# nreHieW/Eagle

Measured on AMD Instinct MI355X. Metric: frames/sec end-to-end (detect+keypoint+homography) @1280x720, higher is better.
Workload: dtype f32 (split: hi/lo binary16 pairs, 3 x fp16 MFMA per product, fp32 accumulate); detector (1.4 % of the FLOP): f32, exact v_mfma_f32_16x16x4_f32 chains

## Files before the change

eagle_amd/csrc/common.h:

```cpp
#pragma once
#include <hip/hip_runtime.h>
#include <hip/hip_fp16.h>
#include <cstdint>
#include <cstdio>
#include <string>
#include <vector>

#include "../../include/eagle.h"

namespace eagle {

enum Act : int { ACT_NONE = 0, ACT_RELU = 1, ACT_SILU = 2 };

struct Err {
    int code;
    std::string msg;
};
[[noreturn]] void fail(int code, const char* fmt, ...);

#define HIP_CHECK(expr)                                                                                \
    do {                                                                                               \
        hipError_t _e = (expr);                                                                        \
        if (_e != hipSuccess) ::eagle::fail(EAGLE_E_HIP, "%s failed: %s (%s:%d)", #expr, hipGetErrorString(_e), \
                                            __FILE__, __LINE__);                                       \
    } while (0)

void ensure_max_dynamic_lds(const void* fn, int bytes);

struct TView {
    void* p = nullptr;
    int n = 0, h = 0, w = 0;
    int c = 0;
    int cs = 0;
    int off = 0;
    int f32 = 0;
    size_t esize() const { return f32 ? 4 : 2; }
    TView slice(int o, int cc) const { TView v = *this; v.off = off + o; v.c = cc; return v; }
};

struct ConvConfig {
    int ks = 3, stride = 1;
    int kc = 0;
    int nt = 0;
    int wx = 2;
    int cin = 0, cout_pad = 0;
    int variant = 0;
};
struct ArgmaxPart { float score; int idx; };
struct ConvLaunch {
    ConvConfig cfg;
    TView x, y, r1, r2;
    const void* w = nullptr;
    const float* bias = nullptr;
    int pre_act = 0, post_act = 0;
    int out_f32 = 0;
    double flop = 0;
    float descale = 1.0f;
    ArgmaxPart* const* am_slot = nullptr;
    unsigned* const* sat_slot = nullptr;
};
int conv_tiles_per_frame(int precision, const ConvConfig& cfg, int ho, int wo);
bool conv_supported(int precision, const ConvConfig& cfg);
void conv_launch(int precision, const ConvLaunch& L, hipStream_t s);
size_t conv_weight_elems(int precision, const ConvConfig& cfg);
size_t conv_lds_bytes(int precision, const ConvConfig& cfg);
void conv_tile_weights(int precision, const ConvConfig& cfg, const float* w_hwio, int cin_real, int cout_real, void* dst, float* descale = nullptr);
inline int prec_tensor_fmt(int precision) { return precision == EAGLE_PREC_F32 ? 1 : precision == EAGLE_PREC_F32S ? 2 : 0; }
inline bool prec_is_f16_kernels(int precision) { return precision == EAGLE_PREC_F16 || precision == EAGLE_PREC_F32S; }
ConvConfig conv_choose(int precision, int ks, int stride, int cin_pad, int cout_pad, int wo, bool plain_epilogue = false, bool second_residual = false);

struct BneckLaunch {
    TView x, res, y;
    const void *w1 = nullptr, *w2 = nullptr, *w3 = nullptr;
    const float *b1 = nullptr, *b2 = nullptr, *b3 = nullptr;
    float ds1 = 1.f, ds2 = 1.f, ds3 = 1.f;
    unsigned* const* sat_slot = nullptr;
    unsigned long long* dbg = nullptr;
    bool ds_fused = false;
};
bool bneck_supported(const TView& x, int cmid, int cout);
void bneck_tile_weights(const float* w, int taps, int cin, int cout, std::vector<_Float16>& out, float* descale);
void bneck_scale_bias(std::vector<float>& b, float descale);
void bneck_launch(const BneckLaunch& L, hipStream_t s);

struct LetterBox { int new_h, new_w, top, left, out_h, out_w; };
LetterBox letterbox_geometry(int h, int w, int imgsz, int square = 0);
void preprocess_launch(int precision, const uint8_t* d_bgr, int n, int h, int w, const TView& kp, const TView& det,
                       const LetterBox& lb, hipStream_t s, int which = 3, int det_precision = -1);
struct FuseUp { TView z; };
void fuse_sum_launch(const TView& base, const FuseUp* ups, int n_up, int relu, const TView& y, hipStream_t s, unsigned* sat = nullptr);
void maxpool5_launch(const TView& x, const TView& y, hipStream_t s);
void upsample2_launch(const TView& x, const TView& y, hipStream_t s);
void split_to_f32_launch(const TView& x, const TView& y, hipStream_t s);

void heat_argmax_launch(const TView& logits, ArgmaxPart* parts, int chunks, hipStream_t s);

struct DetLevel { TView box, cls; int gh, gw; float stride; int a0; };
struct DetScratch {
    int A = 0;
    float* boxes = nullptr;
    float* conf = nullptr;
    int* cls = nullptr;
    unsigned long long* keys = nullptr;
    int* count = nullptr;
};
void yolo_decode_launch(const DetLevel* lv, int n_lv, int n, int nc, float conf_floor, const DetScratch& sc, hipStream_t s);

struct PostParams {
    int frame_h, frame_w, in_h, in_w;
    int hm_h, hm_w, hm_chunks;
    double keypoint_conf, detector_conf, ransac_thresh;
    float nms_iou;
    int ransac_max_iters, lm_iters;
};
void nms_launch(const DetScratch& sc, int n, const PostParams& pp, EagleFrameResult* d_out, hipStream_t s);
void post_launch(const ArgmaxPart* parts, int n, const PostParams& pp, EagleFrameResult* d_out, hipStream_t s);
void reproject_launch(EagleFrameResult* d_recs, const double* d_Hs, const unsigned char* d_flags, int n, int frame_h, int frame_w, hipStream_t s);
void homography_only_launch(const float* d_img, const float* d_world, int npts, double thresh, int max_iters, int lm_iters,
                            double* d_H, uint8_t* d_mask, int* d_ok, hipStream_t s);


struct ClipView {
    const uint8_t* bgr = nullptr;
    const uint8_t* g[3] = {nullptr, nullptr, nullptr};
    int lh[3] = {0, 0, 0}, lw[3] = {0, 0, 0};
    int levels = 0;
    int n = 0, h = 0, w = 0;
};
struct MemList { int n; EagleFlowKp kp[EAGLE_N_LANDMARKS]; };
struct ChainState {
    int n_prev; EagleFlowKp prev[EAGLE_N_LANDMARKS];
    int has_H, compute_h; double H[9];
    int stalled;
    int error;
    int lk_valid, lk_n;
    float lk_prev[2 * EAGLE_N_LANDMARKS], lk_next[2 * EAGLE_N_LANDMARKS];
    unsigned char lk_status[EAGLE_N_LANDMARKS];
    int flow_n; EagleFlowKp flow[EAGLE_N_LANDMARKS];
};
void gray_pyramid_launch(const uint8_t* d_bgr, int n, int h, int w, uint8_t* g0, uint8_t* g1, uint8_t* g2, hipStream_t s);
void lk_launch(const ClipView& cv, int src_frame, int dst_frame, ChainState* st, const MemList* mem, int kint, hipStream_t s);
struct EccResult { int ok, iters; double rho; float M[6]; };
void ecc_small_launch(const uint8_t* gray, uint8_t* small, int n, int h, int w, int dh, int dw, double inv_scale , hipStream_t s);
void ecc_launch(const uint8_t* small, const uint8_t* carry, const int2* pairs, int n_pairs, EccResult* out, int h, int w, int max_iter, double eps, hipStream_t s);
struct YuvArgs {
    const uint8_t* src;
    uint8_t* dst;
    int h, w;
    int64_t frame_stride, y_pitch, c_offset, c_pitch, v_offset;
    int c_step;
    int vec;
};
void yuv_to_bgr_launch(const YuvArgs& a, int n, hipStream_t s);
void team_colors_launch(const uint8_t* d_bgr, int n_frames, int fh, int fw, const EagleCrop* d_crops, int n_crops, int* d_counts, hipStream_t s);

void reid_crop_launch(const uint8_t* d_bgr, int n_frames, int fh, int fw, const EagleCrop* d_crops, int n, const TView& out, hipStream_t s);
void reid_conv7_launch(const TView& x, const float* w, const float* b, const TView& y, int n, hipStream_t s);
void reid_maxpool3s2_launch(const TView& x, const TView& y, int n, hipStream_t s);
void reid_avgpool2_launch(const TView& x, const TView& y, int n, hipStream_t s);
void reid_dw3_launch(const TView& x, const float* w, const float* b, const TView& y, int n, hipStream_t s);
void reid_gate_launch(const TView* streams, const float* w1, const float* b1, const float* w2, const float* b2, int c_real, int r, float* g, const TView& y, int n, hipStream_t s);
void reid_head_launch(const TView& x, const float* w, const float* b, float* feats, int dim, int n, hipStream_t s);

struct Tracker;
Tracker* tracker_create(const EagleTrackParams* p);
void tracker_destroy(Tracker* t);
bool tracker_apply(Tracker* t, EagleFrameResult* rec, int frame_h, int frame_w, double detector_conf, const double* warp = nullptr,
                   const float* feats = nullptr, const int* feat_det = nullptr, int n_feat = 0);
void similarity_ransac(const double* p0, const double* p1, int n, double* W6);
int lk_debug(const char* key, long long value, void* out, long long out_bytes);
void decode_mem_launch(const ArgmaxPart* parts, int n, const PostParams& pp, MemList* mem, int first, int stride, hipStream_t s);
void chain_launch(const ClipView& cv, ChainState* st, const MemList* mem, EagleFrameResult* recs, const PostParams& pp, int frame,
                  int kint, int hint, int calib, hipStream_t s);
void flow_filter_launch(const ClipView& cv, ChainState* st, int hue_frame, hipStream_t s);

}
```

eagle_amd/csrc/conv.hip:

```cpp
#include <algorithm>
#include <cmath>
#include <cstdlib>
#include <mutex>

#include "common.h"
#include "dmath.h"
#include "conv_internal.h"

namespace eagle {

static int f16_ps(int kc) { const int g = kc / 8; return kc * 2 + ((g % 2 == 0) ? 16 : 0); }
static int f16_ni(int ks, int kc) { return (ks * ks * (kc / 8) + 3) / 4; }

enum FormKind { GENERIC, WSTAT, ADIRECT };
enum StrideForm { S1, S2D, S2T };
enum WeightImage { W_F32, W_F16, W_F16_S2D, W_SPLIT, W_SPLIT_AD, W_SPLIT_S2D, W_SPLIT_M32 };
struct Form {
    int prec, variant, kind;
    int pw;
    int sform, rows, cols;
    int kc, nt, halo_bufs;
    int wimage;
    int grid_cap;
    ConvKernelGetter get;
};
static constexpr Form gen(int prec, int variant, int pw, int wimage, int kind = GENERIC) { return {prec, variant, kind, pw, S1, 0, 0, 0, 0, 0, wimage, 0, nullptr}; }
static constexpr Form ad(int prec, int variant, int sform, int rows, int cols, int nt, int halo_bufs, int wimage, ConvKernelGetter get, int grid_cap = 0)
{
    return {prec, variant, ADIRECT, 0, sform, rows, cols, prec == EAGLE_PREC_F16 ? 32 : 16, nt, halo_bufs, wimage, grid_cap, get};
}
static constexpr int F16 = EAGLE_PREC_F16, F32 = EAGLE_PREC_F32, F32S = EAGLE_PREC_F32S;
static constexpr Form g_forms[] = {
    gen(F32, 0, 4, W_F32), gen(F32, 3, 2, W_F32), gen(F32, 4, 1, W_F32),
    gen(F16, 0, 4, W_F16), gen(F16, 2, 4, W_F16), gen(F16, 3, 2, W_F16), gen(F16, 4, 1, W_F16), gen(F16, 6, 4, W_F16, WSTAT), gen(F16, 7, 2, W_F16, WSTAT),
    ad(F16, 8, S1, 4, 32, 12, 2, W_F16, conv_ad_kernel_s1_bn192), ad(F16, 9, S1, 8, 32, 6, 2, W_F16, conv_ad_kernel_s1_bn96),
    ad(F16, 10, S2D, 4, 32, 12, 2, W_F16_S2D, conv_ad_kernel_s2_bn192), ad(F16, 11, S2D, 8, 32, 6, 2, W_F16_S2D, conv_ad_kernel_s2_bn96),
    gen(F32S, 0, 4, W_SPLIT), gen(F32S, 3, 2, W_SPLIT), gen(F32S, 18, 6, W_SPLIT),
    ad(F32S, 8, S1, 4, 32, 12, 2, W_SPLIT_AD, conv_ad_split_kernel_bn192), ad(F32S, 9, S1, 8, 32, 6, 2, W_SPLIT_AD, conv_ad_split_kernel_bn96),
    ad(F32S, 10, S2D, 4, 32, 12, 2, W_SPLIT_S2D, conv_ad_split_kernel_s2_bn192), ad(F32S, 11, S2D, 8, 32, 6, 2, W_SPLIT_S2D, conv_ad_split_kernel_s2_bn96),
    ad(F32S, 12, S1, 8, 32, 3, 2, W_SPLIT_AD, conv_ad_split_kernel48), ad(F32S, 13, S1, 16, 32, 3, 1, W_SPLIT_AD, conv_ad_split_kernel48sb),
    ad(F32S, 19, S1, 16, 32, 3, 2, W_SPLIT_AD, conv_ad_split_kernel48ring, 256),
    ad(F32S, 14, S2T, 4, 32, 12, 1, W_SPLIT_AD, conv_ad_split_kernel_s2t_bn192), ad(F32S, 15, S2T, 4, 32, 6, 1, W_SPLIT_AD, conv_ad_split_kernel_s2t_bn96),
    ad(F32S, 21, S1, 4, 32, 12, 2, W_SPLIT_M32, conv_ad_split32_kernel_bn192), ad(F32S, 22, S1, 8, 32, 6, 2, W_SPLIT_M32, conv_ad_split32_kernel_bn96),
    ad(F32S, 23, S1, 2, 64, 12, 2, W_SPLIT_M32, conv_ad_split32_kernel_w64_bn192), ad(F32S, 24, S1, 4, 64, 6, 2, W_SPLIT_M32, conv_ad_split32_kernel_w64_bn96)};

static const Form* find_form(int precision, int variant)
{
    for (const Form& f : g_forms)
        if (f.prec == precision && f.variant == variant) return &f;
    return nullptr;
}
static const Form& form_of(int precision, const ConvConfig& c)
{
    const Form* f = find_form(precision, c.variant);
    if (!f) fail(EAGLE_E_NOKERNEL, "no conv kernel form: prec=%d variant=%d", precision, c.variant);
    return *f;
}
static int kind_of(int precision, const ConvConfig& c) { const Form* f = find_form(precision, c.variant); return f ? f->kind : -1; }

static size_t lds_bytes(int precision, const ConvConfig& c)
{
    const Form& f = form_of(precision, c);
    if (f.kind == ADIRECT) {
        int hpix, rec, strips;
        if (precision == EAGLE_PREC_F16) { hpix = f.sform == S2D ? (f.rows + 1) * 33 : (f.rows + 2) * 34; rec = 96; strips = 4 * 32 * 112; }
        else if (f.wimage == W_SPLIT_M32) { hpix = (f.rows + 2) * (f.cols + 2); rec = 80; strips = 4 * 32 * 128; }
        else { hpix = f.sform == S2T ? (2 * f.rows + 1) * 66 : (f.rows + 2) * 34; rec = 96; strips = 4 * 16 * 208; }
        const int slabs = ((hpix * rec + 1023) / 1024 + 3) / 4 * 4;
        return (size_t)f.halo_bufs * slabs * 1024 + strips;
    }
    const int th = 4 * f.pw / c.wx, tw = 16 * c.wx;
    const int hw = (tw - 1) * c.stride + c.ks, hh = (th - 1) * c.stride + c.ks;
    const int bn = c.nt * 16;
    if (precision == EAGLE_PREC_F16) {
        const size_t operands = (size_t)f16_ni(c.ks, c.kc) * 4 * bn * 16 + (size_t)hh * hw * f16_ps(c.kc);
        const size_t strips = (size_t)4 * f.pw * 16 * (bn * 2 + 16);
        return f.kind == WSTAT ? operands + strips + 16 : std::max(operands + 16, strips);
    }
    if (precision == EAGLE_PREC_F32S) {
        const size_t operands = (size_t)f16_ni(c.ks, c.kc) * 2 * 4 * bn * 16 + (size_t)hh * hw * f16_ps(2 * c.kc);
        const size_t strips = (size_t)4 * f.pw * 16 * (bn * 4 + 16);
        return std::max(operands + 16, strips);
    }
    return (size_t)c.ks * c.ks * (c.kc / 4) * 4 * bn * 4 + (size_t)hh * hw * (c.kc + 1) * 4;
}

size_t conv_lds_bytes(int precision, const ConvConfig& c) { return lds_bytes(precision, c); }
int conv_tiles_per_frame(int precision, const ConvConfig& c, int ho, int wo)
{
    const Form& f = form_of(precision, c);
    const int th = f.kind == ADIRECT ? f.rows : 4 * f.pw / c.wx, tw = f.kind == ADIRECT ? f.cols : 16 * c.wx;
    return ((wo + tw - 1) / tw) * ((ho + th - 1) / th);
}

static const Inst* generic_inst(int precision, const ConvConfig& c)
{
    for (auto part : {conv_inst_part0, conv_inst_part1, conv_inst_part2, conv_inst_part3, conv_inst_split0, conv_inst_split1, conv_inst_split2}) {
        int n = 0;
        const Inst* t = part(&n);
        for (int k = 0; k < n; ++k)
            if (t[k].prec == precision && t[k].ks == c.ks && t[k].s == c.stride && t[k].kc == c.kc && t[k].nt == c.nt && t[k].variant == c.variant) return &t[k];
    }
    return nullptr;
}
bool conv_supported(int precision, const ConvConfig& c)
{
    const Form* f = find_form(precision, c.variant);
    if (f && f->kind == ADIRECT) return c.ks == 3 && c.stride == (f->sform == S1 ? 1 : 2) && c.kc == f->kc && c.nt == f->nt;
    return f && generic_inst(precision, c);
}

struct Tuned { int ks, s, cin, cout, wo, kc, nt, wx, variant; };
static const Tuned g_tuned[] = {
#include "conv_tuned.inc"
    {0, 0, 0, 0, 0, 0, 0, 0, 0}};
static const Tuned g_tuned_f32[] = {
#include "conv_tuned_f32.inc"
    {0, 0, 0, 0, 0, 0, 0, 0, 0}};
static const Tuned g_tuned_split[] = {
#include "conv_tuned_split.inc"
    {0, 0, 0, 0, 0, 0, 0, 0, 0}};
static bool tuned_match(const Tuned& t, const ConvConfig& c, int wo, ConvConfig* q)
{
    if (t.ks != c.ks || t.s != c.stride || t.cin != c.cin || t.cout != c.cout_pad || t.wo != wo) return false;
    *q = c; q->kc = t.kc; q->nt = t.nt; q->wx = t.wx; q->variant = t.variant;
    return true;
}

static bool env_force(const char* name, int* a, int* b, int* c) { const char* f = getenv(name); return f && sscanf(f, "%d,%d,%d", a, b, c) == 3; }
static bool env_off(const char* name) { const char* e = getenv(name); return e && atoi(e) == 0; }

static const int g_nts[] = {6, 4, 3, 2, 1};
static ConvConfig with_ad(ConvConfig c, int kc, int v192, int v96)
{
    c.kc = kc;
    if (c.cout_pad % 192 == 0) { c.nt = 12; c.variant = v192; } else { c.nt = 6; c.variant = v96; }
    return c;
}

static ConvConfig choose_f32(ConvConfig c, int wo)
{
    ConvConfig q = c; q.kc = (c.cin < 16) ? 4 : 16;
    if (env_force("EAGLE_F32_FORCE", &q.nt, &q.wx, &q.variant) && (q.wx == 1 || q.wx == 2) && q.nt >= 1 && c.cout_pad % (16 * q.nt) == 0 &&
        conv_supported(EAGLE_PREC_F32, q) && lds_bytes(EAGLE_PREC_F32, q) <= 160 * 1024)
        return q;
    for (const Tuned& t : g_tuned_f32)
        if (tuned_match(t, c, wo, &q) && conv_supported(EAGLE_PREC_F32, q)) return q;
    c.nt = 1;
    for (int nt : g_nts)
        if (c.cout_pad % (16 * nt) == 0) { c.nt = nt; break; }
    c.kc = (c.cin < 16) ? 4 : 16;
    if (c.stride == 2 && c.ks == 3) {
        q = c; q.variant = 3;
        if (conv_supported(EAGLE_PREC_F32, q)) return q;
    }
    return c;
}

static ConvConfig choose_split(ConvConfig c, int wo, bool plain_epilogue)
{
    const int prec = EAGLE_PREC_F32S, cin = c.cin, cout = c.cout_pad;
    ConvConfig q = c;
    if (env_force("EAGLE_CONV_FORCE", &q.kc, &q.nt, &q.variant) && cin % q.kc == 0 && cout % (16 * q.nt) == 0 && conv_supported(prec, q)) {
        if (form_of(prec, q).pw == 6) q.wx = 3;
        if (lds_bytes(prec, q) <= 160 * 1024) return q;
    }
    if (plain_epilogue && c.ks == 3 && c.stride == 2 && cin % 48 == 0 && cout % 96 == 0) return with_ad(c, 16, 14, 15);
    if (!env_off("EAGLE_CONV_M32") && plain_epilogue && c.ks == 3 && c.stride == 1 && cin % 16 == 0 && cout % 96 == 0) return with_ad(c, 16, 21, wo > 32 ? 24 : 22);
    for (const Tuned& t : g_tuned_split)
        if (tuned_match(t, c, wo, &q)) {
            const Form* f = find_form(prec, q.variant);
            if (kind_of(prec, q) == ADIRECT && !(plain_epilogue && cin % (f->sform == S2D ? 16 : 48) == 0)) continue;
            if (conv_supported(prec, q) && lds_bytes(prec, q) <= 160 * 1024) return q;
        }
    if (plain_epilogue && c.ks == 3 && c.stride == 1 && cin % 48 == 0 && cout % 96 == 0) return with_ad(c, 16, 8, 9);
    static const int skcs[] = {32, 16, 8};
    long best = -1;
    c.nt = 1; c.kc = 8; c.variant = 0;
    for (int variant : {0, 3})
        for (int nt : g_nts) {
            if (cout % (16 * nt)) continue;
            for (int kc : skcs) {
                if (cin % kc) continue;
                ConvConfig t = c; t.nt = nt; t.kc = kc; t.variant = variant;
                if (!conv_supported(prec, t)) continue;
                if (lds_bytes(prec, t) > 80 * 1024) continue;
                const int pw = form_of(prec, t).pw;
                if (nt * pw > 12) continue;
                const long score = (long)nt * pw * 1000 + kc * 10 + (variant == 0 ? 1 : 0);
                if (score > best) { best = score; c.nt = nt; c.kc = kc; c.variant = variant; }
            }
        }
    return c;
}

static ConvConfig choose_f16(ConvConfig c, int wo, bool plain_epilogue, bool plain_one)
{
    const int prec = EAGLE_PREC_F16, cin = c.cin, cout = c.cout_pad;
    ConvConfig q = c;
    if (env_force("EAGLE_CONV_FORCE", &q.kc, &q.nt, &q.variant) && cin % q.kc == 0 && cout % (16 * q.nt) == 0 && conv_supported(prec, q) &&
        lds_bytes(prec, q) <= 160 * 1024 && (kind_of(prec, q) == WSTAT ? plain_one : kind_of(prec, q) == ADIRECT ? plain_epilogue : true))
        return q;
    if (plain_epilogue && c.ks == 3 && c.stride == 1 && cin % 32 == 0 && cout % 96 == 0) return with_ad(c, 32, 8, 9);
    if (plain_epilogue && c.ks == 3 && c.stride == 2 && cin % 8 == 0 && cin >= 32 && cout % 96 == 0) return with_ad(c, 32, 10, 11);
    for (const Tuned& t : g_tuned)
        if (tuned_match(t, c, wo, &q)) {
            if (kind_of(prec, q) == WSTAT && !plain_one) continue;
            if (conv_supported(prec, q) && lds_bytes(prec, q) <= 160 * 1024) return q;
        }
    static const int kcs[] = {64, 48, 32, 16, 8};
    long best = -1;
    c.nt = 1; c.kc = 8;
    for (int nt : g_nts) {
        if (cout % (16 * nt)) continue;
        for (int kc : kcs) {
            if (cin % kc) continue;
            ConvConfig t = c; t.nt = nt; t.kc = kc;
            if (!conv_supported(prec, t)) continue;
            if (lds_bytes(prec, t) > 80 * 1024) continue;
            const long score = (long)kc * nt * 1000 + kc;
            if (score > best) { best = score; c.nt = nt; c.kc = kc; }
        }
    }
    return c;
}

ConvConfig conv_choose(int precision, int ks, int stride, int cin_pad, int cout_pad, int wo, bool plain_epilogue, bool second_residual)
{
    ConvConfig c;
    c.ks = ks; c.stride = stride; c.cin = cin_pad; c.cout_pad = cout_pad;
    c.wx = (wo > 16) ? 2 : 1;
    if (precision == EAGLE_PREC_F32) return choose_f32(c, wo);
    if (precision == EAGLE_PREC_F32S) return choose_split(c, wo, plain_epilogue);
    return choose_f16(c, wo, plain_epilogue, plain_epilogue && !second_residual);
}

size_t conv_weight_elems(int precision, const ConvConfig& c)
{
    const int bn = c.nt * 16, nblk = c.cout_pad / bn, nch = c.cin / c.kc;
    switch (form_of(precision, c).wimage) {
    case W_F16_S2D: return (size_t)nblk * (4 * c.cin / 32) * 16 * bn * 8;
    case W_F16: return (size_t)nblk * nch * f16_ni(c.ks, c.kc) * 4 * bn * 8;
    case W_SPLIT_S2D: return (size_t)nblk * (4 * c.cin / 16) * 6 * 4 * bn * 8;
    case W_SPLIT_M32: return (size_t)nblk * (c.cin / 16) * 18 * (bn / 32) * 512;
    case W_SPLIT_AD: return (size_t)nblk * (c.cin / 16) * 14 * 4 * bn * 8;
    case W_SPLIT: return (size_t)nblk * nch * f16_ni(c.ks, c.kc) * 2 * 4 * bn * 8;
    default: return (size_t)nblk * nch * c.ks * c.ks * (c.kc / 4) * 4 * bn;
    }
}

void conv_tile_weights(int precision, const ConvConfig& c, const float* w, int cin_real, int cout_real, void* dst, float* descale)
{
    const int bn = c.nt * 16, nblk = c.cout_pad / bn, nch = c.cin / c.kc, taps = c.ks * c.ks, wimage = form_of(precision, c).wimage;
    auto W = [&](int tap, int ci, int co) -> float {
        return (ci < cin_real && co < cout_real) ? w[((size_t)tap * cin_real + ci) * cout_real + co] : 0.0f;
    };
    if (descale) *descale = 1.0f;
    if (precision == EAGLE_PREC_F32S) {
        float amax = 0.f;
        for (size_t k = 0; k < (size_t)taps * cin_real * cout_real; ++k) amax = std::max(amax, std::fabs(w[k]));
        int e = 0;
        if (amax > 0.f) (void)std::frexp(amax, &e);
        const int sw = 15 - e;
        const float scale = std::ldexp(1.0f, sw);
        if (descale) *descale = std::ldexp(1.0f, -(sw + 4));
        _Float16* d = (_Float16*)dst;
        if (wimage == W_SPLIT_S2D) {
            const int per_phase = c.cin / 16;
            for (int b = 0; b < nblk; ++b)
                for (int ch = 0; ch < 4 * per_phase; ++ch)
                    for (int k = 0; k < 6; ++k)
                        for (int qq = 0; qq < 4; ++qq)
                            for (int nn = 0; nn < bn; ++nn)
                                for (int j = 0; j < 8; ++j) {
                                    const int ph = ch / per_phase, c0 = (ch - ph * per_phase) * 16, ry = ph >> 1, rx = ph & 1;
                                    const int tp = k < 4 ? k : 2 * (k - 4) + (qq >> 1), tyy = tp >> 1, txx = tp & 1;
                                    const int ky = tyy == 0 ? (ry == 1 ? 0 : -1) : (ry == 0 ? 1 : 2), kx = txx == 0 ? (rx == 1 ? 0 : -1) : (rx == 0 ? 1 : 2);
                                    float v = 0.f;
                                    if (ky >= 0 && kx >= 0) v = W(ky * 3 + kx, c0 + (qq & 1) * 8 + j, b * bn + nn) * scale;
                                    const _Float16 hi = (_Float16)v;
                                    *d++ = k < 4 ? hi : (_Float16)(v - (float)hi);
                                }
            return;
        }
        if (wimage == W_SPLIT_M32) {
            for (int b = 0; b < nblk; ++b)
                for (int ch = 0; ch < c.cin / 16; ++ch)
                    for (int tap = 0; tap < 9; ++tap)
                        for (int part = 0; part < 2; ++part)
                            for (int mb = 0; mb < bn / 32; ++mb)
                                for (int l = 0; l < 64; ++l)
                                    for (int j = 0; j < 8; ++j) {
                                        const float v = W(tap, ch * 16 + (l >> 5) * 8 + j, b * bn + mb * 32 + (l & 31)) * scale;
                                        const _Float16 hi = (_Float16)v;
                                        *d++ = part == 0 ? hi : (_Float16)(v - (float)hi);
                                    }
            return;
        }
        if (wimage == W_SPLIT_AD) {
            for (int b = 0; b < nblk; ++b)
                for (int ch = 0; ch < c.cin / 16; ++ch)
                    for (int k = 0; k < 14; ++k)
                        for (int qq = 0; qq < 4; ++qq)
                            for (int nn = 0; nn < bn; ++nn)
                                for (int j = 0; j < 8; ++j) {
                                    const int tap = k < 9 ? k : 2 * (k - 9) + (qq >> 1);
                                    float v = 0.f;
                                    if (tap < 9) v = W(tap, ch * 16 + (qq & 1) * 8 + j, b * bn + nn) * scale;
                                    const _Float16 hi = (_Float16)v;
                                    *d++ = k < 9 ? hi : (_Float16)(v - (float)hi);
                                }
            return;
        }
        const int G = c.kc / 8, NGR = taps * G, NI = f16_ni(c.ks, c.kc);
        for (int b = 0; b < nblk; ++b)
            for (int ch = 0; ch < nch; ++ch)
                for (int i = 0; i < NI; ++i)
                    for (int part = 0; part < 2; ++part)
                        for (int qq = 0; qq < 4; ++qq)
                            for (int nn = 0; nn < bn; ++nn)
                                for (int j = 0; j < 8; ++j) {
                                    const int g = 4 * i + qq;
                                    float v = 0.f;
                                    if (g < NGR) { const int tap = g / G, cg = g % G; v = W(tap, ch * c.kc + cg * 8 + j, b * bn + nn) * scale; }
                                    const _Float16 hi = (_Float16)v;
                                    *d++ = part == 0 ? hi : (_Float16)(v - (float)hi);
                                }
        return;
    }
    if (wimage == W_F16_S2D) {
        _Float16* d = (_Float16*)dst;
        const int nch2 = 4 * c.cin / 32;
        for (int b = 0; b < nblk; ++b)
            for (int ch = 0; ch < nch2; ++ch)
                for (int g = 0; g < 16; ++g)
                    for (int nn = 0; nn < bn; ++nn)
                        for (int j = 0; j < 8; ++j) {
                            const int tp = g / 4, cg = g % 4, tyy = tp >> 1, txx = tp & 1;
                            const int sc = ch * 32 + cg * 8 + j, ph = sc / c.cin, ci = sc - ph * c.cin, ry = ph >> 1, rx = ph & 1;
                            const int ky = tyy == 0 ? (ry == 1 ? 0 : -1) : (ry == 0 ? 1 : 2), kx = txx == 0 ? (rx == 1 ? 0 : -1) : (rx == 0 ? 1 : 2);
                            *d++ = (_Float16)((ky < 0 || kx < 0) ? 0.f : W(ky * 3 + kx, ci, b * bn + nn));
                        }
        return;
    }
    if (precision == EAGLE_PREC_F16) {
        const int G = c.kc / 8, NGR = taps * G, NI = f16_ni(c.ks, c.kc);
        _Float16* d = (_Float16*)dst;
        for (int b = 0; b < nblk; ++b)
            for (int ch = 0; ch < nch; ++ch)
                for (int g = 0; g < NI * 4; ++g)
                    for (int nn = 0; nn < bn; ++nn)
                        for (int j = 0; j < 8; ++j) {
                            float v = 0.f;
                            if (g < NGR) {
                                const int tap = g / G, cg = g % G;
                                v = W(tap, ch * c.kc + cg * 8 + j, b * bn + nn);
                            }
                            *d++ = (_Float16)v;
                        }
    } else {
        const int CSTEPS = c.kc / 4;
        float* d = (float*)dst;
        for (int b = 0; b < nblk; ++b)
            for (int ch = 0; ch < nch; ++ch)
                for (int tap = 0; tap < taps; ++tap)
                    for (int cs = 0; cs < CSTEPS; ++cs)
                        for (int qq = 0; qq < 4; ++qq)
                            for (int nn = 0; nn < bn; ++nn) *d++ = W(tap, ch * c.kc + cs * 4 + qq, b * bn + nn);
    }
}

static std::mutex g_page_mutex;
static const void* conv_zero_page()
{
    static void* z[64] = {};
    int dev = 0;
    HIP_CHECK(hipGetDevice(&dev));
    std::lock_guard<std::mutex> g(g_page_mutex);
    if (!z[dev]) { HIP_CHECK(hipMalloc(&z[dev], 256)); HIP_CHECK(hipMemset(z[dev], 0, 256)); }
    return z[dev];
}
static void* conv_trash_page()
{
    static void* z[64] = {};
    int dev = 0;
    HIP_CHECK(hipGetDevice(&dev));
    std::lock_guard<std::mutex> g(g_page_mutex);
    if (!z[dev]) HIP_CHECK(hipMalloc(&z[dev], 8192));
    return z[dev];
}

void conv_launch(int precision, const ConvLaunch& L, hipStream_t s)
{
    const ConvConfig& c = L.cfg;
    if (!conv_supported(precision, c)) fail(EAGLE_E_NOKERNEL, "no conv kernel instance: prec=%d ks=%d s=%d kc=%d nt=%d", precision, c.ks, c.stride, c.kc, c.nt);
    const Form& f = form_of(precision, c);
    ConvArgs a;
    a.x = L.x.p; a.xcs = L.x.cs; a.xoff = L.x.off; a.N = L.x.n; a.H = L.x.h; a.W = L.x.w;
    a.w = L.w; a.bias = L.bias;
    a.y = L.y.p; a.ycs = L.y.cs; a.yoff = L.y.off; a.Ho = L.y.h; a.Wo = L.y.w;
    a.r1 = L.r1.p; a.r1cs = L.r1.cs; a.r1off = L.r1.off;
    a.r2 = L.r2.p; a.r2cs = L.r2.cs; a.r2off = L.r2.off;
    a.descale = L.descale;
    if (precision == EAGLE_PREC_F32S) {
        if (L.x.f32 != 2 || (L.r1.p && L.r1.f32 != 2) || (L.r2.p && L.r2.f32 != 2) || L.y.f32 != (L.out_f32 ? 1 : 2))
            fail(EAGLE_E_INVALID, "split conv: operand tensor formats do not match the family");
        a.xcs *= 2; a.xoff *= 2; a.r1cs *= 2; a.r1off *= 2; a.r2cs *= 2; a.r2off *= 2;
        if (!L.out_f32) { a.ycs *= 2; a.yoff *= 2; }
    }
    if (!a.r1 && a.r2) { a.r1 = a.r2; a.r1cs = a.r2cs; a.r1off = a.r2off; a.r2 = nullptr; }
    a.pre_act = L.pre_act; a.post_act = L.post_act; a.out_f32 = L.out_f32 || precision == EAGLE_PREC_F32;
    a.wx = c.wx;
    a.nchunks = c.cin / c.kc;
    a.zeros = conv_zero_page(); a.trash = conv_trash_page(); a.xcd = 0; a.gy = 1; a.stack = 0;
    a.am = L.am_slot ? *L.am_slot : nullptr; a.am_cs = c.cout_pad;
    a.sat = (L.sat_slot && precision == EAGLE_PREC_F32S) ? *L.sat_slot : nullptr;
    if (f.kind == ADIRECT) {
        if (a.out_f32 || a.pre_act != 0 || a.post_act > 1 || L.am_slot || (precision == EAGLE_PREC_F32S && c.cin % (f.wimage == W_SPLIT_AD ? 48 : 16)))
            fail(EAGLE_E_NOKERNEL, "A-direct conv needs 2-byte / split output, pre_act none, post_act in {none, ReLU} and, in the split family, Cin = 16 k (48 k for variants 8, 9 and 12 - 15)");
        if (f.sform == S2D) a.nchunks = 4 * c.cin / c.kc;
        a.tiles_x = (a.Wo + f.cols - 1) / f.cols; a.tiles_y = (a.Ho + f.rows - 1) / f.rows;
        a.gy = c.cout_pad / (c.nt * 16);
        const size_t lim = (size_t)1 << 31;
        if ((size_t)a.N * a.H * a.W * a.xcs * 2 >= lim || (size_t)a.N * a.Ho * a.Wo * std::max(std::max(a.ycs, a.r1 ? a.r1cs : 0), a.r2 ? a.r2cs : 0) * 2 >= lim)
            fail(EAGLE_E_INVALID, "fp16 conv: a tensor of %d frames reaches 2 GiB; use a smaller device batch", a.N);
        const int nres = (a.r1 ? 1 : 0) + (a.r2 ? 1 : 0);
        const int items = a.tiles_x * a.tiles_y * a.N * a.gy;
        const bool deep = items <= 256;
        for (bool d : {false, true}) ensure_max_dynamic_lds((const void*)f.get(nres, d), 160 * 1024);
        hipLaunchKernelGGL(f.get(nres, deep), dim3(f.grid_cap ? std::min(items, f.grid_cap) : items), dim3(256), lds_bytes(precision, c), s, a);
        HIP_CHECK(hipGetLastError());
        return;
    }
    const int th = 4 * f.pw / c.wx, tw = 16 * c.wx;
    a.tiles_x = (a.Wo + tw - 1) / tw; a.tiles_y = (a.Ho + th - 1) / th;
    if (precision == EAGLE_PREC_F32) {
        if (!env_off("EAGLE_F32_STACK") && c.stride == 1 && a.N > 1 && a.Ho == a.H) { a.stack = 1; a.tiles_y = (a.N * (a.Ho + 1) + th - 1) / th; }
        if ((size_t)a.N * a.H * a.W * a.xcs * 4 >= ((size_t)1 << 31)) fail(EAGLE_E_INVALID, "fp32 conv: the input tensor of %d frames reaches 2 GiB; use a smaller device batch", a.N);
    }
    const bool ws = f.kind == WSTAT;
    if (a.am && (!prec_is_f16_kernels(precision) || ws))
        fail(EAGLE_E_NOKERNEL, "fused heat-map maxima need the generic fp16 kernel");
    if (prec_is_f16_kernels(precision)) {
        const size_t lim = (size_t)1 << 31;
        const size_t cs_out = std::max(std::max(a.out_f32 ? 2 * a.ycs : a.ycs, a.r1 ? a.r1cs : 0), a.r2 ? a.r2cs : 0);
        if ((size_t)a.N * a.H * a.W * a.xcs * 2 >= lim || (size_t)a.N * a.Ho * a.Wo * cs_out * 2 >= lim)
            fail(EAGLE_E_INVALID, "fp16 conv: a tensor of %d frames reaches 2 GiB; use a smaller device batch", a.N);
    }
    const ConvKernel fn = generic_inst(precision, c)->fn;
    const size_t lds = lds_bytes(precision, c);
    ensure_max_dynamic_lds((const void*)fn, 160 * 1024);
    const int gy = c.cout_pad / (c.nt * 16);
    int gx = a.stack ? a.tiles_x * a.tiles_y : a.tiles_x * a.tiles_y * a.N;
    if (ws) {
        if (c.kc != c.cin || a.out_f32 || a.r2 || a.pre_act != 0 || a.post_act > 1 || (size_t)a.N * a.H * a.W * a.xcs * 2 >= (1ull << 31) || (size_t)a.N * a.Ho * a.Wo * std::max(a.ycs, a.r1 ? a.r1cs : 0) * 2 >= (1ull << 31))
            fail(EAGLE_E_NOKERNEL, "weight-stationary conv needs kc == cin, fp16 output, at most one residual, pre_act none, post_act in {none, ReLU} and tensors below 2 GiB (kc=%d cin=%d)", c.kc, c.cin);
        const int per_cu = (int)std::max<size_t>(1, std::min<size_t>(2, (160 * 1024) / lds));
        const int unit = 8 * gy;
        gx = std::max(unit, std::min((gx * gy + unit - 1) / unit * unit, 256 * per_cu / unit * unit));
    }
    a.gy = gy;
    a.xcd = (prec_is_f16_kernels(precision) && !ws && (c.ks == 3 || (c.ks == 1 && gy > 1))) ? 1 : 0;
    dim3 grid(gx, gy);
    if (a.xcd) grid = dim3(gx * gy, 1);
    if (ws) grid = dim3(gx, 1);
    hipLaunchKernelGGL(fn, grid, dim3(256), lds, s, a);
    HIP_CHECK(hipGetLastError());
}

}
```

eagle_amd/csrc/conv_internal.h:

```cpp
#pragma once
#include "common.h"

namespace eagle {

using half8 = __attribute__((ext_vector_type(8))) _Float16;
using half4 = __attribute__((ext_vector_type(4))) _Float16;
using f32x4 = __attribute__((ext_vector_type(4))) float;
using u32x4 = __attribute__((ext_vector_type(4))) unsigned int;
using u32x2 = __attribute__((ext_vector_type(2))) unsigned int;

struct ConvArgs {
    const void* x; int xcs, xoff; int N, H, W;
    const void* w; const float* bias;
    void* y; int ycs, yoff; int Ho, Wo;
    const void* r1; int r1cs, r1off;
    const void* r2; int r2cs, r2off;
    int pre_act, post_act, out_f32;
    int wx, tiles_x, tiles_y, nchunks;
    int gy;
    int stack;
    int xcd;
    ArgmaxPart* am;
    int am_cs;
    float descale;
    const void* zeros;
    void* trash;
    unsigned* sat;
};

struct BneckArgs {
    const void* x; int xcs, xoff; int N, H, W, nch1;
    const void *w1, *w2, *w3; const float *b1, *b2, *b3; float ds1, ds2, ds3;
    const void* r; int rcs, roff;
    void* y; int ycs, yoff;
    int tiles_x, tiles_y;
    unsigned* sat;
    unsigned long long* dbg;
};

typedef void (*ConvKernel)(ConvArgs);
struct Inst { int prec, ks, s, kc, nt, variant; ConvKernel fn; };
const Inst* conv_inst_part0(int* n); const Inst* conv_inst_part1(int* n); const Inst* conv_inst_part2(int* n); const Inst* conv_inst_part3(int* n);
const Inst* conv_inst_split0(int* n); const Inst* conv_inst_split1(int* n); const Inst* conv_inst_split2(int* n);
inline int res_slot(int n_res) { return n_res < 0 ? 0 : n_res > 2 ? 2 : n_res; }
typedef ConvKernel (*ConvKernelGetter)(int n_res, bool deep);
ConvKernel conv_ad_kernel_s1_bn192(int n_res, bool deep);
ConvKernel conv_ad_kernel_s1_bn96(int n_res, bool deep);
ConvKernel conv_ad_kernel_s2_bn192(int n_res, bool deep);
ConvKernel conv_ad_kernel_s2_bn96(int n_res, bool deep);
ConvKernel conv_ad_split_kernel_bn192(int n_res, bool deep);
ConvKernel conv_ad_split_kernel_bn96(int n_res, bool deep);
ConvKernel conv_ad_split_kernel_s2_bn192(int n_res, bool deep);
ConvKernel conv_ad_split_kernel_s2_bn96(int n_res, bool deep);
ConvKernel conv_ad_split_kernel_s2t_bn192(int n_res, bool deep);
ConvKernel conv_ad_split_kernel_s2t_bn96(int n_res, bool deep);
ConvKernel conv_ad_split_kernel48(int n_res, bool deep);
ConvKernel conv_ad_split_kernel48sb(int n_res, bool deep);
ConvKernel conv_ad_split_kernel48ring(int n_res, bool deep);
ConvKernel conv_ad_split32_kernel_bn192(int n_res, bool deep);
ConvKernel conv_ad_split32_kernel_bn96(int n_res, bool deep);
ConvKernel conv_ad_split32_kernel_w64_bn192(int n_res, bool deep);
ConvKernel conv_ad_split32_kernel_w64_bn96(int n_res, bool deep);

}
```

eagle_amd/csrc/conv_kernels.inc:

```
#ifndef EAGLE_CONV_KERNELS_INC
#define EAGLE_CONV_KERNELS_INC
#ifndef EAGLE_ABL
#define EAGLE_ABL 0
#endif
template <int KC> struct F16Geom {
    static constexpr int G = KC / 8;
    static constexpr int PS = KC * 2 + ((G % 2 == 0) ? 16 : 0);
};

using i32x4 = __attribute__((ext_vector_type(4))) int;
__device__ __forceinline__ i32x4 make_rsrc(const void* p, int bytes)
{
    const unsigned long long b = (unsigned long long)p;
    i32x4 r = {(int)(unsigned)b, (int)((unsigned)(b >> 32) & 0xFFFF), bytes, 0x00020000};
    return r;
}
__device__ __forceinline__ float relu_if(float v, bool relu) { return (relu && !(v > 0.0f)) ? 0.0f : v; }

using rsrc_t = __amdgpu_buffer_rsrc_t;
__device__ __forceinline__ rsrc_t tensor_rsrc(const void* p) { return __builtin_amdgcn_make_buffer_rsrc((void*)p, 0, p ? 0x7FFFFFFF : 0, 0x00020000); }
constexpr unsigned OOB_OFF = 0x80000000u;
#ifndef EAGLE_STORE_NT
#define EAGLE_STORE_NT 1
#endif
// ... 114 lines not shown
                float best = -1.0f; int idx = 0x7fffffff;
#pragma unroll
                for (int p = 0; p < PW; ++p) {
                    if (pix[p] == OOB_OFF) continue;
                    const float sg = d_sigmoidf(acc[tt][p][r]);
                    const int li = (int)pix[p] - n * a.Ho * a.Wo;
                    if (sg > best || (sg == best && li < idx)) { best = sg; idx = li; }
                }
                bs[tt * 4 + r] = best; bi[tt * 4 + r] = idx;
            }
#pragma unroll
        for (int m = 1; m < 16; m <<= 1)
#pragma unroll
            for (int k = 0; k < NT * 4; ++k) {
                const float ob = __shfl_xor(bs[k], m, 64); const int oi = __shfl_xor(bi[k], m, 64);
                if (ob > bs[k] || (ob == bs[k] && oi < bi[k])) { bs[k] = ob; bi[k] = oi; }
            }
        ArgmaxPart* red = (ArgmaxPart*)smem_base;
        if (lx == 0) {
#pragma unroll
            for (int tt = 0; tt < NT; ++tt)
#pragma unroll
                for (int r = 0; r < 4; ++r) { ArgmaxPart v; v.score = bs[tt * 4 + r]; v.idx = bi[tt * 4 + r]; red[wave * BN + tt * 16 + q * 4 + r] = v; }
        }
        __syncthreads();
        const int tid = wave * 64 + lane;
        if (tid < BN) {
            ArgmaxPart b = red[tid];
#pragma unroll
            for (int w = 1; w < 4; ++w) { const ArgmaxPart o = red[w * BN + tid]; if (o.score > b.score || (o.score == b.score && o.idx < b.idx)) b = o; }
            const int TH = 4 * PW / WX, TW = 16 * WX;
            const int tile = (oy0 / TH) * a.tiles_x + ox0 / TW;
            a.am[((size_t)n * a.tiles_x * a.tiles_y + tile) * a.am_cs + nb * BN + tid] = b;
        }
        return;
    }
    if (a.out_f32) {
#pragma unroll
        for (int p = 0; p < PW; ++p) {
            if (pix[p] == OOB_OFF) continue;
#pragma unroll
            for (int tt = 0; tt < NT; ++tt)
                *(float4*)((float*)a.y + (size_t)pix[p] * a.ycs + a.yoff + co0 + tt * 16) = make_float4(acc[tt][p][0], acc[tt][p][1], acc[tt][p][2], acc[tt][p][3]);
        }
        return;
    }
    if constexpr (SPLIT) {
        float m = 0.0f;
#pragma unroll
        for (int p = 0; p < PW; ++p)
#pragma unroll
            for (int tt = 0; tt < NT; ++tt) { const float mm = split_absmax4(m, acc[tt][p][0], acc[tt][p][1], acc[tt][p][2], acc[tt][p][3]); m = pix[p] == OOB_OFF ? m : mm; }
        split_report(a.sat, n, m);
    }
#pragma unroll
    for (int p = 0; p < PW; ++p)
#pragma unroll
        for (int tt = 0; tt < NT; ++tt) {
            if constexpr (SPLIT) {
                split_store4(strip + (p * 16 + lx) * RS + split_elem(tt * 16 + q * 4) * 2, acc[tt][p][0], acc[tt][p][1], acc[tt][p][2], acc[tt][p][3]);
            } else {
                half4 o = {(_Float16)acc[tt][p][0], (_Float16)acc[tt][p][1], (_Float16)acc[tt][p][2], (_Float16)acc[tt][p][3]};
                *(half4*)(strip + (p * 16 + lx) * RS + (tt * 16 + q * 4) * 2) = o;
            }
        }
    const rsrc_t ys = tensor_rsrc(a.y);
#pragma unroll
    for (int e0 = 0; e0 < PW * 16 * GO; e0 += 64) {
        const int e = e0 + lane;
        const int px = e / GO, grp = e - px * GO, p = px >> 4, lxp = px & 15;
        const int s = wave * PW + p, row = s / WX, xb = s - row * WX;
        const int oy = oy0 + row, ox = ox0 + xb * 16 + lxp;
        const bool ok = e < PW * 16 * GO && oy < a.Ho && ox < a.Wo;
        const u32x4 v = *(const u32x4*)(strip + (ok ? px * RS + grp * 16 : 0));
        const unsigned vo = (ok && !((EAGLE_ABL == 3 || EAGLE_ABL >= 4) && SPLIT)) ? ((unsigned)((n * a.Ho + oy) * a.Wo + ox) * (unsigned)a.ycs + (unsigned)(a.yoff + nb * EB + grp * 8)) * 2u : OOB_OFF;
        __builtin_amdgcn_raw_buffer_store_b128(v, ys, vo, 0, SPLIT ? EAGLE_STORE_NT * 2 : EAGLE_F16_STORE_NT * 2);
    }
}

template <int R_, int M_, int r> __device__ __forceinline__ void sg_step()
{
    if constexpr (r < R_) {
        __builtin_amdgcn_sched_group_barrier(0x100, 1, 0);
        __builtin_amdgcn_sched_group_barrier(0x008, (M_ * (r + 1)) / R_ - (M_ * r) / R_, 0);
        sg_step<R_, M_, r + 1>();
    }
}
template <int NI_, int R_, int M_, int i> __device__ __forceinline__ void sg_all()
{
    if constexpr (i + 1 < NI_) { sg_step<R_, M_, 0>(); sg_all<NI_, R_, M_, i + 1>(); }
}
template <int NI_, int R_, int M_> __device__ __forceinline__ void mfma_phase_schedule_rm()
{
    __builtin_amdgcn_sched_group_barrier(0x100, R_, 0);
    sg_all<NI_, R_, M_, 0>();
    __builtin_amdgcn_sched_group_barrier(0x008, M_, 0);
}
template <int NI_, int NT_, int PW_> __device__ __forceinline__ void mfma_phase_schedule()
{
    __builtin_amdgcn_sched_group_barrier(0x100, NT_ + PW_, 0);
    sg_all<NI_, NT_ + PW_, NT_ * PW_, 0>();
    __builtin_amdgcn_sched_group_barrier(0x008, NT_ * PW_, 0);
}

#if EAGLE_ABL == 1 || EAGLE_ABL == 4 || EAGLE_ABL == 5 || EAGLE_ABL == 6 || EAGLE_ABL == 8 || EAGLE_ABL == 9
__device__ __forceinline__ f32x4 abl_xor(const half8& a, const half8& b, f32x4 c)
{
    const u32x4 ua = __builtin_bit_cast(u32x4, a), ub = __builtin_bit_cast(u32x4, b);
    u32x4 uc = __builtin_bit_cast(u32x4, c);
    uc[0] = uc[0] ^ ua[0] ^ ub[3];
    return __builtin_bit_cast(f32x4, uc);
}
#define EAGLE_MFMA_SPLIT(A_, B_, C_) abl_xor(A_, B_, C_)
#else
#define EAGLE_MFMA_SPLIT(A_, B_, C_) __builtin_amdgcn_mfma_f32_16x16x32_f16(A_, B_, C_, 0, 0, 0)
#endif
template <int KS, int S, int KC, int NT, bool PIPE, int PW, bool SPLIT = false>
__global__ __launch_bounds__(256, 2) void conv_f16_kernel(ConvArgs a)
{
    constexpr int KCS = SPLIT ? 2 * KC : KC;
    constexpr int GL = KC / 8;
    constexpr int G = F16Geom<KCS>::G;
#ifndef EAGLE_SPLIT_PLANAR
#define EAGLE_SPLIT_PLANAR 0
#endif
    constexpr bool PLANAR = SPLIT && KC == 16 && EAGLE_SPLIT_PLANAR;
    constexpr int PS = PLANAR ? 96 : F16Geom<KCS>::PS;
    constexpr int LO_OFF = PLANAR ? 32 : 16;
#ifndef EAGLE_S2_COLPLANES
#define EAGLE_S2_COLPLANES 0
#endif
    constexpr bool COLPLANES = S == 2 && KS == 3 && EAGLE_S2_COLPLANES;
    constexpr int TAPS = KS * KS;
    constexpr int NGR = TAPS * GL;
    constexpr int NI = (NGR + 3) / 4;
    constexpr int BN = NT * 16;
    constexpr int HALFW = 4 * BN * 16;
    constexpr int STEPB = SPLIT ? 2 * HALFW : HALFW;
    constexpr int WBYTES = NI * STEPB;
    extern __shared__ __attribute__((aligned(16))) char smem[];
    char* lds_w = smem;
    char* lds_a = smem + WBYTES + 16;

    const int WX = a.wx, TH = 4 * PW / WX, TW = 16 * WX;
    const int halo_w = (TW - 1) * S + KS, halo_h = (TH - 1) * S + KS;
    const int tid = threadIdx.x, lane = tid & 63, wave = tid >> 6, q = lane >> 4, lx = lane & 15;
    int t = blockIdx.x, nb = blockIdx.y;
    if (a.xcd) {
        const int gy = a.gy, total = a.tiles_x * a.tiles_y * a.N * gy;
        const int b = blockIdx.x, xcd = b & 7, k = b >> 3, qn = total >> 3, rn = total & 7;
        const int item = (xcd < rn ? xcd * (qn + 1) : rn * (qn + 1) + (xcd - rn) * qn) + k;
        t = item / gy; nb = item - t * gy;
    }
    const int tx = t % a.tiles_x; t /= a.tiles_x;
    const int ty = t % a.tiles_y;
    const int n = t / a.tiles_y;
    const int oy0 = ty * TH, ox0 = tx * TW;
    const int iy0 = oy0 * S - KS / 2, ix0 = ox0 * S - KS / 2;

    f32x4 acc[NT][PW];
#pragma unroll
    for (int i = 0; i < NT; ++i)
#pragma unroll
        for (int p = 0; p < PW; ++p) acc[i][p] = f32x4{0.f, 0.f, 0.f, 0.f};

    int abase[PW];
#pragma unroll
    for (int p = 0; p < PW; ++p) {
        const int s = wave * PW + p, row = s / WX, xb = s - row * WX;
        abase[p] = ((row * S) * halo_w + (xb * 16 + lx) * (COLPLANES ? 1 : S)) * PS;
    }
    int koff[NI];
#pragma unroll
    for (int i = 0; i < NI; ++i) {
        const int g = 4 * i + q;
        if (g < NGR) {
            const int tap = g / GL, cg = g - tap * GL, ky = tap / KS, kx = tap - ky * KS;
            koff[i] = (ky * halo_w + (COLPLANES ? (kx & 1) * ((halo_w + 1) >> 1) + (kx >> 1) : kx)) * PS + cg * ((SPLIT && !PLANAR) ? 32 : 16);
        } else {
            koff[i] = 0;
        }
    }
    const int wlane = (q * BN + lx) * 16;
    const int ngroups = halo_h * halo_w * G;

    constexpr int MAXPIX = (KS == 1) ? 64 * PW : ((S == 1) ? (PW == 6 ? 500 : (PW == 4 ? 340 : (PW == 2 ? 204 : 136))) : (PW == 4 ? 1105 : (PW == 2 ? 585 : 325)));
    constexpr int NPA = (MAXPIX * G + 255) / 256;
    constexpr int NPW = (WBYTES / 16 + 255) / 256;
    constexpr int RND = PIPE ? NPA : 8;
    static_assert(!PIPE || NPA <= 8, "pipelined staging is meant for small chunks");
    const rsrc_t xrs = tensor_rsrc(a.x), wrs = tensor_rsrc(a.w);
    unsigned aoff[NPA];
    int ldso[NPA];
#pragma unroll
    for (int j = 0; j < NPA; ++j) {
        const int idx = tid + 256 * j;
        const int pix = idx / G, g = idx - pix * G;
        const int hy = pix / halo_w, hx = pix - hy * halo_w;
        const int iy = iy0 + hy, ix = ix0 + hx;
        const bool ok = idx < ngroups && iy >= 0 && iy < a.H && ix >= 0 && ix < a.W;
        aoff[j] = ok ? (unsigned)(((n * a.H + iy) * a.W + ix) * a.xcs + g * 8) * 2u : OOB_OFF;
        const int slot = PLANAR ? (g & 1) * 2 + (g >> 1) : g;
        const int lpix = COLPLANES ? hy * halo_w + (hx & 1) * ((halo_w + 1) >> 1) + (hx >> 1) : pix;
        ldso[j] = idx < ngroups ? lpix * PS + slot * 16 : -16;
    }
    u32x4 pw[NPW], pa[RND];
#define STAGE_LOAD(CH_, R0_)                                                                                            \
    {                                                                                                                   \
        if ((R0_) == 0) {                                                                                               \
            const unsigned wso_ = (unsigned)(nb * a.nchunks + (CH_)) * (unsigned)WBYTES;                                \
            if (!((EAGLE_ABL == 5 || EAGLE_ABL == 6 || EAGLE_ABL >= 8) && SPLIT && (CH_) > 0))                                               \
            _Pragma("unroll") for (int i = 0; i < NPW; ++i) { const int o = (tid + 256 * i) * 16; pw[i] = __builtin_amdgcn_raw_buffer_load_b128(wrs, o < WBYTES ? o : 0, wso_, 0); } \
        }                                                                                                               \
        const unsigned xso_ = (unsigned)(a.xoff + (CH_) * KCS) * 2u;                                                    \
        _Pragma("unroll") for (int j = 0; j < RND; ++j)                                                                 \
            if ((R0_) + j < NPA && !((EAGLE_ABL == 2 || EAGLE_ABL >= 4) && SPLIT && (CH_) > 0)) pa[j] = __builtin_amdgcn_raw_buffer_load_b128(xrs, aoff[(R0_) + j < NPA ? (R0_) + j : 0], xso_, 0); \
    }
#define STAGE_STORE(R0_)                                                                                                \
    if (!((EAGLE_ABL == 6 || EAGLE_ABL >= 8) && SPLIT && ch > 0))                                                                         \
    {                                                                                                                   \
        if ((R0_) == 0) {                                                                                               \
            _Pragma("unroll") for (int i = 0; i < NPW; ++i) { const int o = (tid + 256 * i) * 16; if (o < WBYTES) *(u32x4*)(lds_w + o) = pw[i]; } \
        }                                                                                                               \
        _Pragma("unroll") for (int j = 0; j < RND; ++j)                                                                 \
            if ((R0_) + j < NPA) *(u32x4*)(lds_a + ldso[(R0_) + j < NPA ? (R0_) + j : 0]) = pa[j];                      \
    }
#ifndef EAGLE_SPLIT_RPRE
#define EAGLE_SPLIT_RPRE 1
#endif
    constexpr bool RPRE = KS == 3 && NT * PW <= 12 && (!SPLIT || EAGLE_SPLIT_RPRE);
    u32x2 r1pre[NT][PW], r1prel[NT][PW];
#pragma unroll
    for (int tt = 0; tt < NT; ++tt)
#pragma unroll
        for (int p = 0; p < PW; ++p) { r1pre[tt][p] = u32x2{0u, 0u}; if constexpr (SPLIT) r1prel[tt][p] = u32x2{0u, 0u}; }
    if (PIPE) STAGE_LOAD(0, 0)
    for (int ch = 0; ch < a.nchunks; ++ch) {
        if (PIPE) {
            if (ch > 0) __syncthreads();
            STAGE_STORE(0)
            __syncthreads();
            if (ch + 1 < a.nchunks) STAGE_LOAD(ch + 1, 0)
        } else {
#pragma unroll
            for (int r0 = 0; r0 < NPA; r0 += RND) {
                STAGE_LOAD(ch, r0)
                STAGE_STORE(r0)
            }
            __syncthreads();
        }
        if (RPRE && ch == a.nchunks - 1 && a.r1) {
            const rsrc_t rs_ = tensor_rsrc(a.r1);
#pragma unroll
            for (int p = 0; p < PW; ++p) {
                const int s = wave * PW + p, row = s / WX, xb_ = s - row * WX;
                const int oy = oy0 + row, ox = ox0 + xb_ * 16 + lx;
                const int ce_ = SPLIT ? nb * 2 * BN + (q >> 1) * 16 + (q & 1) * 4 : nb * BN + q * 4;
                const unsigned vo_ = (oy < a.Ho && ox < a.Wo) ? ((unsigned)((n * a.Ho + oy) * a.Wo + ox) * (unsigned)a.r1cs + (unsigned)(a.r1off + ce_)) * 2u : OOB_OFF;
#pragma unroll
                for (int tt = 0; tt < NT; ++tt) {
                    r1pre[tt][p] = __builtin_amdgcn_raw_buffer_load_b64(rs_, vo_ + tt * (SPLIT ? 64 : 32), 0, SPLIT ? EAGLE_RES_NT * 2 : 0);
                    if constexpr (SPLIT) r1prel[tt][p] = __builtin_amdgcn_raw_buffer_load_b64(rs_, vo_ + tt * 64 + 16, 0, EAGLE_RES_NT * 2);
                }
            }
        }
#ifndef EAGLE_NO_SETPRIO
        if constexpr (NT >= 4) __builtin_amdgcn_s_setprio(3);
#endif
        if constexpr (SPLIT) {
#pragma unroll
            for (int i_ = 0; i_ < NI; ++i_) {
                const int i = (EAGLE_ABL >= 8) ? 0 : i_;
                half8 wa[NT], wl[NT], xb[PW], xl[PW];
#pragma unroll
                for (int tt = 0; tt < NT; ++tt) wa[tt] = *(const half8*)(lds_w + wlane + i * STEPB + tt * 256);
#pragma unroll
                for (int p = 0; p < PW; ++p) xb[p] = *(const half8*)(lds_a + abase[p] + koff[i]);
#pragma unroll
                for (int tt = 0; tt < NT; ++tt)
#pragma unroll
                    for (int p = 0; p < PW; ++p)
                        acc[tt][p] = EAGLE_MFMA_SPLIT(wa[tt], xb[p], acc[tt][p]);
#pragma unroll
                for (int p = 0; p < PW; ++p) xl[p] = *(const half8*)(lds_a + abase[p] + koff[i] + LO_OFF);
#pragma unroll
                for (int tt = 0; tt < NT; ++tt)
#pragma unroll
                    for (int p = 0; p < PW; ++p)
                        acc[tt][p] = EAGLE_MFMA_SPLIT(wa[tt], xl[p], acc[tt][p]);
#pragma unroll
                for (int tt = 0; tt < NT; ++tt) wl[tt] = *(const half8*)(lds_w + wlane + i * STEPB + HALFW + tt * 256);
#pragma unroll
                for (int tt = 0; tt < NT; ++tt)
#pragma unroll
                    for (int p = 0; p < PW; ++p)
                        acc[tt][p] = EAGLE_MFMA_SPLIT(wl[tt], xb[p], acc[tt][p]);
            }
#if defined(EAGLE_SPLIT_SCHED) && EAGLE_SPLIT_SCHED == 2
            __builtin_amdgcn_sched_group_barrier(0x100, NT + PW, 0);
#pragma unroll
            for (int i = 0; i < NI; ++i) {
                __builtin_amdgcn_sched_group_barrier(0x100, PW, 0); __builtin_amdgcn_sched_group_barrier(0x008, NT * PW, 0);
                __builtin_amdgcn_sched_group_barrier(0x100, NT, 0); __builtin_amdgcn_sched_group_barrier(0x008, NT * PW, 0);
                if (i + 1 < NI) __builtin_amdgcn_sched_group_barrier(0x100, NT + PW, 0);
                __builtin_amdgcn_sched_group_barrier(0x008, NT * PW, 0);
            }
#elif defined(EAGLE_SPLIT_SCHED)
            mfma_phase_schedule_rm<NI, 2 * (NT + PW), 3 * NT * PW>();
#endif
        } else {
#pragma unroll
        for (int i = 0; i < NI; ++i) {
            half8 wa[NT], xb[PW];
#pragma unroll
            for (int tt = 0; tt < NT; ++tt) wa[tt] = *(const half8*)(lds_w + wlane + i * (4 * BN * 16) + tt * 256);
#pragma unroll
            for (int p = 0; p < PW; ++p) xb[p] = *(const half8*)(lds_a + abase[p] + koff[i]);
#pragma unroll
            for (int tt = 0; tt < NT; ++tt)
#pragma unroll
                for (int p = 0; p < PW; ++p)
                    acc[tt][p] = __builtin_amdgcn_mfma_f32_16x16x32_f16(wa[tt], xb[p], acc[tt][p], 0, 0, 0);
        }
        mfma_phase_schedule<NI, NT, PW>();
        }
#ifndef EAGLE_NO_SETPRIO
        if constexpr (NT >= 4) __builtin_amdgcn_s_setprio(0);
#endif
        if (!PIPE) __syncthreads();
    }
#undef STAGE_LOAD
#undef STAGE_STORE

    if (PIPE) __syncthreads();
    constexpr int RS_ = (SPLIT ? BN * 4 : BN * 2) + 16;
    if (EAGLE_ABL == 9 && SPLIT) {
        float sacc = 0.f;
#pragma unroll
        for (int tt = 0; tt < NT; ++tt)
#pragma unroll
            for (int p = 0; p < PW; ++p) sacc += acc[tt][p][0] + acc[tt][p][1] + acc[tt][p][2] + acc[tt][p][3];
        if (sacc == 1.2345e38f) *(float*)a.trash = sacc;
        return;
    }
    f16_epilogue<NT, PW, SPLIT>(a, acc, smem + wave * (PW * 16 * RS_), n, oy0, ox0, nb, wave, q, lx, lane, RPRE ? r1pre : nullptr, smem, (RPRE && SPLIT) ? r1prel : nullptr);
}

template <int CIN, int NT, int PW, int WGS>
__global__ __launch_bounds__(256, WGS) void conv_f16_ws_kernel(ConvArgs a)
{
    constexpr int KS = 3;
    constexpr int G = CIN / 8;
    constexpr int PS = F16Geom<CIN>::PS;
    constexpr int NGR = 9 * G;
    constexpr int NI = (NGR + 3) / 4;
    constexpr int BN = NT * 16, GO = BN / 8, RS = BN * 2 + 16;
    constexpr int WBYTES = NI * 4 * BN * 16;
    extern __shared__ __attribute__((aligned(16))) char smem[];
    char* lds_w = smem;
    char* lds_a = smem + WBYTES + 16;

    const int WX = a.wx, TH = 4 * PW / WX, TW = 16 * WX;
    const int halo_w = TW + 2, halo_h = TH + 2;
    const int tid = threadIdx.x, lane = tid & 63, wave = tid >> 6, q = lane >> 4, lx = lane & 15;
    char* strip = lds_a + halo_h * halo_w * PS + wave * (PW * 16 * RS);

    const int gy = a.gy, nwg = gridDim.x;
// ... 70 lines not shown

    const bool post_relu = a.post_act == 1;
    constexpr int NRV = NT * PW;
    static_assert(NPA <= 16 && NRV <= 16 && NSO <= 16, "prefetch registers");
    u32x4 pa0, pa1, pa2, pa3, pa4, pa5, pa6, pa7, pa8, pa9, pa10, pa11, pa12, pa13, pa14, pa15;
    u32x2 rv0, rv1, rv2, rv3, rv4, rv5, rv6, rv7, rv8, rv9, rv10, rv11, rv12, rv13, rv14, rv15;
#define WS_LIST16(M) M(0) M(1) M(2) M(3) M(4) M(5) M(6) M(7) M(8) M(9) M(10) M(11) M(12) M(13) M(14) M(15)
#define WS_LD1(j)                                                                                                       \
    if constexpr (j < NPA) {                                                                                            \
        const int iy = iy0_ + (hyx[j < NPA ? j : 0] >> 16), ix = ix0_ + (hyx[j < NPA ? j : 0] & 0xFFFF);                \
        const bool ok_ = (unsigned)iy < (unsigned)a.H && (unsigned)ix < (unsigned)a.W;                                   \
        const int vo_ = ok_ ? xb_ + goff[j < NPA ? j : 0] : OOB;                                                        \
        asm volatile("buffer_load_dwordx4 %0, %1, %2, 0 offen" : "=v"(pa##j) : "v"(vo_), "s"(xrs));                     \
    }
#define WS_LOAD_HALO(N_, OY0_, OX0_)                                                                                     \
    {                                                                                                                   \
        const int iy0_ = (OY0_) - 1, ix0_ = (OX0_) - 1;                                                                 \
        const int xb_ = ((((N_) * a.H + iy0_) * a.W + ix0_) * a.xcs + a.xoff) * 2;                                      \
        WS_LIST16(WS_LD1)                                                                                               \
    }
#define WS_RS1(e)                                                                                                       \
    if constexpr (e < NRV) {                                                                                            \
        constexpr int p = (e < NRV ? e : 0) / NT, tt = (e < NRV ? e : 0) % NT;                                          \
        asm volatile("buffer_load_dwordx2 %0, %1, %2, 0 offen offset:%3" : "=v"(rv##e) : "v"(rvo_[p]), "s"(rrs), "n"(tt * 32)); \
    }
#define WS_LOAD_RES(N_, OY0_, OX0_)                                                                                      \
    {                                                                                                                   \
        const int rb_ = (((N_) * a.Ho + (OY0_)) * a.Wo + (OX0_)) * a.r1cs * 2;                                          \
        int rvo_[PW];                                                                                                   \
        _Pragma("unroll") for (int p = 0; p < PW; ++p)                                                                  \
            rvo_[p] = ((OY0_) + (r_yx[p] >> 16) < a.Ho && (OX0_) + (r_yx[p] & 0xFFFF) < a.Wo) ? rb_ + r_off[p] : OOB;   \
        WS_LIST16(WS_RS1)                                                                                               \
    }
#define WS_PIN_PA(j) if constexpr (j < NPA) asm volatile("" : "+v"(pa##j));
#define WS_PIN_RV(e) if constexpr (e < NRV) asm volatile("" : "+v"(rv##e));
#define WS_ST1(j) if constexpr (j < NPA) *(u32x4*)(lds_a + loff[j < NPA ? j : 0]) = pa##j;
#define WS_EP1(e)                                                                                                       \
    if constexpr (e < NRV) {                                                                                            \
        constexpr int p = (e < NRV ? e : 0) / NT, tt = (e < NRV ? e : 0) % NT;                                          \
        const float4 bv = bvr[tt];                                                                                      \
        float v[4] = {acc[tt][p][0] + bv.x, acc[tt][p][1] + bv.y, acc[tt][p][2] + bv.z, acc[tt][p][3] + bv.w};          \
        if constexpr (hasr_) {                                                                                          \
            const half4 rh = __builtin_bit_cast(half4, rv##e);                                                          \
            _Pragma("unroll") for (int r = 0; r < 4; ++r) v[r] = (float)rh[r] + v[r];                                   \
        }                                                                                                               \
        if constexpr (relu_) {                                                                                          \
            _Pragma("unroll") for (int r = 0; r < 4; ++r) v[r] = __builtin_fmaxf(v[r], 0.0f);                           \
        }                                                                                                               \
        half4 o = {(_Float16)v[0], (_Float16)v[1], (_Float16)v[2], (_Float16)v[3]};                                     \
        *(half4*)(strip + (p * 16 + lx) * RS + (tt * 16 + q * 4) * 2) = o;                                              \
    }
#define WS_EPILOGUE(RELU_, HASR_) { constexpr bool relu_ = RELU_, hasr_ = HASR_; WS_LIST16(WS_EP1) }
    const bool has_r1 = a.r1 != nullptr;

    __builtin_amdgcn_s_waitcnt(0x0F70);
    int cx, cy, cn;
    {
        const int tx0 = t_begin % a.tiles_x, r0 = t_begin / a.tiles_x;
        cn = r0 / a.tiles_y; cy = r0 - cn * a.tiles_y; cx = tx0;
        WS_LOAD_HALO(cn, cy * TH, cx * TW)
        WS_LOAD_RES(cn, cy * TH, cx * TW)
    }
    asm volatile("s_waitcnt vmcnt(%0)" ::"n"(NRV));
    for (int t = t_begin; t < t_end; ++t) {
        __builtin_amdgcn_s_barrier();
        asm volatile("s_waitcnt vmcnt(%0)" ::"n"(NSO + NRV));
        WS_LIST16(WS_PIN_PA)
        WS_LIST16(WS_ST1)
        __builtin_amdgcn_fence(__ATOMIC_RELEASE, "workgroup", "local");
        __builtin_amdgcn_s_barrier();
        __builtin_amdgcn_fence(__ATOMIC_ACQUIRE, "workgroup", "local");

        const int n = cn, oy0 = cy * TH, ox0 = cx * TW;
        if (t + 1 < t_end) {
            if (++cx == a.tiles_x) { cx = 0; if (++cy == a.tiles_y) { cy = 0; ++cn; } }
        }
        const int n1 = cn, oy1 = cy * TH, ox1 = cx * TW;
        WS_LOAD_HALO(n1, oy1, ox1)

        f32x4 acc[NT][PW];
#pragma unroll
        for (int i = 0; i < NT; ++i)
#pragma unroll
            for (int p = 0; p < PW; ++p) acc[i][p] = f32x4{0.f, 0.f, 0.f, 0.f};
#pragma unroll
        for (int i = 0; i < NI; ++i) {
            half8 wa[NT], xb[PW];
#pragma unroll
            for (int tt = 0; tt < NT; ++tt) wa[tt] = *(const half8*)(lds_w + wlane + i * (4 * BN * 16) + tt * 256);
#pragma unroll
            for (int p = 0; p < PW; ++p) xb[p] = *(const half8*)(lds_a + abase[p] + koff[i]);
#pragma unroll
            for (int tt = 0; tt < NT; ++tt)
#pragma unroll
                for (int p = 0; p < PW; ++p)
                    acc[tt][p] = __builtin_amdgcn_mfma_f32_16x16x32_f16(wa[tt], xb[p], acc[tt][p], 0, 0, 0);
        }
        mfma_phase_schedule<NI, NT, PW>();

        asm volatile("s_waitcnt vmcnt(%0)" ::"n"(NPA));
        WS_LIST16(WS_PIN_RV)
        if (post_relu) {
            if (has_r1) WS_EPILOGUE(true, true) else WS_EPILOGUE(true, false)
        } else {
            if (has_r1) WS_EPILOGUE(false, true) else WS_EPILOGUE(false, false)
        }
        const int yb = ((n * a.Ho + oy0) * a.Wo + ox0) * a.ycs * 2;
#pragma unroll
        for (int k = 0; k < NSO; ++k) {
            const u32x4 v = *(const u32x4*)(strip + so_l[k]);
            const int vo = (oy0 + (so_yx[k] >> 16) < a.Ho && ox0 + (so_yx[k] & 0xFFFF) < a.Wo) ? yb + so_g[k] : OOB;
            asm volatile("buffer_store_dwordx4 %0, %1, %2, 0 offen\n\ts_nop 1" ::"v"(v), "v"(vo), "s"(yrs) : "memory");
        }
        WS_LOAD_RES(n1, oy1, ox1)
    }
    asm volatile("s_waitcnt vmcnt(0)");
#undef WS_LOAD_HALO
#undef WS_LOAD_RES
#undef WS_LD1
#undef WS_RS1
#undef WS_ST1
#undef WS_EP1
#undef WS_EPILOGUE
#undef WS_PIN_PA
#undef WS_PIN_RV
#undef WS_LIST16
}



template <int KS, int S, int KC, int NT, int PW = 4>
__global__ __launch_bounds__(256) void conv_f32_kernel(ConvArgs a)
{
    constexpr int PSF = KC + 1;
    constexpr int TAPS = KS * KS;
    constexpr int CSTEPS = KC / 4;
    constexpr int NI = TAPS * CSTEPS;
    constexpr int BN = NT * 16;
    constexpr int WFLOATS = NI * 4 * BN;
    extern __shared__ __attribute__((aligned(16))) char smem[];
    float* lds_w = (float*)smem;
    float* lds_a = lds_w + WFLOATS;

    const int WX = a.wx, TH = 4 * PW / WX, TW = 16 * WX;
    const int halo_w = (TW - 1) * S + KS, halo_h = (TH - 1) * S + KS;
    const int tid = threadIdx.x, lane = tid & 63, wave = tid >> 6, q = lane >> 4, lx = lane & 15;
    const bool stack = a.stack != 0;
    const int Hs = a.Ho + 1;
    int t = blockIdx.x;
    const int tx = t % a.tiles_x; t /= a.tiles_x;
    const int ty = stack ? t : t % a.tiles_y;
    const int n0 = stack ? 0 : t / a.tiles_y;
    const int nb = blockIdx.y;
    const int oy0 = ty * TH, ox0 = tx * TW;
    const int iy0 = oy0 * S - KS / 2, ix0 = ox0 * S - KS / 2;

    f32x4 acc[NT][PW];
#pragma unroll
    for (int i = 0; i < NT; ++i)
#pragma unroll
        for (int p = 0; p < PW; ++p) acc[i][p] = f32x4{0.f, 0.f, 0.f, 0.f};
    int abase[PW];
#pragma unroll
    for (int p = 0; p < PW; ++p) {
        const int s = wave * PW + p, row = s / WX, xb = s - row * WX;
        abase[p] = ((row * S) * halo_w + (xb * 16 + lx) * S) * PSF + q;
    }
    const int wlane = q * BN + lx;
    const int nelem = halo_h * halo_w * CSTEPS;
    constexpr int MAXPIX = (KS == 1) ? ((64 * PW - 1) * S + 1) : (S == 1 ? (PW == 4 ? 340 : PW == 2 ? 204 : 136) : (PW == 4 ? 1105 : PW == 2 ? 585 : 325));
    constexpr int NPA = (MAXPIX * CSTEPS + 255) / 256;
    const rsrc_t xrs = tensor_rsrc(a.x);
    unsigned aoff[NPA];
    int ldso[NPA];
#pragma unroll
    for (int j = 0; j < NPA; ++j) {
        const int idx = tid + 256 * j;
        const int pix = idx / CSTEPS, g = idx - pix * CSTEPS;
        const int hy = pix / halo_w, hx = pix - hy * halo_w;
        const int ix = ix0 + hx;
        int n = n0, iy = iy0 + hy;
        bool ok = idx < nelem && ix >= 0 && ix < a.W;
        if (stack) { n = iy >= 0 ? iy / Hs : 0; iy -= n * Hs; ok = ok && n < a.N; }
        ok = ok && iy >= 0 && iy < a.H;
        aoff[j] = ok ? (unsigned)(((n * a.H + iy) * a.W + ix) * a.xcs + a.xoff + g * 4) * 4u : OOB_OFF;
        ldso[j] = idx < nelem ? pix * PSF + g * 4 : -1;
    }

    for (int ch = 0; ch < a.nchunks; ++ch) {
        {
            const float* wsrc = (const float*)a.w + (size_t)(nb * a.nchunks + ch) * WFLOATS;
            for (int o = tid * 4; o < WFLOATS; o += 256 * 4) *(float4*)(lds_w + o) = *(const float4*)(wsrc + o);
        }
        const unsigned cso = (unsigned)(ch * KC) * 4u;
#pragma unroll
        for (int r0 = 0; r0 < NPA; r0 += 8) {
            u32x4 v[8];
#pragma unroll
            for (int j = 0; j < 8; ++j)
                if (r0 + j < NPA) v[j] = __builtin_amdgcn_raw_buffer_load_b128(xrs, aoff[r0 + j < NPA ? r0 + j : 0], cso, 0);
#pragma unroll
            for (int j = 0; j < 8; ++j)
                if (r0 + j < NPA) {
                    const int o = ldso[r0 + j < NPA ? r0 + j : 0];
                    if (o >= 0) {
                        float* d = lds_a + o;
                        const f32x4 f = __builtin_bit_cast(f32x4, v[j]);
                        d[0] = f[0]; d[1] = f[1]; d[2] = f[2]; d[3] = f[3];
                    }
                }
        }
        __syncthreads();
#pragma unroll
        for (int tap = 0; tap < TAPS; ++tap) {
            const int ky = tap / KS, kx = tap - ky * KS;
            const int toff = (ky * halo_w + kx) * PSF;
#pragma unroll
            for (int cs = 0; cs < CSTEPS; ++cs) {
                const int i = tap * CSTEPS + cs;
                float wa[NT], xb[PW];
#pragma unroll
                for (int tt = 0; tt < NT; ++tt) wa[tt] = lds_w[wlane + i * (4 * BN) + tt * 16];
#pragma unroll
                for (int p = 0; p < PW; ++p) xb[p] = lds_a[abase[p] + toff + cs * 4];
#pragma unroll
                for (int tt = 0; tt < NT; ++tt)
#pragma unroll
                    for (int p = 0; p < PW; ++p)
                        acc[tt][p] = __builtin_amdgcn_mfma_f32_16x16x4f32(wa[tt], xb[p], acc[tt][p], 0, 0, 0);
            }
        }
        __syncthreads();
    }

#pragma unroll
    for (int p = 0; p < PW; ++p) {
        const int s = wave * PW + p, row = s / WX, xb = s - row * WX;
        int n = n0, oy = oy0 + row;
        const int ox = ox0 + xb * 16 + lx;
        if (stack) { n = oy / Hs; oy -= n * Hs; }
        if (n >= a.N || oy >= a.Ho || ox >= a.Wo) continue;
        const size_t pidx = (size_t)(n * a.Ho + oy) * a.Wo + ox;
#pragma unroll
        for (int tt = 0; tt < NT; ++tt) {
            const int co = nb * BN + tt * 16 + q * 4;
            const float4 bv = *(const float4*)(a.bias + co);
            float v[4] = {acc[tt][p][0] + bv.x, acc[tt][p][1] + bv.y, acc[tt][p][2] + bv.z, acc[tt][p][3] + bv.w};
#pragma unroll
            for (int r = 0; r < 4; ++r) v[r] = d_act(v[r], a.pre_act);
            if (a.r1) {
                const float4 rv = *(const float4*)((const float*)a.r1 + pidx * a.r1cs + a.r1off + co);
                v[0] = rv.x + v[0]; v[1] = rv.y + v[1]; v[2] = rv.z + v[2]; v[3] = rv.w + v[3];
            }
            if (a.r2) {
                const float4 rv = *(const float4*)((const float*)a.r2 + pidx * a.r2cs + a.r2off + co);
                v[0] = v[0] + rv.x; v[1] = v[1] + rv.y; v[2] = v[2] + rv.z; v[3] = v[3] + rv.w;
            }
#pragma unroll
            for (int r = 0; r < 4; ++r) v[r] = d_act(v[r], a.post_act);
            if constexpr (EAGLE_F32_STORE_NT != 0) __builtin_nontemporal_store(f32x4{v[0], v[1], v[2], v[3]}, (f32x4*)((float*)a.y + pidx * a.ycs + a.yoff + co));
            else *(float4*)((float*)a.y + pidx * a.ycs + a.yoff + co) = make_float4(v[0], v[1], v[2], v[3]);
        }
    }
}

#endif
```

eagle_amd/csrc/elementwise.hip:

```cpp
#include <type_traits>
#include "common.h"
#include "dmath.h"

namespace eagle {

using half8 = __attribute__((ext_vector_type(8))) _Float16;

struct ResizeAxis { int s0, s1; int a0, a1; };

__device__ __forceinline__ ResizeAxis lin_coef(int d, int dsize, int ssize)
{
    const double scale = (double)ssize / (double)dsize;
    float f = (float)(((double)d + 0.5) * scale - 0.5);
    int s = (int)floorf(f);
    f -= (float)s;
    if (s < 0) { s = 0; f = 0.f; }
    if (s >= ssize - 1) { s = ssize - 1; f = 0.f; }
    ResizeAxis r;
    r.s0 = s; r.s1 = (s + 1 < ssize) ? s + 1 : s;
    r.a0 = (int)(short)lrintf((1.f - f) * 2048.f);
    r.a1 = (int)(short)lrintf(f * 2048.f);
    return r;
}

// ... 154 lines not shown
struct FuseArgs { TView base, y; TView z[3]; float sh[3], sw[3]; int n_up; int relu; unsigned* sat; };

constexpr int FUSE_ROWS = 8;
template <typename T, int NUP>
__global__ __launch_bounds__(256) void fuse_sum_kernel(FuseArgs a)
{
    constexpr int VN = Vec<T>::N;
    const int H = a.y.h, W = a.y.w, groups = a.y.c / VN;
    const unsigned col = blockIdx.y * 256u + threadIdx.x;
    if (col >= (unsigned)(W * groups)) return;
    const int hb = (H + FUSE_ROWS - 1) / FUSE_ROWS;
    const int band = gridDim.x >> 3, rb = (int)(blockIdx.x & 7) * band + (int)(blockIdx.x >> 3);
    if (rb >= a.y.n * hb) return;
    const int n = rb / hb, oy0 = (rb - n * hb) * FUSE_ROWS;
    const int ox = (int)(col / (unsigned)groups), g = (int)(col - (unsigned)ox * (unsigned)groups);
    constexpr int NU = NUP > 0 ? NUP : 1;
    Vec<T> p00[NU], p01[NU], p10[NU], p11[NU];
    float lx1[NU];
    int cy0[NU], cy1[NU];
    unsigned zc0[NU], zc1[NU];
#pragma unroll
    for (int j = 0; j < NUP; ++j) {
        const TView& z = a.z[j];
        const float fx = a.sw[j] * (float)ox;
        const int x0 = (int)fx, x1 = x0 + (x0 < z.w - 1 ? 1 : 0);
        lx1[j] = fx - (float)x0;
        const unsigned co = (unsigned)(z.off + g * VN);
        zc0[j] = (unsigned)x0 * (unsigned)z.cs + co; zc1[j] = (unsigned)x1 * (unsigned)z.cs + co;
        cy0[j] = -1; cy1[j] = -1;
    }
    for (int r = 0; r < FUSE_ROWS; ++r) {
        const int oy = oy0 + r;
        if (oy >= H) break;
        const unsigned pix = ((unsigned)n * H + (unsigned)oy) * (unsigned)W + (unsigned)ox;
        Vec<T> acc; acc.load(a.base.p, (size_t)pix * a.base.cs + a.base.off + g * VN);
        float ly1[NU];
#pragma unroll
        for (int j = 0; j < NUP; ++j) {
            const TView& z = a.z[j];
            const float fy = a.sh[j] * (float)oy;
            const int y0 = __builtin_amdgcn_readfirstlane((int)fy);
            const int y1 = y0 + (y0 < z.h - 1 ? 1 : 0);
            ly1[j] = fy - (float)y0;
            const unsigned b = (unsigned)n * z.h;
            if (y0 != cy0[j]) {
                if (y0 == cy1[j]) { p00[j] = p10[j]; p01[j] = p11[j]; }
                else {
                    const unsigned ro = (b + (unsigned)y0) * (unsigned)z.w * (unsigned)z.cs;
                    p00[j].load(z.p, (size_t)(ro + zc0[j])); p01[j].load(z.p, (size_t)(ro + zc1[j]));
                }
                cy0[j] = y0;
            }
            if (y1 != cy1[j]) {
                if (y1 == y0) { p10[j] = p00[j]; p11[j] = p01[j]; }
                else {
                    const unsigned ro = (b + (unsigned)y1) * (unsigned)z.w * (unsigned)z.cs;
                    p10[j].load(z.p, (size_t)(ro + zc0[j])); p11[j].load(z.p, (size_t)(ro + zc1[j]));
                }
                cy1[j] = y1;
            }
        }
#pragma unroll
        for (int j = 0; j < NUP; ++j) {
            const float ly0 = 1.0f - ly1[j], lx0 = 1.0f - lx1[j];
#pragma unroll
            for (int k = 0; k < VN; ++k) {
                const float top = fmaf(lx1[j], p01[j].v[k], lx0 * p00[j].v[k]);
                const float bot = fmaf(lx1[j], p11[j].v[k], lx0 * p10[j].v[k]);
                acc.v[k] = acc.v[k] + fmaf(ly1[j], bot, ly0 * top);
            }
        }
        if (a.relu)
#pragma unroll
            for (int k = 0; k < VN; ++k) acc.v[k] = acc.v[k] > 0.f ? acc.v[k] : 0.f;
        if constexpr (EAGLE_FUSE_NT && std::is_same<T, SplitT>::value) acc.store_nt(a.y.p, (size_t)pix * a.y.cs + a.y.off + g * VN);
        else acc.store(a.y.p, (size_t)pix * a.y.cs + a.y.off + g * VN);
        if constexpr (__is_same(T, SplitT)) {
            float m = 0.0f;
#pragma unroll
            for (int k = 0; k < VN; ++k) m = __builtin_fmaxf(m, __builtin_fabsf(acc.v[k]));
            if (a.sat != nullptr && m > 65504.0f) atomicAdd(a.sat + n, 1u);
        }
    }
}

static int ew_blocks(size_t total) { return (int)std::min<size_t>((total + 255) / 256, 256 * 16); }

void fuse_sum_launch(const TView& base, const FuseUp* ups, int n_up, int relu, const TView& y, hipStream_t s, unsigned* sat)
{
    FuseArgs a; a.base = base; a.y = y; a.n_up = n_up; a.relu = relu; a.sat = sat;
    for (int i = 0; i < n_up; ++i) {
        a.z[i] = ups[i].z;
        a.sh[i] = (y.h > 1) ? (float)(ups[i].z.h - 1) / (float)(y.h - 1) : 0.f;
        a.sw[i] = (y.w > 1) ? (float)(ups[i].z.w - 1) / (float)(y.w - 1) : 0.f;
    }
    const int vn = y.f32 == 1 ? 4 : 8;
    const size_t total = (size_t)y.n * y.h * y.w * (y.c / vn);
    size_t biggest = (size_t)y.n * y.h * y.w * std::max(y.cs, base.cs);
    for (int i = 0; i < n_up; ++i) biggest = std::max(biggest, (size_t)ups[i].z.n * ups[i].z.h * ups[i].z.w * ups[i].z.cs);
    if (biggest >= ((size_t)1 << 31)) fail(EAGLE_E_INVALID, "fuse: a tensor of %d frames reaches 2^31 elements; use a smaller device batch", y.n);
    (void)total;
    const dim3 grid((unsigned)((y.n * ((y.h + FUSE_ROWS - 1) / FUSE_ROWS) + 7) / 8 * 8), (unsigned)((y.w * (y.c / vn) + 255) / 256));
#define FUSE_LAUNCH(T_) \
    switch (n_up) { \
    case 0: hipLaunchKernelGGL((fuse_sum_kernel<T_, 0>), grid, dim3(256), 0, s, a); break; \
    case 1: hipLaunchKernelGGL((fuse_sum_kernel<T_, 1>), grid, dim3(256), 0, s, a); break; \
    case 2: hipLaunchKernelGGL((fuse_sum_kernel<T_, 2>), grid, dim3(256), 0, s, a); break; \
    default: hipLaunchKernelGGL((fuse_sum_kernel<T_, 3>), grid, dim3(256), 0, s, a); break; \
    }
    if (n_up > 3) fail(EAGLE_E_INVALID, "fuse: at most three low-resolution operands");
    if (y.f32 != base.f32) fail(EAGLE_E_INVALID, "fuse: operand formats differ");
    for (int i = 0; i < n_up; ++i) if (ups[i].z.f32 != y.f32) fail(EAGLE_E_INVALID, "fuse: operand formats differ");
    if (y.f32 == 1) { FUSE_LAUNCH(float) } else if (y.f32 == 2) { FUSE_LAUNCH(SplitT) } else { FUSE_LAUNCH(_Float16) }
#undef FUSE_LAUNCH
    HIP_CHECK(hipGetLastError());
}

template <typename T>
__global__ __launch_bounds__(256) void maxpool5_kernel(TView x, TView y)
{
    constexpr int VN = Vec<T>::N;
    const int H = x.h, W = x.w, groups = x.c / VN;
    const size_t total = (size_t)x.n * H * W * groups;
    for (size_t i = (size_t)blockIdx.x * blockDim.x + threadIdx.x; i < total; i += (size_t)gridDim.x * blockDim.x) {
        const int g = (int)(i % groups);
        const size_t pix = i / groups;
        const int ox = (int)(pix % W), oy = (int)((pix / W) % H), n = (int)(pix / ((size_t)W * H));
        Vec<T> m;
        for (int k = 0; k < VN; ++k) m.v[k] = -INFINITY;
        for (int dy = -2; dy <= 2; ++dy) {
            const int iy = oy + dy;
            if (iy < 0 || iy >= H) continue;
            for (int dx = -2; dx <= 2; ++dx) {
                const int ix = ox + dx;
                if (ix < 0 || ix >= W) continue;
                Vec<T> v; v.load(x.p, ((size_t)(n * H + iy) * W + ix) * x.cs + x.off + g * VN);
                for (int k = 0; k < VN; ++k) m.v[k] = v.v[k] > m.v[k] ? v.v[k] : m.v[k];
            }
        }
        m.store(y.p, pix * y.cs + y.off + g * VN);
    }
}
void maxpool5_launch(const TView& x, const TView& y, hipStream_t s)
{
    const int vn = x.f32 == 1 ? 4 : 8;
    const size_t total = (size_t)x.n * x.h * x.w * (x.c / vn);
    if (x.f32 == 1) hipLaunchKernelGGL(maxpool5_kernel<float>, dim3(ew_blocks(total)), dim3(256), 0, s, x, y);
    else if (x.f32 == 2) hipLaunchKernelGGL(maxpool5_kernel<SplitT>, dim3(ew_blocks(total)), dim3(256), 0, s, x, y);
    else hipLaunchKernelGGL(maxpool5_kernel<_Float16>, dim3(ew_blocks(total)), dim3(256), 0, s, x, y);
    HIP_CHECK(hipGetLastError());
}

template <typename T>
__global__ __launch_bounds__(256) void upsample2_kernel(TView x, TView y)
{
    constexpr int VN = Vec<T>::N;
    const int H = y.h, W = y.w, groups = x.c / VN;
    const size_t total = (size_t)y.n * H * W * groups;
    for (size_t i = (size_t)blockIdx.x * blockDim.x + threadIdx.x; i < total; i += (size_t)gridDim.x * blockDim.x) {
        const int g = (int)(i % groups);
        const size_t pix = i / groups;
        const int ox = (int)(pix % W), oy = (int)((pix / W) % H), n = (int)(pix / ((size_t)W * H));
        Vec<T> v; v.load(x.p, ((size_t)(n * x.h + oy / 2) * x.w + ox / 2) * x.cs + x.off + g * VN);
        v.store(y.p, pix * y.cs + y.off + g * VN);
    }
}
void upsample2_launch(const TView& x, const TView& y, hipStream_t s)
{
    const int vn = x.f32 == 1 ? 4 : 8;
    const size_t total = (size_t)y.n * y.h * y.w * (x.c / vn);
    if (x.f32 == 1) hipLaunchKernelGGL(upsample2_kernel<float>, dim3(ew_blocks(total)), dim3(256), 0, s, x, y);
    else if (x.f32 == 2) hipLaunchKernelGGL(upsample2_kernel<SplitT>, dim3(ew_blocks(total)), dim3(256), 0, s, x, y);
    else hipLaunchKernelGGL(upsample2_kernel<_Float16>, dim3(ew_blocks(total)), dim3(256), 0, s, x, y);
    HIP_CHECK(hipGetLastError());
}

__global__ __launch_bounds__(256) void split_to_f32_kernel(TView x, TView y)
{
    const int groups = x.c / 8;
    const size_t total = (size_t)x.n * x.h * x.w * groups;
    for (size_t i = (size_t)blockIdx.x * blockDim.x + threadIdx.x; i < total; i += (size_t)gridDim.x * blockDim.x) {
        const int g = (int)(i % groups);
        const size_t pix = i / groups;
        Vec<SplitT> v; v.load(x.p, pix * x.cs + x.off + g * 8);
        float* o = (float*)y.p + pix * y.cs + y.off + g * 8;
        *(float4*)o = make_float4(v.v[0] * 0.0625f, v.v[1] * 0.0625f, v.v[2] * 0.0625f, v.v[3] * 0.0625f);
        *(float4*)(o + 4) = make_float4(v.v[4] * 0.0625f, v.v[5] * 0.0625f, v.v[6] * 0.0625f, v.v[7] * 0.0625f);
    }
}
void split_to_f32_launch(const TView& x, const TView& y, hipStream_t s)
{
    const size_t total = (size_t)x.n * x.h * x.w * (x.c / 8);
    hipLaunchKernelGGL(split_to_f32_kernel, dim3(ew_blocks(total)), dim3(256), 0, s, x, y);
    HIP_CHECK(hipGetLastError());
}

__global__ __launch_bounds__(256) void heat_argmax_kernel(TView lg, ArgmaxPart* parts, int chunks)
{
    const int c = threadIdx.x & 63, pl = threadIdx.x >> 6;
    const int n = blockIdx.y, chunk = blockIdx.x;
    const int HW = lg.h * lg.w;
    const int per = (HW + chunks - 1) / chunks;
    const int p0 = chunk * per, p1 = min(HW, p0 + per);
    const float* base = (const float*)lg.p + (size_t)n * HW * lg.cs + lg.off + c;
    float best = -1.0f; int bi = 0x7fffffff;
    for (int p = p0 + pl; p < p1; p += 4) {
        const float sg = d_sigmoidf(base[(size_t)p * lg.cs]);
        if (sg > best) { best = sg; bi = p; }
    }
    __shared__ float sb[256];
    __shared__ int si[256];
    sb[threadIdx.x] = best; si[threadIdx.x] = bi;
    __syncthreads();
    if (pl == 0) {
        for (int k = 1; k < 4; ++k) {
            const float ob = sb[k * 64 + c]; const int oi = si[k * 64 + c];
            if (ob > best || (ob == best && oi < bi)) { best = ob; bi = oi; }
        }
        ArgmaxPart r; r.score = best; r.idx = bi;
        parts[((size_t)n * chunks + chunk) * 64 + c] = r;
    }
}
void heat_argmax_launch(const TView& logits, ArgmaxPart* parts, int chunks, hipStream_t s)
{
    hipLaunchKernelGGL(heat_argmax_kernel, dim3(chunks, logits.n), dim3(256), 0, s, logits, parts, chunks);
    HIP_CHECK(hipGetLastError());
}

}
```

eagle_amd/csrc/nets.hip:

```cpp
#include "runtime.h"

namespace eagle {

struct Builder {
    EagleHandle* H;
    Net* net;
    int prec;
    double bn_eps;
    int N;
    const char* label_suffix = "";
    int cur_stream = 0;
    void set_stream(int k) { cur_stream = k; net->pool = k; }
    void fork_join(Op::Kind kind, int nbranch) { Op op; op.kind = kind; op.nbranch = nbranch; op.tag = kind == Op::FORK ? "fork" : "join"; net->ops.push_back(op); }

    int gran() const { return prec == EAGLE_PREC_F32 ? 4 : 8; }

    TView act(int h, int w, int c, bool f32 = false)
    {
        TView v; v.n = N; v.h = h; v.w = w; v.c = c; v.cs = c; v.off = 0;
        v.f32 = (f32 || prec == EAGLE_PREC_F32) ? 1 : prec_tensor_fmt(prec);
        v.p = net->get((size_t)N * h * w * c * v.esize());
        return v;
    }
    void release(const TView& v) { net->put(v.p); }

    const HostTensor& W(const std::string& name)
    {
        auto it = H->weights.find(name);
        if (it == H->weights.end()) fail(EAGLE_E_MISSING, "weight tensor '%s' was not loaded", name.c_str());
        return it->second;
    }

    TView conv(const TView& x, const std::string& cname, const std::string& bn, int stride, int pre, const TView* r1,
               const TView* r2, int post, const TView* out = nullptr, bool out_f32 = false, ArgmaxPart* const* am_slot = nullptr)
    {
        std::vector<float> hwio, bias; int cin, cout, ks;
        fold(cname, bn, hwio, bias, cin, cout, ks);
        if (cin > x.c) fail(EAGLE_E_INVALID, "%s: input has %d channels, weight expects %d", cname.c_str(), x.c, cin);
        const int cout_pad = (cout + 15) / 16 * 16;
        bias.resize(cout_pad, 0.f);
        const int ho = (x.h + 2 * (ks / 2) - ks) / stride + 1, wo = (x.w + 2 * (ks / 2) - ks) / stride + 1;
        if (const char* dump = getenv("EAGLE_DUMP_LAYERS")) {
            if (FILE* f = fopen(dump, "a")) { fprintf(f, "%d,%d,%d,%d,%d,%d,%d\n", ks, stride, x.c, cout_pad, x.h, x.w, N); fclose(f); }
        }
        ConvLaunch L;
        L.cfg = conv_choose(prec, ks, stride, x.c, cout_pad, wo, pre == ACT_NONE && post <= ACT_RELU && !out_f32, r1 && r2);
        if (!conv_supported(prec, L.cfg))
            fail(EAGLE_E_NOKERNEL, "%s: no kernel instance (ks=%d s=%d kc=%d nt=%d)", cname.c_str(), ks, stride, L.cfg.kc, L.cfg.nt);
        const size_t ne = conv_weight_elems(prec, L.cfg);
        std::vector<char> tiled(ne * (prec == EAGLE_PREC_F32 ? 4 : 2));
        conv_tile_weights(prec, L.cfg, hwio.data(), cin, cout, tiled.data(), &L.descale);
        L.w = net->upload(tiled.data(), tiled.size());
        L.bias = (const float*)net->upload(bias.data(), bias.size() * 4);
        L.x = x;
        if (out) {
            L.y = *out;
            if (out->c != cout_pad || out->h != ho || out->w != wo) fail(EAGLE_E_INVALID, "%s: output slice mismatch", cname.c_str());
        } else {
            L.y = act(ho, wo, cout_pad, out_f32);
        }
        if (r1) L.r1 = *r1;
        if (r2) L.r2 = *r2;
        L.pre_act = pre; L.post_act = post; L.out_f32 = out_f32 ? 1 : 0;
        refuse_2gib(cname, "layer", {&L.x, &L.y, r1 ? &L.r1 : nullptr, r2 ? &L.r2 : nullptr});
        L.am_slot = am_slot;
        if (prec == EAGLE_PREC_F32S && !out_f32 && !am_slot) L.sat_slot = &H->cur_sat;
        if (am_slot) { H->hm_chunks = conv_tiles_per_frame(prec, L.cfg, ho, wo); H->fused_argmax = true; }
        L.flop = 2.0 * N * ho * wo * (double)cout * cin * ks * ks;
        const int pr = prec;
        char label[64];
        snprintf(label, sizeof(label), "conv %dx%d/%d %d->%d @%dx%d v%d%s", ks, ks, stride, cin, cout, ho, wo, L.cfg.variant, label_suffix);
        const double es = prec == EAGLE_PREC_F16 ? 2 : 4;
        emit_conv(label, L.flop, (double)N * x.h * x.w * cin * es + (double)N * ho * wo * cout * ((out_f32 || prec != EAGLE_PREC_F16) ? 4 : 2) * (am_slot ? 0 : 1) +
                                 (r1 ? (double)N * ho * wo * cout * es : 0) + (r2 ? (double)N * ho * wo * cout * es : 0) + (double)ks * ks * cin * cout * es,
                  [L, pr](hipStream_t s) { conv_launch(pr, L, s); });
        return L.y;
    }
    void fold(const std::string& cname, const std::string& bn, std::vector<float>& hwio, std::vector<float>& bias, int& cin, int& cout, int& ks)
    {
        const HostTensor& w = W(cname + ".weight");
        if (w.shape.size() != 4) fail(EAGLE_E_INVALID, "%s.weight: expected 4-d", cname.c_str());
        cout = (int)w.shape[0]; cin = (int)w.shape[1]; ks = (int)w.shape[2];
        hwio.assign((size_t)ks * ks * cin * cout, 0.f); bias.assign(cout, 0.f);
        std::vector<double> scale(cout, 1.0);
        if (!bn.empty()) {
            const HostTensor &g = W(bn + ".weight"), &b = W(bn + ".bias"), &m = W(bn + ".running_mean"), &v = W(bn + ".running_var");
            for (int o = 0; o < cout; ++o) {
                scale[o] = (double)g.data[o] / std::sqrt((double)v.data[o] + bn_eps);
                bias[o] = (float)((double)b.data[o] - (double)m.data[o] * scale[o]);
            }
        } else if (H->weights.count(cname + ".bias")) {
            const HostTensor& b = W(cname + ".bias");
            for (int o = 0; o < cout; ++o) bias[o] = b.data[o];
        }
        for (int o = 0; o < cout; ++o)
            for (int i = 0; i < cin; ++i)
                for (int t = 0; t < ks * ks; ++t) {
                    const float wv = w.data[((size_t)o * cin + i) * ks * ks + t];
                    hwio[((size_t)t * cin + i) * cout + o] = bn.empty() ? wv : (float)((double)wv * scale[o]);
                }
    }
    void refuse_2gib(const std::string& name, const char* what, std::initializer_list<const TView*> ts)
    {
        for (const TView* t : ts)
            if (t && (size_t)t->n * t->h * t->w * t->cs * t->esize() >= ((size_t)1 << 31))
                fail(EAGLE_E_INVALID, "%s: a %d x %d x %d x %d-channel tensor of this %s reaches 2 GiB at a device batch of %d frames (32-bit tensor offsets); use a smaller EagleConfig.batch",
                     name.c_str(), t->n, t->h, t->w, t->cs, what, N);
    }
    void emit_conv(const char* label, double flop, double bytes, std::function<void(hipStream_t)> run)
    {
        net->names.emplace_back(new std::string(label));
        Op op; op.kind = Op::CONV; op.flop = flop; op.bytes = bytes; op.tag = net->names.back()->c_str(); op.stream = cur_stream; op.run = std::move(run);
        net->ops.push_back(op);
    }
    TView bottleneck(const TView& x, const std::string& q, const TView& res, const std::string& ds_conv = "", const std::string& ds_bn = "")
    {
        BneckLaunch L;
        const bool dsf = !ds_conv.empty();
        std::vector<float> hw, bs; int ci, co, ks;
        std::vector<_Float16> img;
        double flop = 0;
        const char* cn[3] = {"conv1", "conv2", "conv3"}; const char* bnn[3] = {"bn1", "bn2", "bn3"};
        const int want_ks[3] = {1, 3, 1}, want_ci[3] = {x.c, 64, 64}, want_co[3] = {64, 64, 256};
        for (int k = 0; k < 3; ++k) {
            fold(q + cn[k], q + bnn[k], hw, bs, ci, co, ks);
            if (ks != want_ks[k] || ci != want_ci[k] || co != want_co[k]) fail(EAGLE_E_INVALID, "%s%s: not the Bottleneck shape of the fused kernel", q.c_str(), cn[k]);
            if (k == 2 && dsf) {
                std::vector<float> hwd, bd; int cid, cod, ksd;
                fold(ds_conv, ds_bn, hwd, bd, cid, cod, ksd);
                if (ksd != 1 || cid != 64 || cod != 256 || x.c != 64) fail(EAGLE_E_INVALID, "%s: not the 1x1 64->256 downsample of the fused kernel", ds_conv.c_str());
                hw.insert(hw.end(), hwd.begin(), hwd.end());
                for (int o = 0; o < 256; ++o) bs[o] = bs[o] + bd[o];
                ci = 128;
                flop += 2.0 * N * x.h * x.w * 256.0 * 64;
            }
            float ds = 1.f;
            bneck_tile_weights(hw.data(), ks * ks, ci, co, img, &ds);
            bneck_scale_bias(bs, ds);
            const void* dw = net->upload(img.data(), img.size() * 2);
            const float* db = (const float*)net->upload(bs.data(), bs.size() * 4);
            if (k == 0) { L.w1 = dw; L.b1 = db; L.ds1 = ds; } else if (k == 1) { L.w2 = dw; L.b2 = db; L.ds2 = ds; } else { L.w3 = dw; L.b3 = db; L.ds3 = ds; }
            flop += 2.0 * N * x.h * x.w * (double)co * (k == 2 ? 64 : ci) * ks * ks;
        }
        L.x = x; L.y = act(x.h, x.w, 256); L.res = dsf ? L.y : res; L.ds_fused = dsf;
        L.sat_slot = &H->cur_sat;
        refuse_2gib(q, "block", {&L.x, &L.y, &L.res});
        char label[64];
        snprintf(label, sizeof(label), "bneck %d->64->256%s @%dx%d%s", x.c, dsf ? "+ds" : "", x.h, x.w, label_suffix);
        emit_conv(label, flop, (double)N * x.h * x.w * 4.0 * (x.c + 256 + ((dsf || res.p == x.p) ? 0 : 256)) + 4.0 * (x.c * 64 + 9 * 64 * 64 + 64 * 256 + (dsf ? 64 * 256 : 0)),
                  [L](hipStream_t s) { bneck_launch(L, s); });
        return L.y;
    }
    static double vbytes(const TView& v) { return (double)v.n * v.h * v.w * v.c * (v.f32 ? 4 : 2); }
    void other(std::function<void(hipStream_t)> fn, const char* tag, double bytes = 0)
    {
        Op op; op.kind = Op::OTHER; op.run = std::move(fn); op.tag = tag; op.stream = cur_stream; op.bytes = bytes;
        net->ops.push_back(op);
    }
};

static const char* HRP = "unnormalized_model.0.";

static std::vector<TView> hr_stage(Builder& B, std::vector<TView> xs, int stage_idx, int n_modules, int nb, bool last_single)
{
    const int R = ACT_RELU;
    for (int m = 0; m < n_modules; ++m) {
        const std::string q = std::string(HRP) + "stage" + std::to_string(stage_idx) + "." + std::to_string(m) + ".";
        B.fork_join(Op::FORK, nb - 1);
        const bool interleave = !(getenv("EAGLE_HR_INTERLEAVE") && atoi(getenv("EAGLE_HR_INTERLEAVE")) == 0);
        for (int step = 0; step < 4 * nb; ++step) {
            const int k = interleave ? step / nb : step % 4, b = interleave ? nb - 1 - step % nb : step / 4;
            B.set_stream(b);
            TView x = xs[b];
            const std::string r = q + "branches." + std::to_string(b) + "." + std::to_string(k) + ".";
            TView o = B.conv(x, r + "conv1", r + "bn1", 1, 0, nullptr, nullptr, R);
            TView y = B.conv(o, r + "conv2", r + "bn2", 1, 0, &x, nullptr, R);
            B.release(o);
            B.release(x);
            xs[b] = y;
        }
        B.set_stream(0);
        B.fork_join(Op::JOIN, nb - 1);
        const int n_out = (last_single && m == n_modules - 1) ? 1 : nb;
        std::vector<TView> out;
        if (n_out > 1) B.fork_join(Op::FORK, n_out - 1);
        for (int i = 0; i < n_out; ++i) {
            B.set_stream(n_out > 1 ? i : 0);
            TView y; bool have_y = false;
            for (int j = 0; j < i; ++j) {
                TView t = xs[j];
                for (int k = 0; k < i - j; ++k) {
                    const std::string r = q + "fuse_layers." + std::to_string(i) + "." + std::to_string(j) + "." + std::to_string(k) + ".";
                    const bool last = k == i - j - 1;
                    TView nt;
                    if (!last) {
                        nt = B.conv(t, r + "0", r + "1", 2, 0, nullptr, nullptr, R);
                    } else {
                        const TView* ident = (j == i - 1) ? &xs[i] : nullptr;
                        const bool relu_now = ident && i == nb - 1;
                        nt = B.conv(t, r + "0", r + "1", 2, 0, have_y ? &y : nullptr, ident, relu_now ? R : 0);
                    }
                    if (k > 0) B.release(t);
                    t = nt;
                }
                if (have_y) B.release(y);
                y = t; have_y = true;
            }
            if (i == 0) y = xs[0];
            FuseUp ups[3]; int nu = 0;
            for (int j = i + 1; j < nb; ++j) {
                const std::string r = q + "fuse_layers." + std::to_string(i) + "." + std::to_string(j) + ".";
                ups[nu++].z = B.conv(xs[j], r + "0", r + "1", 1, 0, nullptr, nullptr, 0);
            }
            if (nu) {
                TView o = B.act(y.h, y.w, y.c);
                const TView base = y; FuseUp u0 = ups[0], u1 = ups[1], u2 = ups[2]; const int n_up = nu;
                EagleHandle* const Hh = B.H;
                B.other([base, u0, u1, u2, n_up, o, Hh](hipStream_t s) { FuseUp u[3] = {u0, u1, u2}; fuse_sum_launch(base, u, n_up, 1, o, s, Hh->cur_sat); }, "fuse_sum",
                        Builder::vbytes(base) + Builder::vbytes(o) + (nu > 0 ? Builder::vbytes(ups[0].z) : 0) + (nu > 1 ? Builder::vbytes(ups[1].z) : 0) + (nu > 2 ? Builder::vbytes(ups[2].z) : 0));
                for (int k = 0; k < nu; ++k) B.release(ups[k].z);
                if (i != 0) B.release(y);
                y = o;
            }
            out.push_back(y);
        }
        B.set_stream(0);
        if (n_out > 1) B.fork_join(Op::JOIN, n_out - 1);
        for (int b = 0; b < nb; ++b) B.release(xs[b]);
        xs = out;
    }
    return xs;
}

static TView build_hrnet(Builder& B, const TView& x_in)
{
    const int R = ACT_RELU;
    const std::string P = HRP;
    TView x = B.conv(x_in, P + "conv1", P + "bn1", 2, 0, nullptr, nullptr, R);
    TView x2 = B.conv(x, P + "conv2", P + "bn2", 2, 0, nullptr, nullptr, R);
    B.release(x); x = x2;
    for (int b = 0; b < 4; ++b) {
        const std::string q = P + "layer1." + std::to_string(b) + ".";
        const char* fe = getenv("EAGLE_BNECK_FUSED");
        const char* de = getenv("EAGLE_BNECK_DS");
        const bool fused = B.prec == EAGLE_PREC_F32S && !(fe && atoi(fe) == 0) && bneck_supported(x, 64, 256);
        const bool dsf = fused && b == 0 && x.c == 64 && !(de && atoi(de) == 0);
        TView res = x;
        if (b == 0 && !dsf) res = B.conv(x, q + "downsample.0", q + "downsample.1", 1, 0, nullptr, nullptr, 0);
        if (fused) {
            TView y = dsf ? B.bottleneck(x, q, x, q + "downsample.0", q + "downsample.1") : B.bottleneck(x, q, res);
            if (b == 0 && !dsf) B.release(res);
            B.release(x);
            x = y;
            continue;
        }
        TView o1 = B.conv(x, q + "conv1", q + "bn1", 1, 0, nullptr, nullptr, R);
        TView o2 = B.conv(o1, q + "conv2", q + "bn2", 1, 0, nullptr, nullptr, R);
        TView y = B.conv(o2, q + "conv3", q + "bn3", 1, 0, &res, nullptr, R);
        B.release(o1); B.release(o2);
        if (b == 0) B.release(res);
        B.release(x);
        x = y;
    }
    std::vector<TView> ys(2);
    B.fork_join(Op::FORK, 1);
    B.set_stream(1);
    ys[1] = B.conv(x, P + "transition1.1.0.0", P + "transition1.1.0.1", 2, 0, nullptr, nullptr, R);
    B.set_stream(0);
    ys[0] = B.conv(x, P + "transition1.0.0", P + "transition1.0.1", 1, 0, nullptr, nullptr, R);
    B.fork_join(Op::JOIN, 1);
    B.release(x);
    ys = hr_stage(B, ys, 2, 1, 2, false);
    ys.push_back(B.conv(ys.back(), P + "transition2.2.0.0", P + "transition2.2.0.1", 2, 0, nullptr, nullptr, R));
    ys = hr_stage(B, ys, 3, 4, 3, false);
    ys.push_back(B.conv(ys.back(), P + "transition3.3.0.0", P + "transition3.3.0.1", 2, 0, nullptr, nullptr, R));
    ys = hr_stage(B, ys, 4, 3, 4, true);
    ArgmaxPart* const* am = (prec_is_f16_kernels(B.prec) && !getenv("EAGLE_NO_FUSED_ARGMAX")) ? &B.H->cur_parts : nullptr;
    TView logits = B.conv(ys[0], "unnormalized_model.1", "", 1, 0, nullptr, nullptr, 0, nullptr, true, am);
    B.release(ys[0]);
    return logits;
}

struct YoloDims { int c[5]; int n[4]; };
static YoloDims yolo_dims(int variant)
{
    static const double D[5] = {0.33, 0.33, 0.67, 1.0, 1.0}, Wd[5] = {0.25, 0.5, 0.75, 1.0, 1.25};
    static const int MC[5] = {1024, 1024, 768, 512, 512};
    YoloDims y;
    const int base[5] = {64, 128, 256, 512, 1024};
    for (int i = 0; i < 5; ++i) y.c[i] = (int)std::ceil(std::min(base[i], MC[variant]) * Wd[variant] / 8.0) * 8;
    const int rep[4] = {3, 6, 6, 3};
    for (int i = 0; i < 4; ++i) y.n[i] = std::max((int)std::nearbyint(rep[i] * D[variant]), 1);
    return y;
}

struct YoloBuilder {
    Builder& B;
    int S = ACT_SILU;
    TView cv(const TView& x, const std::string& name, int stride = 1, const TView* r1 = nullptr, const TView* out = nullptr)
    {
        return B.conv(x, name + ".conv", name + ".bn", stride, S, r1, nullptr, 0, out);
    }
    TView c2f(const TView& x, int idx, int cout, int n, bool shortcut, const TView* out = nullptr)
    {
        const std::string p = "model." + std::to_string(idx);
        const int c = cout / 2;
        TView cat = B.act(x.h, x.w, (2 + n) * c);
        TView first = cat.slice(0, 2 * c);
        cv(x, p + ".cv1", 1, nullptr, &first);
        for (int k = 0; k < n; ++k) {
            TView in = cat.slice((1 + k) * c, c);
            TView t = cv(in, p + ".m." + std::to_string(k) + ".cv1");
            TView o = cat.slice((2 + k) * c, c);
            cv(t, p + ".m." + std::to_string(k) + ".cv2", 1, shortcut ? &in : nullptr, &o);
            B.release(t);
        }
        TView y = cv(cat, p + ".cv2", 1, nullptr, out);
        B.release(cat);
        return y;
    }
};

static void build_yolo(Builder& B, const TView& x_in, int variant, DetLevel lv[3], int nc, bool mixed = false)
{
    YoloBuilder Y{B};
    const YoloDims d = yolo_dims(variant);
    const int c1 = d.c[0], c2 = d.c[1], c3 = d.c[2], c4 = d.c[3], c5 = d.c[4];
    TView x0 = Y.cv(x_in, "model.0", 2);
    TView x1 = Y.cv(x0, "model.1", 2); B.release(x0);
    TView x2 = Y.c2f(x1, 2, c2, d.n[0], true); B.release(x1);
    TView x3 = Y.cv(x2, "model.3", 2); B.release(x2);
    const int h3 = x3.h, w3 = x3.w;
    const int h4 = (h3 - 1) / 2 + 1, w4 = (w3 - 1) / 2 + 1, h5 = (h4 - 1) / 2 + 1, w5 = (w4 - 1) / 2 + 1;
    TView cat15 = B.act(h3, w3, c4 + c3);
    TView cat12 = B.act(h4, w4, c5 + c4);
    TView cat18 = B.act(h4, w4, c3 + c4);
    TView cat21 = B.act(h5, w5, c4 + c5);
    TView p3 = cat15.slice(c4, c3), p4 = cat12.slice(c5, c4), p5 = cat21.slice(c4, c5), h12 = cat18.slice(c3, c4);
    Y.c2f(x3, 4, c3, d.n[1], true, &p3); B.release(x3);
    TView x5 = Y.cv(p3, "model.5", 2);
    Y.c2f(x5, 6, c4, d.n[2], true, &p4); B.release(x5);
    TView x7 = Y.cv(p4, "model.7", 2);
    TView x8 = Y.c2f(x7, 8, c5, d.n[3], true); B.release(x7);
    {
        const int ch = c5 / 2;
        TView cat = B.act(h5, w5, 4 * ch);
        TView s0 = cat.slice(0, ch), s1 = cat.slice(ch, ch), s2 = cat.slice(2 * ch, ch), s3 = cat.slice(3 * ch, ch);
        Y.cv(x8, "model.9.cv1", 1, nullptr, &s0); B.release(x8);
        B.other([s0, s1](hipStream_t s) { maxpool5_launch(s0, s1, s); }, "maxpool5", 2 * Builder::vbytes(s0));
        B.other([s1, s2](hipStream_t s) { maxpool5_launch(s1, s2, s); }, "maxpool5", 2 * Builder::vbytes(s0));
        B.other([s2, s3](hipStream_t s) { maxpool5_launch(s2, s3, s); }, "maxpool5", 2 * Builder::vbytes(s0));
        Y.cv(cat, "model.9.cv2", 1, nullptr, &p5);
        B.release(cat);
    }
    {
        TView u = cat12.slice(0, c5);
        B.other([p5, u](hipStream_t s) { upsample2_launch(p5, u, s); }, "upsample2", Builder::vbytes(p5) + Builder::vbytes(u));
        Y.c2f(cat12, 12, c4, d.n[0], false, &h12);
    }
    TView h15, h18, h21;
    {
        TView u = cat15.slice(0, c4);
        B.other([h12, u](hipStream_t s) { upsample2_launch(h12, u, s); }, "upsample2", Builder::vbytes(h12) + Builder::vbytes(u));
    }
    if (!mixed) {
        h15 = Y.c2f(cat15, 15, c3, d.n[0], false);
        {
            TView o = cat18.slice(0, c3);
            Y.cv(h15, "model.16", 2, nullptr, &o);
        }
        h18 = Y.c2f(cat18, 18, c4, d.n[0], false);
        {
            TView o = cat21.slice(0, c4);
            Y.cv(h18, "model.19", 2, nullptr, &o);
        }
        h21 = Y.c2f(cat21, 21, c5, d.n[0], false);
    } else {
        B.prec = EAGLE_PREC_F32;
        auto to_f32 = [&B](const TView& x, const TView& y) {
            B.other([x, y](hipStream_t s) { split_to_f32_launch(x, y, s); }, "split_to_f32", Builder::vbytes(x) + Builder::vbytes(y));
        };
        TView cat15f = B.act(h3, w3, c4 + c3), cat18f = B.act(h4, w4, c3 + c4), cat21f = B.act(h5, w5, c4 + c5);
        to_f32(cat15, cat15f);
        h15 = Y.c2f(cat15f, 15, c3, d.n[0], false);
        {
            TView o = cat18f.slice(0, c3);
            Y.cv(h15, "model.16", 2, nullptr, &o);
            to_f32(h12, cat18f.slice(c3, c4));
        }
        h18 = Y.c2f(cat18f, 18, c4, d.n[0], false);
        {
            TView o = cat21f.slice(0, c4);
            Y.cv(h18, "model.19", 2, nullptr, &o);
            to_f32(p5, cat21f.slice(c4, c5));
        }
        h21 = Y.c2f(cat21f, 21, c5, d.n[0], false);
    }
    const TView feats[3] = {h15, h18, h21};
    const float strides[3] = {8.f, 16.f, 32.f};
    int a0 = 0;
    for (int l = 0; l < 3; ++l) {
        const std::string pb = "model.22.cv2." + std::to_string(l), pc = "model.22.cv3." + std::to_string(l);
        TView b0 = Y.cv(feats[l], pb + ".0");
        TView b1 = Y.cv(b0, pb + ".1"); B.release(b0);
        TView box = B.conv(b1, pb + ".2", "", 1, 0, nullptr, nullptr, 0, nullptr, true); B.release(b1);
        TView k0 = Y.cv(feats[l], pc + ".0");
        TView k1 = Y.cv(k0, pc + ".1"); B.release(k0);
        TView cls = B.conv(k1, pc + ".2", "", 1, 0, nullptr, nullptr, 0, nullptr, true); B.release(k1);
        lv[l].box = box; lv[l].cls = cls; lv[l].gh = box.h; lv[l].gw = box.w; lv[l].stride = strides[l]; lv[l].a0 = a0;
        a0 += box.h * box.w;
    }
    (void)c1; (void)nc;
}

static const char* RP = "reid.";

struct ReidFold { std::vector<float> scale, shift; };
static ReidFold reid_bn(Builder& B, const std::string& bn, int c)
{
    const HostTensor &g = B.W(bn + ".weight"), &b = B.W(bn + ".bias"), &m = B.W(bn + ".running_mean"), &v = B.W(bn + ".running_var");
    ReidFold f; f.scale.resize(c); f.shift.resize(c);
    for (int o = 0; o < c; ++o) {
        const double sc = (double)g.data[o] / std::sqrt((double)v.data[o] + 1e-5);
        f.scale[o] = (float)sc; f.shift[o] = (float)((double)b.data[o] - (double)m.data[o] * sc);
    }
    return f;
}

static TView reid_light(Builder& B, const TView& x, const std::string& lc, int mid)
{
    TView t = B.conv(x, lc + ".conv1", "", 1, 0, nullptr, nullptr, 0);
    const HostTensor& w = B.W(lc + ".conv2.weight");
    const ReidFold f = reid_bn(B, lc + ".bn", mid);
    const int C = t.c;
    std::vector<float> wk((size_t)9 * C, 0.f), bk(C, 0.f);
    for (int c = 0; c < mid; ++c) {
        for (int k = 0; k < 9; ++k) wk[(size_t)k * C + c] = (float)((double)w.data[(size_t)c * 9 + k] * (double)f.scale[c]);
        bk[c] = f.shift[c];
    }
    const float* dw = (const float*)B.net->upload(wk.data(), wk.size() * 4);
    const float* db = (const float*)B.net->upload(bk.data(), bk.size() * 4);
    TView y = B.act(t.h, t.w, C);
    const int n = B.N;
    B.other([t, dw, db, y, n](hipStream_t s) { reid_dw3_launch(t, dw, db, y, n, s); }, "reid dw3x3", 2 * Builder::vbytes(y));
    B.release(t);
    return y;
}

static TView reid_osblock(Builder& B, const TView& x, const std::string& b, int cin, int cout)
{
    const int mid = cout / 4, R = ACT_RELU;
    TView x1 = B.conv(x, b + ".conv1.conv", b + ".conv1.bn", 1, 0, nullptr, nullptr, R);
    TView st[4];
    st[0] = reid_light(B, x1, b + ".conv2a", mid);
    const char* names[3] = {"b", "c", "d"};
    for (int k = 0; k < 3; ++k) {
        TView y = x1;
        for (int d = 0; d < k + 2; ++d) {
            TView nx = reid_light(B, y, b + ".conv2" + names[k] + "." + std::to_string(d), mid);
            if (d > 0) B.release(y);
            y = nx;
        }
        st[k + 1] = y;
    }
    B.release(x1);
    const HostTensor &w1 = B.W(b + ".gate.fc1.weight"), &b1 = B.W(b + ".gate.fc1.bias"), &w2 = B.W(b + ".gate.fc2.weight"), &b2 = B.W(b + ".gate.fc2.bias");
    const int r = (int)w1.shape[0];
    const float* d1 = (const float*)B.net->upload(w1.data.data(), w1.data.size() * 4);
    const float* e1 = (const float*)B.net->upload(b1.data.data(), b1.data.size() * 4);
    const float* d2 = (const float*)B.net->upload(w2.data.data(), w2.data.size() * 4);
    const float* e2 = (const float*)B.net->upload(b2.data.data(), b2.data.size() * 4);
    const int C = st[0].c, n = B.N;
    float* g = (float*)B.net->get((size_t)n * 4 * C * 4);
    TView x2 = B.act(st[0].h, st[0].w, C);
    const TView s0 = st[0], s1 = st[1], s2 = st[2], s3 = st[3];
    B.other([s0, s1, s2, s3, d1, e1, d2, e2, mid, r, g, x2, n](hipStream_t s) { const TView ss[4] = {s0, s1, s2, s3}; reid_gate_launch(ss, d1, e1, d2, e2, mid, r, g, x2, n, s); },
            "reid gate", 5 * Builder::vbytes(x2));
    for (auto& t : st) B.release(t);
    TView ident = x;
    if (cin != cout) ident = B.conv(x, b + ".downsample.conv", b + ".downsample.bn", 1, 0, nullptr, nullptr, 0);
    TView y = B.conv(x2, b + ".conv3.conv", b + ".conv3.bn", 1, 0, &ident, nullptr, R);
    B.release(x2);
    if (cin != cout) B.release(ident);
    return y;
}

static void build_reid(Builder& B, EagleHandle* h)
{
    const std::string P = RP;
    const int n = B.N;
    h->reid_in = B.act(256, 128, 4);
    const HostTensor& w1 = B.W(P + "conv1.conv.weight");
    const ReidFold f1 = reid_bn(B, P + "conv1.bn", 16);
    std::vector<float> wk(7 * 7 * 3 * 16), bk(16);
    for (int o = 0; o < 16; ++o) {
        for (int c = 0; c < 3; ++c)
            for (int k = 0; k < 49; ++k) wk[(size_t)(k * 3 + c) * 16 + o] = (float)((double)w1.data[((size_t)o * 3 + c) * 49 + k] * (double)f1.scale[o]);
        bk[o] = f1.shift[o];
    }
    const float* dw = (const float*)B.net->upload(wk.data(), wk.size() * 4);
    const float* db = (const float*)B.net->upload(bk.data(), bk.size() * 4);
    TView c1 = B.act(128, 64, 16);
    const TView in = h->reid_in;
    B.other([in, dw, db, c1, n](hipStream_t s) { reid_conv7_launch(in, dw, db, c1, n, s); }, "reid conv7x7", Builder::vbytes(in) + Builder::vbytes(c1));
    TView x = B.act(64, 32, 16);
    B.other([c1, x, n](hipStream_t s) { reid_maxpool3s2_launch(c1, x, n, s); }, "reid maxpool", Builder::vbytes(c1) + Builder::vbytes(x));
    B.release(c1);
    static const int CH[4] = {16, 64, 96, 128};
    const char* stage[3] = {"conv2", "conv3", "conv4"};
    for (int sI = 0; sI < 3; ++sI) {
        const int cin = CH[sI], cout = CH[sI + 1];
        const std::string sp = P + stage[sI];
        TView y = reid_osblock(B, x, sp + ".0", cin, cout); B.release(x); x = y;
        y = reid_osblock(B, x, sp + ".1", cout, cout); B.release(x); x = y;
        if (sI < 2) {
            TView t = B.conv(x, sp + ".2.0.conv", sp + ".2.0.bn", 1, 0, nullptr, nullptr, ACT_RELU); B.release(x);
            TView p = B.act(t.h / 2, t.w / 2, t.c);
            B.other([t, p, n](hipStream_t s) { reid_avgpool2_launch(t, p, n, s); }, "reid avgpool", Builder::vbytes(t) + Builder::vbytes(p));
            B.release(t);
            x = p;
        }
    }
    TView c5 = B.conv(x, P + "conv5.conv", P + "conv5.bn", 1, 0, nullptr, nullptr, ACT_RELU); B.release(x);
    const HostTensor &fw = B.W(P + "fc.0.weight"), &fb = B.W(P + "fc.0.bias");
    const ReidFold ff = reid_bn(B, P + "fc.1", EAGLE_REID_DIM);
    std::vector<float> hw((size_t)EAGLE_REID_DIM * c5.c, 0.f), hb(EAGLE_REID_DIM);
    for (int o = 0; o < EAGLE_REID_DIM; ++o) {
        for (int c = 0; c < 128; ++c) hw[(size_t)o * c5.c + c] = (float)((double)fw.data[(size_t)o * 128 + c] * (double)ff.scale[o]);
        hb[o] = (float)((double)fb.data[o] * (double)ff.scale[o] + (double)ff.shift[o]);
    }
    const float* dhw = (const float*)B.net->upload(hw.data(), hw.size() * 4);
    const float* dhb = (const float*)B.net->upload(hb.data(), hb.size() * 4);
    h->reid_feats = (float*)B.net->get((size_t)n * EAGLE_REID_DIM * 4);
    float* feats = h->reid_feats;
    B.other([c5, dhw, dhb, feats, n](hipStream_t s) { reid_head_launch(c5, dhw, dhb, feats, EAGLE_REID_DIM, n, s); }, "reid head", Builder::vbytes(c5));
    h->reid_crops = (EagleCrop*)B.net->get(sizeof(EagleCrop) * (size_t)n);
    HIP_CHECK(hipHostMalloc((void**)&h->reid_crops_h, sizeof(EagleCrop) * (size_t)n, hipHostMallocDefault));
    HIP_CHECK(hipHostMalloc((void**)&h->reid_feats_h, sizeof(float) * EAGLE_REID_DIM * (size_t)n, hipHostMallocDefault));
}

void finalize(EagleHandle* h)
{
    const EagleConfig& c = h->cfg;
    const int B = c.batch;
    h->prec = c.precision;
    const bool det_mixed = c.det_precision == EAGLE_DET_PREC_MIXED;
    h->det_prec = det_mixed ? EAGLE_PREC_F32S : c.det_precision ? c.det_precision - 1 : c.precision;
    h->hr.reset(new Net); h->yo.reset(new Net); h->misc.reset(new Net);
    const int cin_pad = h->prec == EAGLE_PREC_F32 ? 4 : 8, det_cin_pad = h->det_prec == EAGLE_PREC_F32 ? 4 : 8;
    h->lb = letterbox_geometry(c.frame_h, c.frame_w, c.det_imgsz, c.letterbox);
    Builder Bh{h, h->hr.get(), h->prec, 1e-5, B};
    Builder By{h, h->yo.get(), h->det_prec, 1e-3, B};
    By.label_suffix = " d";
    h->kp_in = Bh.act(540, 960, cin_pad);
    h->det_in = By.act(h->lb.out_h, h->lb.out_w, det_cin_pad);
    h->logits = build_hrnet(Bh, h->kp_in);
    build_yolo(By, h->det_in, c.det_variant, h->levels, 5, det_mixed);
    if (h->weights.count(std::string(RP) + "conv1.conv.weight")) {
        h->reid.reset(new Net);
        Builder Br{h, h->reid.get(), EAGLE_PREC_F32, 1e-5, REID_NB};
        build_reid(Br, h);
// ... 40 lines not shown
```

eagle_amd/csrc/ops_api.hip:

```cpp
#include "runtime.h"

extern "C" {

static void to_dev(Net& net, int prec, const float* src, int n, int h, int w, int c, int cpad, TView& v)
{
    v.n = n; v.h = h; v.w = w; v.c = cpad; v.cs = cpad; v.off = 0; v.f32 = prec_tensor_fmt(prec);
    const size_t px = (size_t)n * h * w;
    if (v.f32 == 2) {
        std::vector<_Float16> t(px * cpad * 2, (_Float16)0.f);
        for (size_t p = 0; p < px; ++p)
            for (int k = 0; k < c; ++k) {
                const float sv = src[p * c + k] * 16.0f;
                const _Float16 hi = (_Float16)sv;
                t[p * cpad * 2 + (k / 8) * 16 + (k % 8)] = hi;
                t[p * cpad * 2 + (k / 8) * 16 + 8 + (k % 8)] = (_Float16)(sv - (float)hi);
            }
        v.p = net.upload(t.data(), t.size() * 2);
    } else if (v.f32) {
        std::vector<float> t(px * cpad, 0.f);
        for (size_t p = 0; p < px; ++p) for (int k = 0; k < c; ++k) t[p * cpad + k] = src[p * c + k];
        v.p = net.upload(t.data(), t.size() * 4);
    } else {
        std::vector<_Float16> t(px * cpad, (_Float16)0.f);
        for (size_t p = 0; p < px; ++p) for (int k = 0; k < c; ++k) t[p * cpad + k] = (_Float16)src[p * c + k];
        v.p = net.upload(t.data(), t.size() * 2);
    }
}
static void from_dev(const TView& v, int c, float* dst)
{
    const size_t px = (size_t)v.n * v.h * v.w;
    if (v.f32 == 2) {
        std::vector<_Float16> t(px * v.cs * 2);
        HIP_CHECK(hipMemcpy(t.data(), v.p, t.size() * 2, hipMemcpyDeviceToHost));
        for (size_t p = 0; p < px; ++p)
            for (int k = 0; k < c; ++k) {
                const size_t e = p * v.cs * 2 + (size_t)((v.off + k) / 8) * 16 + (v.off + k) % 8;
                dst[p * c + k] = ((float)t[e] + (float)t[e + 8]) * 0.0625f;
            }
    } else if (v.f32) {
        std::vector<float> t(px * v.cs);
        HIP_CHECK(hipMemcpy(t.data(), v.p, t.size() * 4, hipMemcpyDeviceToHost));
        for (size_t p = 0; p < px; ++p) for (int k = 0; k < c; ++k) dst[p * c + k] = t[p * v.cs + v.off + k];
    } else {
        std::vector<_Float16> t(px * v.cs);
        HIP_CHECK(hipMemcpy(t.data(), v.p, t.size() * 2, hipMemcpyDeviceToHost));
        for (size_t p = 0; p < px; ++p) for (int k = 0; k < c; ++k) dst[p * c + k] = (float)t[p * v.cs + v.off + k];
    }
}

int eagle_op_conv2d(int device, int precision, const float* x, int n, int h, int w, int cin, const float* w_hwio,
                    const float* bias, int cout, int ks, int stride, int pre_act, const float* r1, const float* r2,
                    int post_act, float* y)
{
    EagleHandle* hh = nullptr;
    API_BEGIN
    HIP_CHECK(hipSetDevice(device));
    Net net;
    const int g = precision == EAGLE_PREC_F32 ? 4 : 8;
    const int cin_pad = cin <= g ? g : (cin + 15) / 16 * 16, cout_pad = (cout + 15) / 16 * 16;
    const int ho = (h + 2 * (ks / 2) - ks) / stride + 1, wo = (w + 2 * (ks / 2) - ks) / stride + 1;
    ConvLaunch L;
    to_dev(net, precision, x, n, h, w, cin, cin_pad, L.x);
    L.cfg = conv_choose(precision, ks, stride, cin_pad, cout_pad, wo, pre_act == ACT_NONE && post_act <= ACT_RELU, r1 && r2);
    if (!conv_supported(precision, L.cfg)) fail(EAGLE_E_NOKERNEL, "no kernel instance ks=%d s=%d kc=%d nt=%d", ks, stride, L.cfg.kc, L.cfg.nt);
    std::vector<char> tiled(conv_weight_elems(precision, L.cfg) * (precision == EAGLE_PREC_F32 ? 4 : 2));
    conv_tile_weights(precision, L.cfg, w_hwio, cin, cout, tiled.data(), &L.descale);
    L.w = net.upload(tiled.data(), tiled.size());
    std::vector<float> b(cout_pad, 0.f);
    for (int i = 0; i < cout; ++i) b[i] = bias[i];
    L.bias = (const float*)net.upload(b.data(), b.size() * 4);
    L.y.n = n; L.y.h = ho; L.y.w = wo; L.y.c = cout_pad; L.y.cs = cout_pad; L.y.f32 = prec_tensor_fmt(precision);
    L.y.p = net.get((size_t)n * ho * wo * cout_pad * L.y.esize());
    if (r1) to_dev(net, precision, r1, n, ho, wo, cout, cout_pad, L.r1);
    if (r2) to_dev(net, precision, r2, n, ho, wo, cout, cout_pad, L.r2);
    L.pre_act = pre_act; L.post_act = post_act;
    conv_launch(precision, L, nullptr);
    HIP_CHECK(hipDeviceSynchronize());
    from_dev(L.y, cout, y);
    API_END(hh)
}

int eagle_op_bottleneck(int device, const float* x, int n, int h, int w, int cin, const float* w1, const float* b1, const float* w2, const float* b2,
                        const float* w3, const float* b3, const float* res, float* y, int reps, float* ms, const float* wd, const float* bd)
{
    EagleHandle* hh = nullptr;
    API_BEGIN
    HIP_CHECK(hipSetDevice(device));
    if (!x || !w1 || !b1 || !w2 || !b2 || !w3 || !b3 || !y || n < 1 || h < 1 || w < 1 || cin % 16 || cin < 16) fail(EAGLE_E_INVALID, "eagle_op_bottleneck: bad argument (Cin must be a multiple of 16)");
    if ((wd != nullptr) != (bd != nullptr) || (wd && (res || cin != 64))) fail(EAGLE_E_INVALID, "eagle_op_bottleneck: the in-kernel downsample branch takes (wd, bd) together, Cin = 64 and no residual tensor");
    if (!res && !wd && cin != 256) fail(EAGLE_E_INVALID, "eagle_op_bottleneck: an identity shortcut needs Cin = 256");
    Net net;
    BneckLaunch L;
    to_dev(net, EAGLE_PREC_F32S, x, n, h, w, cin, cin, L.x);
    if (res) to_dev(net, EAGLE_PREC_F32S, res, n, h, w, 256, 256, L.res); else L.res = L.x;
    L.y = L.x; L.y.c = L.y.cs = 256; L.y.off = 0; L.y.p = net.get((size_t)n * h * w * 256 * 4);
    if (wd) L.res = L.y;
    std::vector<_Float16> img;
    bneck_tile_weights(w1, 1, cin, 64, img, &L.ds1); L.w1 = net.upload(img.data(), img.size() * 2);
    bneck_tile_weights(w2, 9, 64, 64, img, &L.ds2); L.w2 = net.upload(img.data(), img.size() * 2);
    std::vector<float> w3x(w3, w3 + 64 * 256), sb3(b3, b3 + 256);
    if (wd) {
        w3x.insert(w3x.end(), wd, wd + 64 * 256);
        for (int o = 0; o < 256; ++o) sb3[o] = sb3[o] + bd[o];
        L.ds_fused = true;
    }
    bneck_tile_weights(w3x.data(), 1, wd ? 128 : 64, 256, img, &L.ds3); L.w3 = net.upload(img.data(), img.size() * 2);
    std::vector<float> sb1(b1, b1 + 64), sb2(b2, b2 + 64);
    bneck_scale_bias(sb1, L.ds1); bneck_scale_bias(sb2, L.ds2); bneck_scale_bias(sb3, L.ds3);
    L.b1 = (const float*)net.upload(sb1.data(), 64 * 4); L.b2 = (const float*)net.upload(sb2.data(), 64 * 4); L.b3 = (const float*)net.upload(sb3.data(), 256 * 4);
    if (getenv("EAGLE_BNECK_TIMING")) L.dbg = (unsigned long long*)net.get(8192 * 8 * 8);
    unsigned* op_sat = nullptr; unsigned* const* op_sat_slot = &op_sat;
    if (getenv("EAGLE_BNECK_OPSAT")) { op_sat = (unsigned*)net.get(sizeof(unsigned) * (size_t)n); L.sat_slot = op_sat_slot; }
    bneck_launch(L, nullptr);
    HIP_CHECK(hipDeviceSynchronize());
    if (L.dbg) {
        std::vector<unsigned long long> t(8192 * 8);
        HIP_CHECK(hipMemcpy(t.data(), L.dbg, t.size() * 8, hipMemcpyDeviceToHost));
        double sum[8] = {0}; int nw = 0;
        for (int b = 0; b < 8192; ++b) { bool any = false; for (int k = 0; k < 8; ++k) { sum[k] += (double)t[b * 8 + k]; any |= t[b * 8 + k] != 0; } nw += any; }
        if (nw) fprintf(stderr, "[bneck timing] %d workgroups, mean us per workgroup: phase1 %.1f  wait %.1f  epi1 %.1f  phase2 %.1f  epi2 %.1f  phase3 %.1f\n", nw,
                        sum[0] / nw / 100, sum[1] / nw / 100, sum[2] / nw / 100, sum[3] / nw / 100, sum[4] / nw / 100, sum[5] / nw / 100);
    }
    if (reps > 0 && ms) {
        hipEvent_t e0, e1;
        HIP_CHECK(hipEventCreate(&e0)); HIP_CHECK(hipEventCreate(&e1));
        HIP_CHECK(hipEventRecord(e0, nullptr));
        for (int i = 0; i < reps; ++i) bneck_launch(L, nullptr);
        HIP_CHECK(hipEventRecord(e1, nullptr));
        HIP_CHECK(hipEventSynchronize(e1));
        HIP_CHECK(hipEventElapsedTime(ms, e0, e1));
        *ms /= (float)reps;
        (void)hipEventDestroy(e0); (void)hipEventDestroy(e1);
    }
    from_dev(L.y, 256, y);
    API_END(hh)
}

int eagle_op_fuse_sum(int device, int precision, const float* base, int n, int H, int W, int c, int n_up,
                      const float* const* ups, const int* up_h, const int* up_w, int relu, float* y)
{
    EagleHandle* hh = nullptr;
    API_BEGIN
    HIP_CHECK(hipSetDevice(device));
    if (n_up > 3 || c % 8) fail(EAGLE_E_INVALID, "fuse_sum: n_up <= 3 and c %% 8 == 0 required");
    Net net;
    TView b, o;
    to_dev(net, precision, base, n, H, W, c, c, b);
    FuseUp u[3];
    for (int i = 0; i < n_up; ++i) to_dev(net, precision, ups[i], n, up_h[i], up_w[i], c, c, u[i].z);
    o = b; o.p = net.get((size_t)n * H * W * c * b.esize());
    fuse_sum_launch(b, u, n_up, relu, o, nullptr);
    HIP_CHECK(hipDeviceSynchronize());
    from_dev(o, c, y);
    API_END(hh)
}

int eagle_op_preprocess(int device, int precision, const uint8_t* bgr, int n, int h, int w, int det_imgsz,
                        float* kp_out, float* det_out, int* det_hw)
{
    return eagle_op_preprocess_lb(device, precision, bgr, n, h, w, det_imgsz, EAGLE_LETTERBOX_RECT, kp_out, det_out, det_hw);
}

int eagle_op_preprocess_lb(int device, int precision, const uint8_t* bgr, int n, int h, int w, int det_imgsz, int letterbox,
                           float* kp_out, float* det_out, int* det_hw)
{
    EagleHandle* hh = nullptr;
    API_BEGIN
    HIP_CHECK(hipSetDevice(device));
    Net net;
    const int cp = precision == EAGLE_PREC_F32 ? 4 : 8;
    const LetterBox lb = letterbox_geometry(h, w, det_imgsz, letterbox);
    det_hw[0] = lb.out_h; det_hw[1] = lb.out_w;
    if (!kp_out || !det_out) return EAGLE_OK;
    uint8_t* d = (uint8_t*)net.upload(bgr, (size_t)n * h * w * 3);
    TView kp, det;
    kp.n = n; kp.h = 540; kp.w = 960; kp.c = kp.cs = cp; kp.f32 = prec_tensor_fmt(precision);
    det = kp; det.h = lb.out_h; det.w = lb.out_w;
    kp.p = net.get((size_t)n * 540 * 960 * cp * kp.esize());
    det.p = net.get((size_t)n * lb.out_h * lb.out_w * cp * det.esize());
    preprocess_launch(precision, d, n, h, w, kp, det, lb, nullptr);
    HIP_CHECK(hipDeviceSynchronize());
    from_dev(kp, 3, kp_out);
    from_dev(det, 3, det_out);
    API_END(hh)
}

int eagle_op_find_homography(int device, const float* img_pts, const float* world_pts, int n, double thresh,
                             int max_iters, int lm_iters, double* H9, uint8_t* mask, int* ok)
{
    EagleHandle* hh = nullptr;
    API_BEGIN
    HIP_CHECK(hipSetDevice(device));
    if (n < 0 || n > EAGLE_MAX_KP) fail(EAGLE_E_INVALID, "0 <= n <= %d required", EAGLE_MAX_KP);
    Net net;
    float* di = (float*)net.upload(img_pts, sizeof(float) * 2 * std::max(n, 1));
    float* dw = (float*)net.upload(world_pts, sizeof(float) * 2 * std::max(n, 1));
    double* dH = (double*)net.get(72);
    uint8_t* dm = (uint8_t*)net.get(256);
    int* dok = (int*)net.get(16);
    homography_only_launch(di, dw, n, thresh, max_iters, lm_iters, dH, dm, dok, nullptr);
    HIP_CHECK(hipDeviceSynchronize());
    HIP_CHECK(hipMemcpy(H9, dH, 72, hipMemcpyDeviceToHost));
    if (n > 0) HIP_CHECK(hipMemcpy(mask, dm, n, hipMemcpyDeviceToHost));
    HIP_CHECK(hipMemcpy(ok, dok, sizeof(int), hipMemcpyDeviceToHost));
    API_END(hh)
}

}
```

eagle_amd/lib.py:

```python
import ctypes as C
import os

import numpy as np

_HERE = os.path.dirname(os.path.abspath(__file__))
LIB_PATH = os.environ.get("EAGLE_HIP_LIB") or os.path.join(_HERE, "libeagle_hip.so")

MAX_DET, N_LANDMARKS, MAX_KP = 300, 57, 87
PREC_F16, PREC_F32, PREC_F32S = 0, 1, 2
PRECISIONS = {"f16": PREC_F16, "f32": PREC_F32, "f32s": PREC_F32S}
DET_VARIANTS = {"n": 0, "s": 1, "m": 2, "l": 3, "x": 4}
AUTO, SMALL_BATCH = -1, 32
LETTERBOX = {"rect": 0, "square": 1}
DET_PREC_AUTO = -1
DET_PREC_MIXED = 4


class EagleError(RuntimeError):
    pass


class EagleRangeError(EagleError):
    records = None


class EagleConfig(C.Structure):
    _fields_ = [("device", C.c_int32), ("frame_h", C.c_int32), ("frame_w", C.c_int32), ("det_variant", C.c_int32),
                ("det_imgsz", C.c_int32), ("batch", C.c_int32), ("precision", C.c_int32),
                ("keypoint_conf", C.c_double), ("detector_conf", C.c_double), ("ransac_thresh", C.c_double),
                ("detector_floor", C.c_float), ("nms_iou", C.c_float),
                ("ransac_max_iters", C.c_int32), ("lm_iters", C.c_int32), ("use_graph", C.c_int32), ("det_precision", C.c_int32),
                ("allow_saturation", C.c_int32), ("multi_stream", C.c_int32), ("letterbox", C.c_int32), ("reserved", C.c_int32 * 3)]


class EagleTimings(C.Structure):
    _fields_ = [("total_ms", C.c_float), ("conv_ms", C.c_float), ("n_launches", C.c_int32),
                ("n_conv_launches", C.c_int32), ("conv_flop", C.c_double), ("sat_events", C.c_int32), ("sat_frames", C.c_int32),
                ("graph_captures", C.c_int32), ("graph_skipped", C.c_int32), ("reserved", C.c_int32 * 4)]


class EagleTrackParams(C.Structure):
    _fields_ = [("track_high_thresh", C.c_float), ("track_low_thresh", C.c_float), ("new_track_thresh", C.c_float), ("match_thresh", C.c_float),
                ("track_buffer", C.c_int32), ("frame_rate", C.c_int32)]


class EagleYuvLayout(C.Structure):
    _fields_ = [("frame_stride", C.c_int64), ("y_pitch", C.c_int64), ("c_offset", C.c_int64), ("c_pitch", C.c_int64), ("v_offset", C.c_int64)]


PIX_FORMATS = {"nv12": 1, "i420": 2}


class EagleKernelTime(C.Structure):
    _fields_ = [("name", C.c_char * 40), ("ms", C.c_float), ("launches", C.c_int32), ("bytes", C.c_double), ("flop", C.c_double)]


DET_DTYPE = np.dtype([("x1", "<f4"), ("y1", "<f4"), ("x2", "<f4"), ("y2", "<f4"), ("conf", "<f4"), ("cls", "<i4"),
                      ("id", "<i4"), ("bx1", "<i4"), ("by1", "<i4"), ("bx2", "<i4"), ("by2", "<i4"),
                      ("foot_x", "<i4"), ("foot_y", "<i4"), ("pitch_xf", "<f4"), ("pitch_yf", "<f4"),
                      ("pitch_x", "<i4"), ("pitch_y", "<i4"), ("reported", "u1"), ("in_bounds", "u1"), ("pad", "u1", 2)],
                     align=True)
KP_DTYPE = np.dtype([("label", "<i4"), ("x", "<i4"), ("y", "<i4"), ("score", "<f4"), ("synthesized", "u1"),
                     ("on_plane", "u1"), ("inlier", "u1"), ("pad", "u1")], align=True)
RESULT_DTYPE = np.dtype([("n_det", "<i4"), ("n_kp", "<i4"), ("n_candidates", "<i4"), ("H_valid", "u1"),
                         ("bounds_valid", "u1"), ("pad", "u1", 2), ("H", "<f8", 9), ("bounds", "<f8", 4),
                         ("hm_idx", "<i4", N_LANDMARKS), ("hm_score", "<f4", N_LANDMARKS),
                         ("kp", KP_DTYPE, MAX_KP), ("det", DET_DTYPE, MAX_DET)], align=True)

_lib = None


def require_torch_first():
    import sys
    if "torch" not in sys.modules and _lib is not None:
        raise EagleError("torch must be imported before eagle_amd.lib loads libeagle_hip.so in a process that uses both "
                         "(two ROCm runtimes would be mapped: torch's bundled one and /opt/rocm's); import torch first, or keep the process torch-free")


def load():
    global _lib
    if _lib is not None:
        return _lib
    if not os.path.exists(LIB_PATH):
        raise EagleError(f"{LIB_PATH} not found: run `python -c 'import __graft_entry__ as g; g.build()'` "
                         "(there is no CPU fallback for the product path)")
    L = C.CDLL(LIB_PATH)
    vp, i32, i64 = C.c_void_p, C.c_int, C.c_int64
    fp, dp, u8p = C.POINTER(C.c_float), C.POINTER(C.c_double), C.POINTER(C.c_uint8)
    L.eagle_abi_sizes.argtypes = [C.POINTER(C.c_int32)]
    L.eagle_default_config.argtypes = [C.POINTER(EagleConfig)]
    L.eagle_create.argtypes = [C.POINTER(EagleConfig), C.POINTER(vp)]
    L.eagle_destroy.argtypes = [vp]
    L.eagle_destroy.restype = None
    L.eagle_last_error.argtypes = [vp]
    L.eagle_last_error.restype = C.c_char_p
    L.eagle_get_config.argtypes = [vp, C.POINTER(EagleConfig)]
    L.eagle_resolve_config.argtypes = [C.POINTER(EagleConfig)]
    L.eagle_load_weights.argtypes = [vp, C.c_char_p, fp, C.POINTER(i64), i32]
    L.eagle_finalize_weights.argtypes = [vp]
    L.eagle_process_frames.argtypes = [vp, u8p, i32, i64, i64, vp]
    L.eagle_process_device_frames.argtypes = [vp, vp, i32, vp]
    L.eagle_host_alloc.argtypes = [vp, i64, C.POINTER(vp)]
    L.eagle_host_free.argtypes = [vp, vp]
    L.eagle_device_alloc.argtypes = [vp, i64, C.POINTER(vp)]
    L.eagle_device_free.argtypes = [vp, vp]
    L.eagle_device_upload.argtypes = [vp, vp, vp, i64]
    L.eagle_reproject.argtypes = [vp, vp, i32, dp, u8p]
    L.eagle_clip_open.argtypes = [vp, vp, i32]
    L.eagle_clip_close.argtypes = [vp]
    L.eagle_clip_detect_keypoints.argtypes = [vp, i32, i32, i32]
    L.eagle_clip_get_keypoints.argtypes = [vp, i32, vp, C.POINTER(i32)]
    L.eagle_clip_set_keypoints.argtypes = [vp, i32, vp, i32]
    L.eagle_clip_flow.argtypes = [vp, i32, i32, i32, vp, i32, vp, C.POINTER(i32), fp, u8p]
    L.eagle_clip_run.argtypes = [vp, i32, i32, i32, i32, i32, i32, C.POINTER(i32)]
    L.eagle_clip_detect_objects.argtypes = [vp, i32, i32]
    L.eagle_clip_fetch.argtypes = [vp, vp]
    L.eagle_comm_id.argtypes = [vp]
    L.eagle_comm_init.argtypes = [vp, i32, i32, vp]
    L.eagle_gather.argtypes = [vp, vp, i32, vp]
    L.eagle_set_profiling.argtypes = [vp, i32]
    L.eagle_get_timings.argtypes = [vp, C.POINTER(EagleTimings)]
    L.eagle_get_kernel_times.argtypes = [vp, C.POINTER(EagleKernelTime), i32, C.POINTER(i32)]
    L.eagle_op_conv2d.argtypes = [i32, i32, fp, i32, i32, i32, i32, fp, fp, i32, i32, i32, i32, fp, fp, i32, fp]
    L.eagle_op_bottleneck.argtypes = [i32, fp, i32, i32, i32, i32, fp, fp, fp, fp, fp, fp, fp, fp, i32, fp, fp, fp]
    L.eagle_op_fuse_sum.argtypes = [i32, i32, fp, i32, i32, i32, i32, i32, C.POINTER(fp), C.POINTER(i32), C.POINTER(i32), i32, fp]
    L.eagle_op_preprocess.argtypes = [i32, i32, u8p, i32, i32, i32, i32, fp, fp, C.POINTER(i32)]
    L.eagle_op_preprocess_lb.argtypes = [i32, i32, u8p, i32, i32, i32, i32, i32, fp, fp, C.POINTER(i32)]
    L.eagle_op_find_homography.argtypes = [i32, fp, fp, i32, C.c_double, i32, i32, dp, u8p, C.POINTER(i32)]
    L.eagle_debug.argtypes = [C.c_char_p, i64, vp, i64]
    L.eagle_team_colors.argtypes = [vp, vp, i32, vp, i32, vp]
    L.eagle_track_open.argtypes = [vp, C.POINTER(EagleTrackParams)]
    L.eagle_track_frames.argtypes = [vp, vp, i32]
    L.eagle_track_frames_cmc.argtypes = [vp, vp, i32, C.POINTER(C.c_double)]
    L.eagle_clip_motion.argtypes = [vp, i32, i32, C.POINTER(C.c_double)]
    L.eagle_clip_motion_ecc.argtypes = [vp, i32, i32, i32, C.POINTER(C.c_double), C.POINTER(i32)]
    L.eagle_reid_features.argtypes = [vp, vp, i32, vp, i32, fp]
    yl = C.POINTER(EagleYuvLayout)
    L.eagle_process_frames_yuv.argtypes = [vp, i32, u8p, i32, yl, vp]
    L.eagle_process_device_frames_yuv.argtypes = [vp, i32, vp, i32, yl, vp]
    L.eagle_yuv_to_bgr.argtypes = [vp, i32, vp, i32, yl, vp]
    L.eagle_op_yuv_to_bgr.argtypes = [i32, i32, u8p, i32, i32, i32, yl, u8p]
    L.eagle_track_frames_reid.argtypes = [vp, vp, i32, C.POINTER(C.c_double), fp, C.POINTER(i32), C.POINTER(i32)]
    _lib = L
    return L


EXPORTS = ["eagle_abi_sizes", "eagle_default_config", "eagle_create", "eagle_destroy", "eagle_last_error", "eagle_get_config", "eagle_resolve_config", "eagle_load_weights",
           "eagle_finalize_weights", "eagle_process_frames", "eagle_process_device_frames", "eagle_device_alloc",
           "eagle_device_free", "eagle_device_upload", "eagle_host_alloc", "eagle_host_free", "eagle_reproject", "eagle_comm_id", "eagle_comm_init", "eagle_gather",
           "eagle_set_profiling", "eagle_get_timings", "eagle_get_kernel_times", "eagle_op_conv2d", "eagle_op_bottleneck", "eagle_op_fuse_sum", "eagle_op_preprocess", "eagle_op_preprocess_lb",
           "eagle_op_find_homography", "eagle_clip_open", "eagle_clip_close", "eagle_clip_detect_objects", "eagle_clip_detect_keypoints", "eagle_clip_get_keypoints",
           "eagle_clip_set_keypoints", "eagle_clip_flow", "eagle_clip_run", "eagle_clip_fetch", "eagle_debug", "eagle_track_open", "eagle_track_frames", "eagle_track_frames_cmc", "eagle_clip_motion_ecc", "eagle_clip_motion", "eagle_team_colors",
           "eagle_reid_features", "eagle_track_frames_reid", "eagle_process_frames_yuv", "eagle_process_device_frames_yuv", "eagle_yuv_to_bgr",
           "eagle_op_yuv_to_bgr"]

FLOWKP_DTYPE = np.dtype([("label", "<i4"), ("x", "<i4"), ("y", "<i4"), ("score", "<f4")], align=True)
E_REFERENCE_RAISES = -7
E_RANGE = -8


def debug(key, value=0, out=None):
    rc = load().eagle_debug(key.encode(), int(value), None if out is None else out.ctypes.data_as(C.c_void_p), 0 if out is None else out.nbytes)
    if rc:
        raise EagleError(f"eagle_debug({key}) failed ({rc})")
    return out


def resolve_config(cfg):
    out = EagleConfig.from_buffer_copy(cfg)
    if load().eagle_resolve_config(C.byref(out)):
        raise EagleError("eagle_resolve_config failed")
    return out


def abi_sizes():
    o = (C.c_int32 * 4)()
    load().eagle_abi_sizes(o)
    return list(o)


def _fp(a):
    return a.ctypes.data_as(C.POINTER(C.c_float)) if a is not None else None


def default_config(**kw):
    cfg = EagleConfig()
    load().eagle_default_config(C.byref(cfg))
    for k, v in kw.items():
        if k == "det_variant" and isinstance(v, str):
            v = DET_VARIANTS[v]
        if k == "letterbox" and isinstance(v, str):
            v = LETTERBOX[v]
        if not hasattr(cfg, k):
            raise TypeError(f"unknown config field {k}")
        setattr(cfg, k, v)
    return cfg


class Handle:

    def __init__(self, cfg=None, **kw):
        self.L = load()
        self.cfg = cfg or default_config(**kw)
        self._h = C.c_void_p()
        rc = self.L.eagle_create(C.byref(self.cfg), C.byref(self._h))
        if rc:
            raise EagleError(f"eagle_create failed ({rc}): {self.L.eagle_last_error(None).decode()}")
        resolved = EagleConfig()
        self._check(self.L.eagle_get_config(self._h, C.byref(resolved)), "get_config")
        self.cfg = resolved

    def _check(self, rc, what):
        if rc == E_RANGE:
            raise EagleRangeError(f"{what}: {self.L.eagle_last_error(self._h).decode()}")
        if rc:
            raise EagleError(f"{what} failed ({rc}): {self.L.eagle_last_error(self._h).decode()}")

    def _check_records(self, rc, what, out):
        try:
            self._check(rc, what)
        except EagleRangeError as e:
            e.records = out
            raise

    def close(self):
        if self._h:
            self.L.eagle_destroy(self._h)
            self._h = C.c_void_p()

    def __del__(self):
        try:
            self.close()
        except Exception:
            pass

    def load_weight(self, name, arr):
        arr = np.ascontiguousarray(arr, np.float32)
        shape = (C.c_int64 * max(arr.ndim, 1))(*arr.shape)
        self._check(self.L.eagle_load_weights(self._h, name.encode(), _fp(arr), shape, arr.ndim), f"load_weights({name})")

    def finalize_weights(self):
        self._check(self.L.eagle_finalize_weights(self._h), "finalize_weights")

    def process(self, frames, out=None, strides=None):
        frames = np.asarray(frames)
        if frames.dtype != np.uint8:
            frames = frames.astype(np.uint8)
        if frames.ndim == 3:
            frames = frames[None]
        n, h, w, c = frames.shape
        if (h, w, c) != (self.cfg.frame_h, self.cfg.frame_w, 3):
            raise EagleError(f"frame shape {(h, w, c)} does not match the handle ({self.cfg.frame_h}, {self.cfg.frame_w}, 3)")
        fs, rs, ps, cs = frames.strides
        if n == 1:
            fs = max(fs, rs * (h - 1) + 3 * w)
        if not (cs == 1 and ps == 3 and rs >= 3 * w and fs >= rs * (h - 1) + 3 * w):
            frames = np.ascontiguousarray(frames)
            fs, rs = h * w * 3, w * 3
        if strides is not None:
            fs, rs = strides
        if out is None:
            out = np.zeros(n, RESULT_DTYPE)
        assert out.dtype == RESULT_DTYPE and len(out) >= n and out.flags.c_contiguous
        self._check_records(self.L.eagle_process_frames(self._h, C.cast(frames.ctypes.data, C.POINTER(C.c_uint8)), n, int(fs), int(rs),
                                                        out.ctypes.data_as(C.c_void_p)), "process_frames", out)
        return out

    def host_frames(self, n):
        shape = (n, self.cfg.frame_h, self.cfg.frame_w, 3)
        nbytes = int(np.prod(shape))
        p = C.c_void_p()
        self._check(self.L.eagle_host_alloc(self._h, nbytes, C.byref(p)), "host_alloc")
        buf = (C.c_uint8 * max(nbytes, 1)).from_address(p.value)
        a = np.frombuffer(buf, np.uint8, nbytes).reshape(shape)
        self._pinned = getattr(self, "_pinned", {})
        self._pinned[a.ctypes.data] = p
        return a

    def host_buffer(self, nbytes):
        p = C.c_void_p()
        self._check(self.L.eagle_host_alloc(self._h, int(nbytes), C.byref(p)), "host_alloc")
        a = np.frombuffer((C.c_uint8 * max(int(nbytes), 1)).from_address(p.value), np.uint8, int(nbytes))
        self._pinned = getattr(self, "_pinned", {})
        self._pinned[a.ctypes.data] = p
        return a

    def host_free(self, a):
        p = self._pinned.pop(a.ctypes.data)
        self._check(self.L.eagle_host_free(self._h, p), "host_free")

    def upload(self, frames):
        frames = np.ascontiguousarray(frames, np.uint8)
        d = C.c_void_p()
        self._check(self.L.eagle_device_alloc(self._h, frames.nbytes, C.byref(d)), "device_alloc")
        self._check(self.L.eagle_device_upload(self._h, d, frames.ctypes.data_as(C.c_void_p), frames.nbytes), "device_upload")
        return d

    def free(self, d):
        self._check(self.L.eagle_device_free(self._h, d), "device_free")

    def process_device(self, dptr, n, out=None):
        if out is None:
            out = np.zeros(n, RESULT_DTYPE)
        self._check_records(self.L.eagle_process_device_frames(self._h, dptr, n, out.ctypes.data_as(C.c_void_p)), "process_device_frames", out)
        return out

    def _yuv_frames(self, frames, fmt, layout, n):
# ... 61 lines not shown

    def reproject(self, recs, Hs, flags):
        Hs = np.ascontiguousarray(Hs, np.float64).reshape(-1, 9)
        flags = np.ascontiguousarray(flags, np.uint8)
        assert recs.flags.c_contiguous and len(Hs) == len(flags) == len(recs)
        self._check(self.L.eagle_reproject(self._h, recs.ctypes.data_as(C.c_void_p), len(recs), Hs.ctypes.data_as(C.POINTER(C.c_double)),
                                           flags.ctypes.data_as(C.POINTER(C.c_uint8))), "reproject")
        return recs

    def clip_open(self, dptr, n):
        self._check(self.L.eagle_clip_open(self._h, dptr, n), "clip_open")

    def clip_close(self):
        self._check(self.L.eagle_clip_close(self._h), "clip_close")

    def clip_detect_objects(self, first, count):
        self._check(self.L.eagle_clip_detect_objects(self._h, first, count), "clip_detect_objects")

    def clip_detect_keypoints(self, first, stride=1, count=1):
        self._check(self.L.eagle_clip_detect_keypoints(self._h, first, stride, count), "clip_detect_keypoints")

    def clip_get_keypoints(self, frame):
        buf = np.zeros(N_LANDMARKS, FLOWKP_DTYPE); n = C.c_int(0)
        self._check(self.L.eagle_clip_get_keypoints(self._h, frame, buf.ctypes.data_as(C.c_void_p), C.byref(n)), "clip_get_keypoints")
        return None if n.value < 0 else buf[: n.value].copy()

    def clip_set_keypoints(self, frame, kps):
        kps = np.ascontiguousarray(kps, FLOWKP_DTYPE)
        self._check(self.L.eagle_clip_set_keypoints(self._h, frame, kps.ctypes.data_as(C.c_void_p), len(kps)), "clip_set_keypoints")

    def clip_flow(self, src_frame, dst_frame, hue_frame, kps, raw=False):
        kps = np.ascontiguousarray(kps, FLOWKP_DTYPE)
        out = np.zeros(N_LANDMARKS, FLOWKP_DTYPE); n = C.c_int(0)
        nxt = np.zeros((max(len(kps), 1), 2), np.float32); st = np.zeros(max(len(kps), 1), np.uint8)
        self._check(self.L.eagle_clip_flow(self._h, src_frame, dst_frame, hue_frame, kps.ctypes.data_as(C.c_void_p), len(kps),
                                           out.ctypes.data_as(C.c_void_p), C.byref(n), _fp(nxt), st.ctypes.data_as(C.POINTER(C.c_uint8))), "clip_flow")
        return (out[: n.value].copy(), nxt[: len(kps)], st[: len(kps)]) if raw else out[: n.value].copy()

    def clip_run(self, first, last, keypoint_interval, homography_interval, calibration=False, wait=True):
        stalled = C.c_int(-1)
        rc = self.L.eagle_clip_run(self._h, first, last, keypoint_interval, homography_interval, int(calibration), int(wait), C.byref(stalled))
        if rc == E_REFERENCE_RAISES:
            raise IndexError(self.L.eagle_last_error(self._h).decode())
        self._check(rc, "clip_run")
        return stalled.value

    def clip_fetch(self, n):
        out = np.zeros(n, RESULT_DTYPE)
        self._check(self.L.eagle_clip_fetch(self._h, out.ctypes.data_as(C.c_void_p)), "clip_fetch")
        return out

    def team_colors(self, dptr, n_frames, crops):
        crops = np.ascontiguousarray(crops, np.int32).reshape(-1, 5)
        out = np.zeros((len(crops), 12), np.int32)
        self._check(self.L.eagle_team_colors(self._h, dptr, n_frames, crops.ctypes.data_as(C.c_void_p), len(crops), out.ctypes.data_as(C.c_void_p)), "team_colors")
        return out

    def track_open(self, **params):
        p = None
        if params:
            d = dict(track_high_thresh=0.5, track_low_thresh=0.1, new_track_thresh=0.6, match_thresh=0.8, track_buffer=30, frame_rate=30)
            d.update(params)
            p = C.byref(EagleTrackParams(**d))
        self._check(self.L.eagle_track_open(self._h, p), "track_open")

    def reid_features(self, dptr, n_frames, crops):
        crops = np.ascontiguousarray(crops, np.int32).reshape(-1, 5)
        out = np.zeros((len(crops), 512), np.float32)
        self._check(self.L.eagle_reid_features(self._h, dptr, n_frames, crops.ctypes.data_as(C.c_void_p), len(crops), out.ctypes.data_as(C.POINTER(C.c_float))), "reid_features")
        return out

    def track_frames_reid(self, recs, feats, feat_det, feat_count, warps=None):
        assert recs.dtype == RESULT_DTYPE and recs.flags.c_contiguous
        feats = np.ascontiguousarray(feats, np.float32).reshape(-1, 512)
        feat_det = np.ascontiguousarray(feat_det, np.int32); feat_count = np.ascontiguousarray(feat_count, np.int32)
        assert len(feat_count) == len(recs) and int(feat_count.sum()) == len(feats) == len(feat_det)
        w = None if warps is None else np.ascontiguousarray(warps, np.float64).reshape(len(recs), 6)
        self._check(self.L.eagle_track_frames_reid(self._h, recs.ctypes.data_as(C.c_void_p), len(recs), None if w is None else w.ctypes.data_as(C.POINTER(C.c_double)),
                                                   feats.ctypes.data_as(C.POINTER(C.c_float)), feat_det.ctypes.data_as(C.POINTER(C.c_int32)),
                                                   feat_count.ctypes.data_as(C.POINTER(C.c_int32))), "track_frames_reid")
        return recs

    def track_frames(self, recs, warps=None):
        assert recs.dtype == RESULT_DTYPE and recs.flags.c_contiguous
        w = None
        if warps is not None:
            w = np.ascontiguousarray(warps, np.float64).reshape(len(recs), 6)
        self._check(self.L.eagle_track_frames_cmc(self._h, recs.ctypes.data_as(C.c_void_p), len(recs),
                                                  w.ctypes.data_as(C.POINTER(C.c_double)) if w is not None else None), "track_frames")
        return recs

    def clip_motion(self, first, count):
        w = np.zeros((max(count, 0), 6), np.float64)
        self._check(self.L.eagle_clip_motion(self._h, first, count, w.ctypes.data_as(C.POINTER(C.c_double))), "clip_motion")
        return w

    def clip_motion_ecc(self, first, count, carry=False, return_ok=False):
        w = np.zeros((max(count, 0), 6), np.float64)
        ok = np.zeros(max(count, 0), np.int32)
        self._check(self.L.eagle_clip_motion_ecc(self._h, first, count, int(bool(carry)), w.ctypes.data_as(C.POINTER(C.c_double)),
                                                 ok.ctypes.data_as(C.POINTER(C.c_int32))), "clip_motion_ecc")
        return (w, ok) if return_ok else w

    def set_profiling(self, on):
        self._check(self.L.eagle_set_profiling(self._h, int(on)), "set_profiling")

    def timings(self):
        t = EagleTimings()
        self._check(self.L.eagle_get_timings(self._h, C.byref(t)), "get_timings")
        return t

    def kernel_times(self):
        buf = (EagleKernelTime * 256)(); n = C.c_int(0)
        self._check(self.L.eagle_get_kernel_times(self._h, buf, 256, C.byref(n)), "get_kernel_times")
        return [(buf[i].name.decode(), float(buf[i].ms), int(buf[i].launches), float(buf[i].bytes), float(buf[i].flop)) for i in range(min(n.value, 256))]

    def comm_init(self, rank, world, uid_bytes):
        buf = C.create_string_buffer(bytes(uid_bytes), 128)
        self._check(self.L.eagle_comm_init(self._h, rank, world, buf), "comm_init")

    def gather(self, local, world, out=None):
        local = np.ascontiguousarray(local)
        if out is None:
            out = np.zeros(len(local) * world, RESULT_DTYPE)
        assert out.dtype == RESULT_DTYPE and len(out) == len(local) * world and out.flags.c_contiguous
        self._check(self.L.eagle_gather(self._h, local.ctypes.data_as(C.c_void_p), len(local), out.ctypes.data_as(C.c_void_p)), "gather")
        return out


def comm_unique_id():
    buf = C.create_string_buffer(128)
    rc = load().eagle_comm_id(buf)
    if rc:
        raise EagleError(f"eagle_comm_id failed ({rc}): {load().eagle_last_error(None).decode()}")
    return buf.raw


def op_conv2d(x, w_hwio, bias, stride=1, pre=0, r1=None, r2=None, post=0, precision=PREC_F32, device=0):
    L = load()
    x = np.ascontiguousarray(x, np.float32); w = np.ascontiguousarray(w_hwio, np.float32); b = np.ascontiguousarray(bias, np.float32)
    n, h, wd, cin = x.shape
    ks, _, _, cout = w.shape
    ho = (h + 2 * (ks // 2) - ks) // stride + 1
    wo = (wd + 2 * (ks // 2) - ks) // stride + 1
    y = np.empty((n, ho, wo, cout), np.float32)
    r1 = None if r1 is None else np.ascontiguousarray(r1, np.float32)
    r2 = None if r2 is None else np.ascontiguousarray(r2, np.float32)
    rc = L.eagle_op_conv2d(device, precision, _fp(x), n, h, wd, cin, _fp(w), _fp(b), cout, ks, stride, pre, _fp(r1), _fp(r2), post, _fp(y))
    if rc:
        raise EagleError(f"eagle_op_conv2d failed ({rc}): {L.eagle_last_error(None).decode()}")
    return y


def op_bottleneck(x, w1, b1, w2, b2, w3, b3, res=None, reps=0, device=0, wd=None, bd=None):
    L = load()
    x = np.ascontiguousarray(x, np.float32)
    n, h, w, cin = x.shape
    arrs = [np.ascontiguousarray(a, np.float32) for a in (w1, b1, w2, b2, w3, b3)]
    assert arrs[0].shape == (1, 1, cin, 64) and arrs[2].shape == (3, 3, 64, 64) and arrs[4].shape == (1, 1, 64, 256), "HWIO weights of a 64-wide Bottleneck"
    res = None if res is None else np.ascontiguousarray(res, np.float32)
    y = np.empty((n, h, w, 256), np.float32)
    ms = C.c_float(0)
    wd = None if wd is None else np.ascontiguousarray(wd, np.float32)
    bd = None if bd is None else np.ascontiguousarray(bd, np.float32)
    rc = L.eagle_op_bottleneck(device, _fp(x), n, h, w, cin, *[_fp(a) for a in arrs], _fp(res), _fp(y), int(reps), C.byref(ms), _fp(wd), _fp(bd))
    if rc:
        raise EagleError(f"eagle_op_bottleneck failed ({rc}): {L.eagle_last_error(None).decode()}")
    return (y, ms.value) if reps > 0 else y


def op_fuse_sum(base, ups, relu=True, precision=PREC_F32, device=0):
    L = load()
    base = np.ascontiguousarray(base, np.float32)
    n, H, W, c = base.shape
    ups = [np.ascontiguousarray(u, np.float32) for u in ups]
    arr = (C.POINTER(C.c_float) * max(len(ups), 1))(*[_fp(u) for u in ups])
    uh = (C.c_int * max(len(ups), 1))(*[u.shape[1] for u in ups])
    uw = (C.c_int * max(len(ups), 1))(*[u.shape[2] for u in ups])
    y = np.empty_like(base)
    rc = L.eagle_op_fuse_sum(device, precision, _fp(base), n, H, W, c, len(ups), arr, uh, uw, int(relu), _fp(y))
    if rc:
        raise EagleError(f"eagle_op_fuse_sum failed ({rc}): {L.eagle_last_error(None).decode()}")
    return y


def op_preprocess(frames, det_imgsz=640, precision=PREC_F32, device=0, letterbox=0):
    L = load()
    frames = np.ascontiguousarray(frames, np.uint8)
    n, h, w, _ = frames.shape
    hw = (C.c_int * 2)()
    rc = L.eagle_op_preprocess_lb(device, precision, frames.ctypes.data_as(C.POINTER(C.c_uint8)), n, h, w, det_imgsz, int(letterbox), None, None, hw)
    if rc:
        raise EagleError(f"eagle_op_preprocess failed ({rc}): {L.eagle_last_error(None).decode()}")
    kp = np.empty((n, 540, 960, 3), np.float32)
    det = np.empty((n, hw[0], hw[1], 3), np.float32)
    rc = L.eagle_op_preprocess_lb(device, precision, frames.ctypes.data_as(C.POINTER(C.c_uint8)), n, h, w, det_imgsz, int(letterbox), _fp(kp), _fp(det), hw)
    if rc:
        raise EagleError(f"eagle_op_preprocess failed ({rc}): {L.eagle_last_error(None).decode()}")
    return kp, det


def op_find_homography(img_pts, world_pts, thresh=5.0, max_iters=2000, lm_iters=10, device=0):
    L = load()
    a = np.ascontiguousarray(img_pts, np.float32).reshape(-1, 2)
    b = np.ascontiguousarray(world_pts, np.float32).reshape(-1, 2)
    n = len(a)
    H = np.zeros(9, np.float64); mask = np.zeros(max(n, 1), np.uint8); ok = C.c_int(0)
    rc = L.eagle_op_find_homography(device, _fp(a), _fp(b), n, thresh, max_iters, lm_iters,
                                    H.ctypes.data_as(C.POINTER(C.c_double)), mask.ctypes.data_as(C.POINTER(C.c_uint8)), C.byref(ok))
    if rc:
        raise EagleError(f"eagle_op_find_homography failed ({rc}): {L.eagle_last_error(None).decode()}")
    return (H.reshape(3, 3), mask[:n]) if ok.value else (None, None)


def _pix(fmt):
    if isinstance(fmt, str):
        if fmt.lower() not in PIX_FORMATS:
            raise EagleError(f"unknown pixel format {fmt!r} (nv12 or i420)")
        return PIX_FORMATS[fmt.lower()]
    return int(fmt)


def _yuv_layout(layout):
    if layout is None or isinstance(layout, EagleYuvLayout):
        return layout
    lay = EagleYuvLayout()
    for k, v in dict(layout).items():
        if k not in dict(EagleYuvLayout._fields_):
            raise TypeError(f"unknown layout field {k}")
        setattr(lay, k, int(v))
    return lay


def yuv_span(fmt, h, w, layout, n):
    lay = _yuv_layout(layout) or EagleYuvLayout()
    nv12 = _pix(fmt) == PIX_FORMATS["nv12"]
    c_row = w if nv12 else w // 2
    yp = lay.y_pitch or w
    co = lay.c_offset or yp * h
    cp = lay.c_pitch or c_row
    planes = [(0, yp, h, w), (co, cp, h // 2, c_row)]
    if not nv12:
        planes.append((lay.v_offset or co + cp * (h // 2), cp, h // 2, c_row))
    extent = max(o + p * (r - 1) + b for o, p, r, b in planes)
    stride = lay.frame_stride or max(o + p * r for o, p, r, _ in planes)
    return 0 if n <= 0 else (n - 1) * stride + extent


def op_yuv_to_bgr(frames, fmt="nv12", layout=None, h=None, w=None, n=None, device=0):
    L = load()
    a = np.asarray(frames)
    if a.ndim in (2, 3):
        if a.ndim == 2:
            a = a[None]
        n, h, w = a.shape[0], a.shape[1] * 2 // 3, a.shape[2]
    elif h is None or w is None or n is None:
        raise EagleError("a flat 4:2:0 buffer needs h, w and n")
    a = np.ascontiguousarray(a, np.uint8)
    lay = _yuv_layout(layout)
    if a.ndim == 1 and a.nbytes < yuv_span(fmt, h, w, lay, n):
        raise EagleError(f"the buffer holds {a.nbytes} bytes, {n} frames of this layout span {yuv_span(fmt, h, w, lay, n)}")
    out = np.empty((n, h, w, 3), np.uint8)
    rc = L.eagle_op_yuv_to_bgr(device, _pix(fmt), a.ctypes.data_as(C.POINTER(C.c_uint8)), n, h, w, None if lay is None else C.byref(lay),
                               out.ctypes.data_as(C.POINTER(C.c_uint8)))
    if rc:
        raise EagleError(f"eagle_op_yuv_to_bgr failed ({rc}): {L.eagle_last_error(None).decode()}")
    return out
```

include/eagle.h:

```cpp
#ifndef EAGLE_H
#define EAGLE_H
#include <stdint.h>

#ifdef __cplusplus
extern "C" {
#endif

#define EAGLE_OK 0
#define EAGLE_E_INVALID (-1)
#define EAGLE_E_HIP (-2)
#define EAGLE_E_STATE (-3)
#define EAGLE_E_MISSING (-4)
#define EAGLE_E_NOKERNEL (-5)
#define EAGLE_E_COMM (-6)
#define EAGLE_E_RANGE (-8)

#define EAGLE_MAX_DET 300
#define EAGLE_N_LANDMARKS 57
#define EAGLE_MAX_KP 87

#define EAGLE_PREC_F16 0
#define EAGLE_PREC_F32 1
#define EAGLE_PREC_F32S 2

// ... 16 lines not shown
typedef struct EagleConfig {
    int32_t device;
    int32_t frame_h, frame_w;
    int32_t det_variant;
    int32_t det_imgsz;
    int32_t batch;
    int32_t precision;
    double keypoint_conf;
    double detector_conf;
    double ransac_thresh;
    float detector_floor;
    float nms_iou;
    int32_t ransac_max_iters;
    int32_t lm_iters;
    int32_t use_graph;
    int32_t det_precision;
    int32_t allow_saturation;
    int32_t multi_stream;
    int32_t letterbox;
    int32_t reserved[3];
} EagleConfig;

typedef struct EagleDet {
    float x1, y1, x2, y2;
    float conf;
    int32_t cls;
    int32_t id;
    int32_t bx1, by1, bx2, by2;
    int32_t foot_x, foot_y;
    float pitch_xf, pitch_yf;
    int32_t pitch_x, pitch_y;
    uint8_t reported;
    uint8_t in_bounds;
    uint8_t pad[2];
} EagleDet;

typedef struct EagleKeypoint {
    int32_t label;
    int32_t x, y;
    float score;
    uint8_t synthesized;
    uint8_t on_plane;
    uint8_t inlier;
    uint8_t pad;
} EagleKeypoint;

typedef struct EagleFrameResult {
    int32_t n_det;
    int32_t n_kp;
    int32_t n_candidates;
    uint8_t H_valid;
    uint8_t bounds_valid;
    uint8_t pad[2];
    double H[9];
    double bounds[4];
    int32_t hm_idx[EAGLE_N_LANDMARKS];
    float hm_score[EAGLE_N_LANDMARKS];
    EagleKeypoint kp[EAGLE_MAX_KP];
    EagleDet det[EAGLE_MAX_DET];
} EagleFrameResult;

int eagle_abi_sizes(int32_t* out4);
int eagle_default_config(EagleConfig* cfg);
int eagle_create(const EagleConfig* cfg, EagleHandle** out);
void eagle_destroy(EagleHandle* h);
const char* eagle_last_error(EagleHandle* h);
int eagle_resolve_config(EagleConfig* cfg);
int eagle_get_config(EagleHandle* h, EagleConfig* cfg);

int eagle_load_weights(EagleHandle* h, const char* name, const float* data, const int64_t* shape, int ndim);
int eagle_finalize_weights(EagleHandle* h);

int eagle_process_frames(EagleHandle* h, const uint8_t* bgr, int n, int64_t frame_stride, int64_t row_stride,
                         EagleFrameResult* out);
int eagle_host_alloc(EagleHandle* h, int64_t bytes, void** ptr);
int eagle_host_free(EagleHandle* h, void* ptr);

int eagle_process_device_frames(EagleHandle* h, const void* d_bgr, int n, EagleFrameResult* out);
int eagle_device_alloc(EagleHandle* h, int64_t bytes, void** dptr);
int eagle_device_free(EagleHandle* h, void* dptr);
int eagle_device_upload(EagleHandle* h, void* dptr, const void* src, int64_t bytes);

#define EAGLE_PIX_NV12 1
#define EAGLE_PIX_I420 2
typedef struct EagleYuvLayout {
    int64_t frame_stride;
    int64_t y_pitch;
    int64_t c_offset;
    int64_t c_pitch;
    int64_t v_offset;
} EagleYuvLayout;
int eagle_process_frames_yuv(EagleHandle* h, int format, const uint8_t* src, int n, const EagleYuvLayout* layout, EagleFrameResult* out);
int eagle_process_device_frames_yuv(EagleHandle* h, int format, const void* d_src, int n, const EagleYuvLayout* layout, EagleFrameResult* out);
int eagle_yuv_to_bgr(EagleHandle* h, int format, const void* d_src, int n, const EagleYuvLayout* layout, void* d_bgr);
int eagle_op_yuv_to_bgr(int device, int format, const uint8_t* src, int n, int h, int w, const EagleYuvLayout* layout, uint8_t* bgr);

int eagle_reproject(EagleHandle* h, EagleFrameResult* recs, int n, const double* Hs, const uint8_t* flags);

typedef struct EagleFlowKp { int32_t label; int32_t x, y; float score; } EagleFlowKp;
int eagle_clip_open(EagleHandle* h, const void* d_bgr, int n);
int eagle_clip_detect_objects(EagleHandle* h, int first, int count);
int eagle_clip_detect_keypoints(EagleHandle* h, int first, int stride, int count);
int eagle_clip_get_keypoints(EagleHandle* h, int frame, EagleFlowKp* out , int* n );
int eagle_clip_set_keypoints(EagleHandle* h, int frame, const EagleFlowKp* in, int n);
int eagle_clip_flow(EagleHandle* h, int src_frame, int dst_frame, int hue_frame, const EagleFlowKp* in, int n_in,
                    EagleFlowKp* out , int* n_out, float* next_pts , uint8_t* status );
int eagle_clip_run(EagleHandle* h, int first, int last, int keypoint_interval, int homography_interval, int calibration, int wait,
                   int* stalled_at);
int eagle_clip_fetch(EagleHandle* h, EagleFrameResult* out);
int eagle_clip_close(EagleHandle* h);
#define EAGLE_E_REFERENCE_RAISES (-7)

typedef struct EagleCrop { int32_t frame, x1, y1, x2, y2; } EagleCrop;
typedef struct EagleTrackParams {
    float track_high_thresh, track_low_thresh, new_track_thresh, match_thresh;
    int32_t track_buffer, frame_rate;
} EagleTrackParams;
int eagle_track_open(EagleHandle* h, const EagleTrackParams* params );
int eagle_track_frames(EagleHandle* h, EagleFrameResult* recs, int n);
int eagle_clip_motion(EagleHandle* h, int first, int count, double* warps);
int eagle_clip_motion_ecc(EagleHandle* h, int first, int count, int carry, double* warps, int* ok);
int eagle_track_frames_cmc(EagleHandle* h, EagleFrameResult* recs, int n, const double* warps );
#define EAGLE_REID_DIM 512
int eagle_reid_features(EagleHandle* h, const void* d_bgr, int n_frames, const EagleCrop* crops, int n_crops, float* feats);
int eagle_track_frames_reid(EagleHandle* h, EagleFrameResult* recs, int n, const double* warps , const float* feats,
                            const int32_t* feat_det, const int32_t* feat_count);

int eagle_team_colors(EagleHandle* h, const void* d_bgr, int n_frames, const EagleCrop* crops, int n_crops, int32_t* counts);

int eagle_comm_id(void* id128);
int eagle_comm_init(EagleHandle* h, int rank, int world, const void* id128);
int eagle_gather(EagleHandle* h, const EagleFrameResult* local, int n_local, EagleFrameResult* all );

typedef struct EagleTimings {
    float total_ms;
    float conv_ms;
    int32_t n_launches;
    int32_t n_conv_launches;
    double conv_flop;
    int32_t sat_events;
    int32_t sat_frames;
    int32_t graph_captures;
    int32_t graph_skipped;
    int32_t reserved[4];
} EagleTimings;
int eagle_set_profiling(EagleHandle* h, int per_kernel_events);
int eagle_get_timings(EagleHandle* h, EagleTimings* t);
typedef struct EagleKernelTime { char name[40]; float ms; int32_t launches; double bytes; double flop; } EagleKernelTime;
int eagle_get_kernel_times(EagleHandle* h, EagleKernelTime* out, int cap, int* n);

int eagle_op_conv2d(int device, int precision, const float* x, int n, int h, int w, int cin, const float* w_hwio,
                    const float* bias, int cout, int ks, int stride, int pre_act, const float* r1, const float* r2,
                    int post_act, float* y);
int eagle_op_bottleneck(int device, const float* x, int n, int h, int w, int cin, const float* w1, const float* b1, const float* w2, const float* b2,
                        const float* w3, const float* b3, const float* res, float* y, int reps, float* ms,
                        const float* wd , const float* bd);
int eagle_op_fuse_sum(int device, int precision, const float* base, int n, int H, int W, int c, int n_up,
                      const float* const* ups, const int* up_h, const int* up_w, int relu, float* y);
int eagle_op_preprocess(int device, int precision, const uint8_t* bgr, int n, int h, int w, int det_imgsz,
                        float* kp_out , float* det_out , int* det_hw );
int eagle_op_preprocess_lb(int device, int precision, const uint8_t* bgr, int n, int h, int w, int det_imgsz, int letterbox ,
                           float* kp_out, float* det_out, int* det_hw);
int eagle_op_find_homography(int device, const float* img_pts, const float* world_pts, int n, double thresh,
                             int max_iters, int lm_iters, double* H9, uint8_t* mask, int* ok);

int eagle_debug(const char* key, int64_t value, void* out, int64_t out_bytes);

#ifdef __cplusplus
}
#endif
#endif
```

Baseline: 819.5.

## Group paired detector head convs into one launch and fuse SPPF maxpools

The YOLO detection head's box and class branches are merged. Their weights are concatenated along Cout, so each pair of same-shaped convs runs as one launch. Block columns past a boundary read input from a second channel offset (grouped conv), and the first layer, which shares its input, runs as a plain concatenated conv. The three chained SPPF 5x5 maxpools become one kernel that keeps intermediates in LDS. The aim is to cut kernel launches and improve occupancy for the small detector convs, at the cost of stricter pairing conditions (matching configs and weight exponents) and an extra per-block offset computation.

After: 818.2. About the same (-0.2%).

```diff
diff --git a/eagle_amd/csrc/common.h b/eagle_amd/csrc/common.h
--- a/eagle_amd/csrc/common.h
+++ b/eagle_amd/csrc/common.h
@@ -58,13 +58,18 @@
     float descale = 1.0f;
     ArgmaxPart* const* am_slot = nullptr;
     unsigned* const* sat_slot = nullptr;
+    int g_cout = 0, g_xoff = 0;
 };
 int conv_tiles_per_frame(int precision, const ConvConfig& cfg, int ho, int wo);
 bool conv_supported(int precision, const ConvConfig& cfg);
+bool conv_groupable(int precision, const ConvConfig& cfg);
+void conv_prepare(int precision, const ConvLaunch& L);
 void conv_launch(int precision, const ConvLaunch& L, hipStream_t s);
 size_t conv_weight_elems(int precision, const ConvConfig& cfg);
 size_t conv_lds_bytes(int precision, const ConvConfig& cfg);
 void conv_tile_weights(int precision, const ConvConfig& cfg, const float* w_hwio, int cin_real, int cout_real, void* dst, float* descale = nullptr);
+int conv_weight_exponent(const float* w, size_t n);
+void maxpool5x3_launch(const TView& x, const TView& y1, const TView& y2, const TView& y3, hipStream_t s);
 inline int prec_tensor_fmt(int precision) { return precision == EAGLE_PREC_F32 ? 1 : precision == EAGLE_PREC_F32S ? 2 : 0; }
 inline bool prec_is_f16_kernels(int precision) { return precision == EAGLE_PREC_F16 || precision == EAGLE_PREC_F32S; }
 ConvConfig conv_choose(int precision, int ks, int stride, int cin_pad, int cout_pad, int wo, bool plain_epilogue = false, bool second_residual = false);
diff --git a/eagle_amd/csrc/conv.hip b/eagle_amd/csrc/conv.hip
--- a/eagle_amd/csrc/conv.hip
+++ b/eagle_amd/csrc/conv.hip
@@ -1,4 +1,5 @@
 #include <algorithm>
+#include <climits>
 #include <cmath>
 #include <cstdlib>
 #include <mutex>
@@ -103,6 +104,7 @@
     }
     return nullptr;
 }
+bool conv_groupable(int precision, const ConvConfig& c) { return kind_of(precision, c) == GENERIC && generic_inst(precision, c); }
 bool conv_supported(int precision, const ConvConfig& c)
 {
     const Form* f = find_form(precision, c.variant);
@@ -249,6 +251,15 @@
     }
 }
 
+int conv_weight_exponent(const float* w, size_t n)
+{
+    float amax = 0.f;
+    for (size_t k = 0; k < n; ++k) amax = std::max(amax, std::fabs(w[k]));
+    int e = 0;
+    if (amax > 0.f) (void)std::frexp(amax, &e);
+    return e;
+}
+
 void conv_tile_weights(int precision, const ConvConfig& c, const float* w, int cin_real, int cout_real, void* dst, float* descale)
 {
     const int bn = c.nt * 16, nblk = c.cout_pad / bn, nch = c.cin / c.kc, taps = c.ks * c.ks, wimage = form_of(precision, c).wimage;
@@ -257,10 +268,7 @@
     };
     if (descale) *descale = 1.0f;
     if (precision == EAGLE_PREC_F32S) {
-        float amax = 0.f;
-        for (size_t k = 0; k < (size_t)taps * cin_real * cout_real; ++k) amax = std::max(amax, std::fabs(w[k]));
-        int e = 0;
-        if (amax > 0.f) (void)std::frexp(amax, &e);
+        const int e = conv_weight_exponent(w, (size_t)taps * cin_real * cout_real);
         const int sw = 15 - e;
         const float scale = std::ldexp(1.0f, sw);
         if (descale) *descale = std::ldexp(1.0f, -(sw + 4));
@@ -390,6 +398,16 @@
     return z[dev];
 }
 
+void conv_prepare(int precision, const ConvLaunch& L)
+{
+    const ConvConfig& c = L.cfg;
+    if (!conv_supported(precision, c)) return;
+    const Form& f = form_of(precision, c);
+    const int nres = (L.r1.p ? 1 : 0) + (L.r2.p ? 1 : 0);
+    if (f.kind == ADIRECT) { for (bool d : {false, true}) ensure_max_dynamic_lds((const void*)f.get(nres, d), 160 * 1024); }
+    else ensure_max_dynamic_lds((const void*)generic_inst(precision, c)->fn, 160 * 1024);
+}
+
 void conv_launch(int precision, const ConvLaunch& L, hipStream_t s)
 {
     const ConvConfig& c = L.cfg;
@@ -413,6 +431,12 @@
     a.wx = c.wx;
     a.nchunks = c.cin / c.kc;
     a.zeros = conv_zero_page(); a.trash = conv_trash_page(); a.xcd = 0; a.gy = 1; a.stack = 0;
+    a.g_nb = INT_MAX; a.g_xoff = 0;
+    if (L.g_cout) {
+        if (!conv_groupable(precision, c) || L.g_cout % (c.nt * 16) || L.g_cout >= c.cout_pad || L.g_xoff < 0 || L.x.off + L.g_xoff + c.cin > L.x.cs || L.am_slot)
+            fail(EAGLE_E_NOKERNEL, "grouped conv: needs a generic kernel form, a first problem of whole Cout blocks and both inputs inside one buffer");
+        a.g_nb = L.g_cout / (c.nt * 16); a.g_xoff = L.g_xoff * (precision == EAGLE_PREC_F32S ? 2 : 1);
+    }
     a.am = L.am_slot ? *L.am_slot : nullptr; a.am_cs = c.cout_pad;
     a.sat = (L.sat_slot && precision == EAGLE_PREC_F32S) ? *L.sat_slot : nullptr;
     if (f.kind == ADIRECT) {
diff --git a/eagle_amd/csrc/conv_internal.h b/eagle_amd/csrc/conv_internal.h
--- a/eagle_amd/csrc/conv_internal.h
+++ b/eagle_amd/csrc/conv_internal.h
@@ -20,6 +20,7 @@
     int gy;
     int stack;
     int xcd;
+    int g_nb, g_xoff;
     ArgmaxPart* am;
     int am_cs;
     float descale;
diff --git a/eagle_amd/csrc/conv_kernels.inc b/eagle_amd/csrc/conv_kernels.inc
--- a/eagle_amd/csrc/conv_kernels.inc
+++ b/eagle_amd/csrc/conv_kernels.inc
@@ -290,6 +290,7 @@
         const int item = (xcd < rn ? xcd * (qn + 1) : rn * (qn + 1) + (xcd - rn) * qn) + k;
         t = item / gy; nb = item - t * gy;
     }
+    const int xoff = a.xoff + (nb >= a.g_nb ? a.g_xoff : 0);
     const int tx = t % a.tiles_x; t /= a.tiles_x;
     const int ty = t % a.tiles_y;
     const int n = t / a.tiles_y;
@@ -350,7 +351,7 @@
             if (!((EAGLE_ABL == 5 || EAGLE_ABL == 6 || EAGLE_ABL >= 8) && SPLIT && (CH_) > 0))                                               \
             _Pragma("unroll") for (int i = 0; i < NPW; ++i) { const int o = (tid + 256 * i) * 16; pw[i] = __builtin_amdgcn_raw_buffer_load_b128(wrs, o < WBYTES ? o : 0, wso_, 0); } \
         }                                                                                                               \
-        const unsigned xso_ = (unsigned)(a.xoff + (CH_) * KCS) * 2u;                                                    \
+        const unsigned xso_ = (unsigned)(xoff + (CH_) * KCS) * 2u;                                                      \
         _Pragma("unroll") for (int j = 0; j < RND; ++j)                                                                 \
             if ((R0_) + j < NPA && !((EAGLE_ABL == 2 || EAGLE_ABL >= 4) && SPLIT && (CH_) > 0)) pa[j] = __builtin_amdgcn_raw_buffer_load_b128(xrs, aoff[(R0_) + j < NPA ? (R0_) + j : 0], xso_, 0); \
     }
@@ -727,6 +728,7 @@
     const int ty = stack ? t : t % a.tiles_y;
     const int n0 = stack ? 0 : t / a.tiles_y;
     const int nb = blockIdx.y;
+    const int xoff = a.xoff + (nb >= a.g_nb ? a.g_xoff : 0);
     const int oy0 = ty * TH, ox0 = tx * TW;
     const int iy0 = oy0 * S - KS / 2, ix0 = ox0 * S - KS / 2;
 
@@ -758,7 +760,7 @@
         bool ok = idx < nelem && ix >= 0 && ix < a.W;
         if (stack) { n = iy >= 0 ? iy / Hs : 0; iy -= n * Hs; ok = ok && n < a.N; }
         ok = ok && iy >= 0 && iy < a.H;
-        aoff[j] = ok ? (unsigned)(((n * a.H + iy) * a.W + ix) * a.xcs + a.xoff + g * 4) * 4u : OOB_OFF;
+        aoff[j] = ok ? (unsigned)(((n * a.H + iy) * a.W + ix) * a.xcs + xoff + g * 4) * 4u : OOB_OFF;
         ldso[j] = idx < nelem ? pix * PSF + g * 4 : -1;
     }
 
diff --git a/eagle_amd/csrc/elementwise.hip b/eagle_amd/csrc/elementwise.hip
--- a/eagle_amd/csrc/elementwise.hip
+++ b/eagle_amd/csrc/elementwise.hip
@@ -330,6 +330,61 @@
 }
 
 template <typename T>
+__global__ __launch_bounds__(256) void maxpool5x3_kernel(TView x, TView y1, TView y2, TView y3)
+{
+    constexpr int VN = Vec<T>::N;
+    extern __shared__ __attribute__((aligned(16))) float pool_lds[];
+    const int H = x.h, W = x.w, groups = x.c / VN, HW = H * W;
+    const int g = blockIdx.x % groups, n = blockIdx.x / groups;
+    for (int p = threadIdx.x; p < HW; p += blockDim.x) {
+        Vec<T> v; v.load(x.p, ((size_t)n * HW + p) * x.cs + x.off + g * VN);
+        for (int k = 0; k < VN; ++k) pool_lds[p * VN + k] = v.v[k];
+    }
+    __syncthreads();
+    for (int stage = 0; stage < 3; ++stage) {
+        const float* src = pool_lds + (size_t)stage * HW * VN;
+        float* dst = pool_lds + (size_t)(stage + 1) * HW * VN;
+        const TView& y = stage == 0 ? y1 : stage == 1 ? y2 : y3;
+        for (int p = threadIdx.x; p < HW; p += blockDim.x) {
+            const int oy = p / W, ox = p - oy * W;
+            Vec<T> m;
+            for (int k = 0; k < VN; ++k) m.v[k] = -INFINITY;
+            for (int dy = -2; dy <= 2; ++dy) {
+                const int iy = oy + dy;
+                if (iy < 0 || iy >= H) continue;
+                for (int dx = -2; dx <= 2; ++dx) {
+                    const int ix = ox + dx;
+                    if (ix < 0 || ix >= W) continue;
+                    const float* v = src + (iy * W + ix) * VN;
+                    for (int k = 0; k < VN; ++k) m.v[k] = v[k] > m.v[k] ? v[k] : m.v[k];
+                }
+            }
+            const size_t e = ((size_t)n * HW + p) * y.cs + y.off + g * VN;
+            m.store(y.p, e);
+            if (stage < 2) {
+                Vec<T> r; r.load(y.p, e);
+                for (int k = 0; k < VN; ++k) dst[p * VN + k] = r.v[k];
+            }
+        }
+        __syncthreads();
+    }
+}
+void maxpool5x3_launch(const TView& x, const TView& y1, const TView& y2, const TView& y3, hipStream_t s)
+{
+    const int vn = x.f32 == 1 ? 4 : 8;
+    const size_t lds = (size_t)3 * x.h * x.w * vn * 4;
+    if (lds > 64 * 1024) {
+        maxpool5_launch(x, y1, s); maxpool5_launch(y1, y2, s); maxpool5_launch(y2, y3, s);
+        return;
+    }
+    const dim3 grid((unsigned)(x.n * (x.c / vn)));
+    if (x.f32 == 1) hipLaunchKernelGGL(maxpool5x3_kernel<float>, grid, dim3(256), lds, s, x, y1, y2, y3);
+    else if (x.f32 == 2) hipLaunchKernelGGL(maxpool5x3_kernel<SplitT>, grid, dim3(256), lds, s, x, y1, y2, y3);
+    else hipLaunchKernelGGL(maxpool5x3_kernel<_Float16>, grid, dim3(256), lds, s, x, y1, y2, y3);
+    HIP_CHECK(hipGetLastError());
+}
+
+template <typename T>
 __global__ __launch_bounds__(256) void upsample2_kernel(TView x, TView y)
 {
     constexpr int VN = Vec<T>::N;
diff --git a/eagle_amd/csrc/nets.hip b/eagle_amd/csrc/nets.hip
--- a/eagle_amd/csrc/nets.hip
+++ b/eagle_amd/csrc/nets.hip
@@ -71,10 +71,58 @@
         char label[64];
         snprintf(label, sizeof(label), "conv %dx%d/%d %d->%d @%dx%d v%d%s", ks, ks, stride, cin, cout, ho, wo, L.cfg.variant, label_suffix);
         const double es = prec == EAGLE_PREC_F16 ? 2 : 4;
+        conv_prepare(prec, L);
         emit_conv(label, L.flop, (double)N * x.h * x.w * cin * es + (double)N * ho * wo * cout * ((out_f32 || prec != EAGLE_PREC_F16) ? 4 : 2) * (am_slot ? 0 : 1) +
                                  (r1 ? (double)N * ho * wo * cout * es : 0) + (r2 ? (double)N * ho * wo * cout * es : 0) + (double)ks * ks * cin * cout * es,
                   [L, pr](hipStream_t s) { conv_launch(pr, L, s); });
         return L.y;
+    }
+    bool conv_pair(const TView& xa, const TView& xb, const std::string cname[2], const std::string bn[2], int pre, bool out_f32, TView out[2])
+    {
+        if (xa.p != xb.p || xa.h != xb.h || xa.w != xb.w || xa.c != xb.c || xa.cs != xb.cs || xa.f32 != xb.f32 || xb.off < xa.off) return false;
+        std::vector<float> hw[2], bs[2]; int cin[2], cout[2], ks[2], cpad[2];
+        ConvConfig cfg[2];
+        for (int k = 0; k < 2; ++k) {
+            fold(cname[k], bn[k], hw[k], bs[k], cin[k], cout[k], ks[k]);
+            cpad[k] = (cout[k] + 15) / 16 * 16;
+            if (cin[k] > xa.c) fail(EAGLE_E_INVALID, "%s: input has %d channels, weight expects %d", cname[k].c_str(), xa.c, cin[k]);
+            cfg[k] = conv_choose(prec, ks[k], 1, xa.c, cpad[k], xa.w, pre == ACT_NONE && !out_f32, false);
+        }
+        if (cin[0] != cin[1] || ks[0] != ks[1] || cfg[0].kc != cfg[1].kc || cfg[0].nt != cfg[1].nt || cfg[0].wx != cfg[1].wx || cfg[0].variant != cfg[1].variant) return false;
+        if (!conv_groupable(prec, cfg[0]) || cpad[0] % (cfg[0].nt * 16)) return false;
+        if (prec == EAGLE_PREC_F32S && conv_weight_exponent(hw[0].data(), hw[0].size()) != conv_weight_exponent(hw[1].data(), hw[1].size())) return false;
+        const int k_s = ks[0], ci = cin[0], ct = cpad[0] + cout[1], ctp = cpad[0] + cpad[1];
+        std::vector<float> hwio((size_t)k_s * k_s * ci * ct, 0.f), bias(ctp, 0.f);
+        for (int t = 0; t < k_s * k_s * ci; ++t) {
+            std::copy(hw[0].begin() + (size_t)t * cout[0], hw[0].begin() + (size_t)(t + 1) * cout[0], hwio.begin() + (size_t)t * ct);
+            std::copy(hw[1].begin() + (size_t)t * cout[1], hw[1].begin() + (size_t)(t + 1) * cout[1], hwio.begin() + (size_t)t * ct + cpad[0]);
+        }
+        std::copy(bs[0].begin(), bs[0].end(), bias.begin());
+        std::copy(bs[1].begin(), bs[1].end(), bias.begin() + cpad[0]);
+        ConvLaunch L;
+        L.cfg = cfg[0]; L.cfg.cout_pad = ctp;
+        if (!conv_supported(prec, L.cfg)) return false;
+        std::vector<char> tiled(conv_weight_elems(prec, L.cfg) * (prec == EAGLE_PREC_F32 ? 4 : 2));
+        conv_tile_weights(prec, L.cfg, hwio.data(), ci, ct, tiled.data(), &L.descale);
+        L.w = net->upload(tiled.data(), tiled.size());
+        L.bias = (const float*)net->upload(bias.data(), bias.size() * 4);
+        const bool grouped = xb.off != xa.off;
+        L.x = xa;
+        if (grouped) { L.g_cout = cpad[0]; L.g_xoff = xb.off - xa.off; }
+        L.y = act(xa.h, xa.w, ctp, out_f32);
+        L.pre_act = pre; L.post_act = 0; L.out_f32 = out_f32 ? 1 : 0;
+        refuse_2gib(cname[0], "layer", {&L.x, &L.y});
+        if (prec == EAGLE_PREC_F32S && !out_f32) L.sat_slot = &H->cur_sat;
+        L.flop = 2.0 * N * xa.h * xa.w * (double)(cout[0] + cout[1]) * ci * k_s * k_s;
+        const int pr = prec;
+        char label[80];
+        snprintf(label, sizeof(label), "conv %dx%d/1 %d->%d%c%d @%dx%d v%d%s", k_s, k_s, ci, cout[0], grouped ? '|' : '+', cout[1], xa.h, xa.w, L.cfg.variant, label_suffix);
+        const double es = prec == EAGLE_PREC_F16 ? 2 : 4, co = cout[0] + cout[1];
+        conv_prepare(prec, L);
+        emit_conv(label, L.flop, (double)N * xa.h * xa.w * ci * es * (grouped ? 2 : 1) + (double)N * xa.h * xa.w * co * ((out_f32 || prec != EAGLE_PREC_F16) ? 4 : 2) + (double)k_s * k_s * ci * co * es,
+                  [L, pr](hipStream_t s) { conv_launch(pr, L, s); });
+        out[0] = L.y.slice(0, cpad[0]); out[1] = L.y.slice(cpad[0], cpad[1]);
+        return true;
     }
     void fold(const std::string& cname, const std::string& bn, std::vector<float>& hwio, std::vector<float>& bias, int& cin, int& cout, int& ks)
     {
@@ -325,6 +373,7 @@
 {
     YoloBuilder Y{B};
     const YoloDims d = yolo_dims(variant);
+    const bool det_grouping = !(getenv("EAGLE_DET_GROUPING") && atoi(getenv("EAGLE_DET_GROUPING")) == 0);
     const int c1 = d.c[0], c2 = d.c[1], c3 = d.c[2], c4 = d.c[3], c5 = d.c[4];
     TView x0 = Y.cv(x_in, "model.0", 2);
     TView x1 = Y.cv(x0, "model.1", 2); B.release(x0);
@@ -347,9 +396,13 @@
         TView cat = B.act(h5, w5, 4 * ch);
         TView s0 = cat.slice(0, ch), s1 = cat.slice(ch, ch), s2 = cat.slice(2 * ch, ch), s3 = cat.slice(3 * ch, ch);
         Y.cv(x8, "model.9.cv1", 1, nullptr, &s0); B.release(x8);
-        B.other([s0, s1](hipStream_t s) { maxpool5_launch(s0, s1, s); }, "maxpool5", 2 * Builder::vbytes(s0));
-        B.other([s1, s2](hipStream_t s) { maxpool5_launch(s1, s2, s); }, "maxpool5", 2 * Builder::vbytes(s0));
-        B.other([s2, s3](hipStream_t s) { maxpool5_launch(s2, s3, s); }, "maxpool5", 2 * Builder::vbytes(s0));
+        if (det_grouping) {
+            B.other([s0, s1, s2, s3](hipStream_t s) { maxpool5x3_launch(s0, s1, s2, s3, s); }, "maxpool5x3", 4 * Builder::vbytes(s0));
+        } else {
+            B.other([s0, s1](hipStream_t s) { maxpool5_launch(s0, s1, s); }, "maxpool5", 2 * Builder::vbytes(s0));
+            B.other([s1, s2](hipStream_t s) { maxpool5_launch(s1, s2, s); }, "maxpool5", 2 * Builder::vbytes(s0));
+            B.other([s2, s3](hipStream_t s) { maxpool5_launch(s2, s3, s); }, "maxpool5", 2 * Builder::vbytes(s0));
+        }
         Y.cv(cat, "model.9.cv2", 1, nullptr, &p5);
         B.release(cat);
     }
@@ -401,12 +454,19 @@
     int a0 = 0;
     for (int l = 0; l < 3; ++l) {
         const std::string pb = "model.22.cv2." + std::to_string(l), pc = "model.22.cv3." + std::to_string(l);
-        TView b0 = Y.cv(feats[l], pb + ".0");
-        TView b1 = Y.cv(b0, pb + ".1"); B.release(b0);
-        TView box = B.conv(b1, pb + ".2", "", 1, 0, nullptr, nullptr, 0, nullptr, true); B.release(b1);
-        TView k0 = Y.cv(feats[l], pc + ".0");
-        TView k1 = Y.cv(k0, pc + ".1"); B.release(k0);
-        TView cls = B.conv(k1, pc + ".2", "", 1, 0, nullptr, nullptr, 0, nullptr, true); B.release(k1);
+        TView t[2] = {feats[l], feats[l]};
+        for (int k = 0; k < 3; ++k) {
+            const std::string sfx = "." + std::to_string(k);
+            const std::string cn[2] = {pb + sfx + (k < 2 ? ".conv" : ""), pc + sfx + (k < 2 ? ".conv" : "")};
+            const std::string bnn[2] = {k < 2 ? pb + sfx + ".bn" : "", k < 2 ? pc + sfx + ".bn" : ""};
+            TView o[2];
+            const bool paired = det_grouping && B.conv_pair(t[0], t[1], cn, bnn, k < 2 ? Y.S : 0, k == 2, o);
+            if (!paired)
+                for (int j = 0; j < 2; ++j) o[j] = B.conv(t[j], cn[j], bnn[j], 1, k < 2 ? Y.S : 0, nullptr, nullptr, 0, nullptr, k == 2);
+            if (k > 0) { B.release(t[0]); if (t[1].p != t[0].p) B.release(t[1]); }
+            t[0] = o[0]; t[1] = o[1];
+        }
+        const TView box = t[0], cls = t[1];
         lv[l].box = box; lv[l].cls = cls; lv[l].gh = box.h; lv[l].gw = box.w; lv[l].stride = strides[l]; lv[l].a0 = a0;
         a0 += box.h * box.w;
     }
diff --git a/eagle_amd/csrc/ops_api.hip b/eagle_amd/csrc/ops_api.hip
--- a/eagle_amd/csrc/ops_api.hip
+++ b/eagle_amd/csrc/ops_api.hip
@@ -80,6 +80,78 @@
     API_END(hh)
 }
 
+int eagle_op_conv2d_pair(int device, int precision, const float* const* x, int n, int h, int w, int cin, const float* const* w_hwio, const float* const* bias,
+                         const int* cout, int ks, int pre_act, int grouped, float* const* y)
+{
+    EagleHandle* hh = nullptr;
+    API_BEGIN
+    HIP_CHECK(hipSetDevice(device));
+    if (!x || !w_hwio || !bias || !cout || !y || n < 1 || cin < 1 || cout[0] < 1 || cout[1] < 1) fail(EAGLE_E_INVALID, "eagle_op_conv2d_pair: bad argument");
+    Net net;
+    const int cin_pad = (cin + 15) / 16 * 16, cp[2] = {(cout[0] + 15) / 16 * 16, (cout[1] + 15) / 16 * 16};
+    std::vector<float> xx((size_t)n * h * w * 2 * cin_pad, 0.f);
+    for (size_t p = 0; p < (size_t)n * h * w; ++p)
+        for (int k = 0; k < 2; ++k) std::copy(x[k] + p * cin, x[k] + (p + 1) * cin, xx.begin() + (p * 2 + k) * cin_pad);
+    TView X, Y;
+    to_dev(net, precision, xx.data(), n, h, w, 2 * cin_pad, 2 * cin_pad, X);
+    Y = X; Y.c = Y.cs = cp[0] + cp[1]; Y.off = 0;
+    Y.p = net.get((size_t)n * h * w * Y.cs * Y.esize());
+    ConvLaunch L;
+    L.cfg = conv_choose(precision, ks, 1, cin_pad, cp[0], w, pre_act == ACT_NONE, false);
+    if (!conv_groupable(precision, L.cfg) || cp[1] % (L.cfg.nt * 16)) fail(EAGLE_E_NOKERNEL, "eagle_op_conv2d_pair: the first problem's tile configuration does not fit both");
+    L.pre_act = pre_act;
+    const int ct = cp[0] + cout[1];
+    std::vector<float> wc((size_t)ks * ks * cin * ct, 0.f), bc(cp[0] + cp[1], 0.f);
+    for (int t = 0; t < ks * ks * cin; ++t)
+        for (int k = 0; k < 2; ++k) std::copy(w_hwio[k] + (size_t)t * cout[k], w_hwio[k] + (size_t)(t + 1) * cout[k], wc.begin() + (size_t)t * ct + (k ? cp[0] : 0));
+    for (int k = 0; k < 2; ++k) std::copy(bias[k], bias[k] + cout[k], bc.begin() + (k ? cp[0] : 0));
+    auto tile = [&](ConvLaunch& q, const float* wsrc, int co_real, const float* b, int nb) {
+        std::vector<char> tiled(conv_weight_elems(precision, q.cfg) * (precision == EAGLE_PREC_F32 ? 4 : 2));
+        conv_tile_weights(precision, q.cfg, wsrc, cin, co_real, tiled.data(), &q.descale);
+        q.w = net.upload(tiled.data(), tiled.size());
+        q.bias = (const float*)net.upload(b, (size_t)nb * 4);
+    };
+    if (grouped) {
+        if (precision == EAGLE_PREC_F32S && conv_weight_exponent(w_hwio[0], (size_t)ks * ks * cin * cout[0]) != conv_weight_exponent(w_hwio[1], (size_t)ks * ks * cin * cout[1]))
+            fail(EAGLE_E_INVALID, "eagle_op_conv2d_pair: split family — the two weight tensors need the same power-of-two scale to share an image");
+        L.cfg.cout_pad = cp[0] + cp[1];
+        tile(L, wc.data(), ct, bc.data(), cp[0] + cp[1]);
+        L.x = X.slice(0, cin_pad); L.y = Y; L.g_cout = cp[0]; L.g_xoff = cin_pad;
+        conv_launch(precision, L, nullptr);
+    } else {
+        for (int k = 0; k < 2; ++k) {
+            ConvLaunch q = L;
+            q.cfg.cout_pad = cp[k];
+            std::vector<float> b(cp[k], 0.f);
+            std::copy(bias[k], bias[k] + cout[k], b.begin());
+            tile(q, w_hwio[k], cout[k], b.data(), cp[k]);
+            q.x = X.slice(k * cin_pad, cin_pad); q.y = Y.slice(k ? cp[0] : 0, cp[k]);
+            conv_launch(precision, q, nullptr);
+        }
+    }
+    HIP_CHECK(hipDeviceSynchronize());
+    from_dev(Y.slice(0, cp[0]), cout[0], y[0]);
+    from_dev(Y.slice(cp[0], cp[1]), cout[1], y[1]);
+    API_END(hh)
+}
+
+int eagle_op_maxpool5x3(int device, int precision, const float* x, int n, int h, int w, int c, int fused, float* y1, float* y2, float* y3)
+{
+    EagleHandle* hh = nullptr;
+    API_BEGIN
+    HIP_CHECK(hipSetDevice(device));
+    if (!x || !y1 || !y2 || !y3 || n < 1 || h < 1 || w < 1 || c < 8 || c % 8) fail(EAGLE_E_INVALID, "eagle_op_maxpool5x3: c must be a positive multiple of 8");
+    Net net;
+    TView X, Y[3];
+    to_dev(net, precision, x, n, h, w, c, c, X);
+    for (auto& v : Y) { v = X; v.p = net.get((size_t)n * h * w * c * X.esize()); }
+    if (fused) maxpool5x3_launch(X, Y[0], Y[1], Y[2], nullptr);
+    else { maxpool5_launch(X, Y[0], nullptr); maxpool5_launch(Y[0], Y[1], nullptr); maxpool5_launch(Y[1], Y[2], nullptr); }
+    HIP_CHECK(hipDeviceSynchronize());
+    from_dev(Y[0], c, y1); from_dev(Y[1], c, y2); from_dev(Y[2], c, y3);
+    API_END(hh)
+}
+
 int eagle_op_bottleneck(int device, const float* x, int n, int h, int w, int cin, const float* w1, const float* b1, const float* w2, const float* b2,
                         const float* w3, const float* b3, const float* res, float* y, int reps, float* ms, const float* wd, const float* bd)
 {
diff --git a/eagle_amd/lib.py b/eagle_amd/lib.py
--- a/eagle_amd/lib.py
+++ b/eagle_amd/lib.py
@@ -127,6 +127,9 @@
     L.eagle_op_preprocess.argtypes = [i32, i32, u8p, i32, i32, i32, i32, fp, fp, C.POINTER(i32)]
     L.eagle_op_preprocess_lb.argtypes = [i32, i32, u8p, i32, i32, i32, i32, i32, fp, fp, C.POINTER(i32)]
     L.eagle_op_find_homography.argtypes = [i32, fp, fp, i32, C.c_double, i32, i32, dp, u8p, C.POINTER(i32)]
+    if hasattr(L, "eagle_op_conv2d_pair"):
+        L.eagle_op_conv2d_pair.argtypes = [i32, i32, C.POINTER(fp), i32, i32, i32, i32, C.POINTER(fp), C.POINTER(fp), C.POINTER(i32), i32, i32, i32, C.POINTER(fp)]
+        L.eagle_op_maxpool5x3.argtypes = [i32, i32, fp, i32, i32, i32, i32, i32, fp, fp, fp]
     L.eagle_debug.argtypes = [C.c_char_p, i64, vp, i64]
     L.eagle_team_colors.argtypes = [vp, vp, i32, vp, i32, vp]
     L.eagle_track_open.argtypes = [vp, C.POINTER(EagleTrackParams)]
@@ -152,7 +155,7 @@
            "eagle_op_find_homography", "eagle_clip_open", "eagle_clip_close", "eagle_clip_detect_objects", "eagle_clip_detect_keypoints", "eagle_clip_get_keypoints",
            "eagle_clip_set_keypoints", "eagle_clip_flow", "eagle_clip_run", "eagle_clip_fetch", "eagle_debug", "eagle_track_open", "eagle_track_frames", "eagle_track_frames_cmc", "eagle_clip_motion_ecc", "eagle_clip_motion", "eagle_team_colors",
            "eagle_reid_features", "eagle_track_frames_reid", "eagle_process_frames_yuv", "eagle_process_device_frames_yuv", "eagle_yuv_to_bgr",
-           "eagle_op_yuv_to_bgr"]
+           "eagle_op_yuv_to_bgr", "eagle_op_conv2d_pair", "eagle_op_maxpool5x3"]
 
 FLOWKP_DTYPE = np.dtype([("label", "<i4"), ("x", "<i4"), ("y", "<i4"), ("score", "<f4")], align=True)
 E_REFERENCE_RAISES = -7
@@ -520,6 +523,31 @@
     return y
 
 
+def op_conv2d_pair(xs, ws, bs, pre=0, grouped=True, precision=PREC_F32, device=0):
+    L = load()
+    xs = [np.ascontiguousarray(x, np.float32) for x in xs]; ws = [np.ascontiguousarray(w, np.float32) for w in ws]; bs = [np.ascontiguousarray(b, np.float32) for b in bs]
+    n, h, wd, cin = xs[0].shape
+    assert xs[1].shape == xs[0].shape and ws[0].shape[:3] == ws[1].shape[:3] == (ws[0].shape[0], ws[0].shape[0], cin)
+    ks = ws[0].shape[0]
+    ys = [np.empty((n, h, wd, w.shape[3]), np.float32) for w in ws]
+    arr = lambda a: (C.POINTER(C.c_float) * 2)(*[_fp(v) for v in a])
+    rc = L.eagle_op_conv2d_pair(device, precision, arr(xs), n, h, wd, cin, arr(ws), arr(bs), (C.c_int * 2)(ws[0].shape[3], ws[1].shape[3]), ks, pre, int(grouped), arr(ys))
+    if rc:
+        raise EagleError(f"eagle_op_conv2d_pair failed ({rc}): {L.eagle_last_error(None).decode()}")
+    return ys
+
+
+def op_maxpool5x3(x, fused=True, precision=PREC_F32, device=0):
+    L = load()
+    x = np.ascontiguousarray(x, np.float32)
+    n, h, w, c = x.shape
+    ys = [np.empty_like(x) for _ in range(3)]
+    rc = L.eagle_op_maxpool5x3(device, precision, _fp(x), n, h, w, c, int(fused), *[_fp(y) for y in ys])
+    if rc:
+        raise EagleError(f"eagle_op_maxpool5x3 failed ({rc}): {L.eagle_last_error(None).decode()}")
+    return ys
+
+
 def op_bottleneck(x, w1, b1, w2, b2, w3, b3, res=None, reps=0, device=0, wd=None, bd=None):
     L = load()
     x = np.ascontiguousarray(x, np.float32)
diff --git a/include/eagle.h b/include/eagle.h
--- a/include/eagle.h
+++ b/include/eagle.h
@@ -192,6 +192,9 @@
 int eagle_op_conv2d(int device, int precision, const float* x, int n, int h, int w, int cin, const float* w_hwio,
                     const float* bias, int cout, int ks, int stride, int pre_act, const float* r1, const float* r2,
                     int post_act, float* y);
+int eagle_op_conv2d_pair(int device, int precision, const float* const* x, int n, int h, int w, int cin, const float* const* w_hwio, const float* const* bias,
+                         const int* cout, int ks, int pre_act, int grouped, float* const* y);
+int eagle_op_maxpool5x3(int device, int precision, const float* x, int n, int h, int w, int c, int fused, float* y1, float* y2, float* y3);
 int eagle_op_bottleneck(int device, const float* x, int n, int h, int w, int cin, const float* w1, const float* b1, const float* w2, const float* b2,
                         const float* w3, const float* b3, const float* res, float* y, int reps, float* ms,
                         const float* wd , const float* bd);
```
